# mmetcalf14/qml-cutensornet

Measured on AMD Instinct MI355X. Metric: Gram kernel entries/sec @ 60 qubits x 6 layers, higher is better.
Workload: dtype f64 (complex128)

## Files before the change

qml-cutensornet_amd/csrc/qk_fused.h:

```cpp
#pragma once
#include "qk_device.h"
#include "qk_plan.h"

#define QKF_PRIO_LO() __builtin_amdgcn_s_setprio(0)
#define QKF_PRIO_HI() __builtin_amdgcn_s_setprio(2)
typedef double v2d __attribute__((ext_vector_type(2)));
typedef __attribute__((address_space(3))) v2d lds_v2d;
static constexpr int QKF_XSTEP = 4 * TILE;
static constexpr int QKF_XBLOCK = TILE * TILE;


#ifndef QKF_LDS3M
#define QKF_LDS3M 0
#endif
#ifndef QKF_P2_PROBE
#define QKF_P2_PROBE 0
#endif
#ifndef QKF_ABL
#define QKF_ABL 0
#endif
#define QKF_STEP_BARRIER()                            \
  do {                                                \
    if (QKF_ABL & 4) asm volatile("s_waitcnt lgkmcnt(0)" ::: "memory"); \
    else qk_lds_barrier();                            \
  } while (0)
#define QKF_SUM(a, b) ((QKF_ABL & 1) ? (a) : (a) + (b))
#define QKF_DIF(a, b) ((QKF_ABL & 1) ? (b) : (a) - (b))
template <bool CONJB>
__device__ __forceinline__ void qkf_kstep(v4d& p1, v4d& p2, v4d& p3, const double ar, const double ai, const double br, const double bi) {
  const double sa = QKF_SUM(ar, ai), sb = CONJB ? QKF_DIF(br, bi) : QKF_SUM(br, bi);
  p1 = __builtin_amdgcn_mfma_f64_16x16x4f64(ar, br, p1, 0, 0, 0);
  p2 = __builtin_amdgcn_mfma_f64_16x16x4f64(ai, bi, p2, 0, 0, 0);
  p3 = __builtin_amdgcn_mfma_f64_16x16x4f64(sa, sb, p3, 0, 0, 0);
}

struct QkfTile {
  v4d re, im;
};

__device__ __forceinline__ v2d qkf_ldg(const v2d* __restrict__ base, const unsigned off) {
  return *reinterpret_cast<const v2d*>(reinterpret_cast<const char*>(base) + (size_t)(off * 16u));
}
#ifndef QKF_NT_A
#define QKF_NT_A 0
#endif
#ifndef QKF_NT_B
#define QKF_NT_B 0
#endif
__device__ __forceinline__ v2d qkf_ldg_nt(const v2d* __restrict__ base, const unsigned off) {
  return __builtin_nontemporal_load(reinterpret_cast<const v2d*>(reinterpret_cast<const char*>(base) + (size_t)(off * 16u)));
}
__device__ __forceinline__ v2d qkf_ldg_a(const v2d* __restrict__ base, const unsigned off) { return QKF_NT_A ? qkf_ldg_nt(base, off) : qkf_ldg(base, off); }
__device__ __forceinline__ v2d qkf_ldg_b(const v2d* __restrict__ base, const unsigned off) { return QKF_NT_B ? qkf_ldg_nt(base, off) : qkf_ldg(base, off); }
__device__ __forceinline__ v2d qkf_ldx(const v2d* __restrict__ base, const unsigned off) { return qkf_ldg(base, off); }
__device__ __forceinline__ v2d qkf_ldx(const lds_v2d* base, const unsigned off) { return base[off]; }

struct QkfStream {
  const v2d* base;
  unsigned off;
  int step;
  int lim = 4;
};
__device__ __forceinline__ const v2d* qkf_kbase(const v2d* const base, const int step, const int i, const int lim) { return base + max(min(i, lim - 1), 0) * step; }
__device__ __forceinline__ void qkf_load4(v2d (&fr)[4], const QkfStream& st) {
#pragma unroll
  for (int i = 0; i < 4; ++i) fr[i] = qkf_ldg(qkf_kbase(st.base, st.step, i, st.lim), st.off);
}
__device__ __forceinline__ v2d qkf_ldgb(const v2d* __restrict__ base, const unsigned boff) {
  const v2d* const at = reinterpret_cast<const v2d*>(reinterpret_cast<const char*>(base) + (size_t)boff);
  return QKF_NT_B ? __builtin_nontemporal_load(at) : *at;
}
struct QkfXLds {
  const lds_v2d* p;
  __device__ __forceinline__ void advance() { p += 4 * QKF_XSTEP; }
  __device__ __forceinline__ v2d kstep(const int i) const { return p[i * QKF_XSTEP]; }
};
struct QkfXGlobal {
  const v2d* base;
  unsigned bo;
  __device__ __forceinline__ void advance() { bo += 4 * QKF_XSTEP * 16u; }
  __device__ __forceinline__ v2d kstep(const int i) const { return *reinterpret_cast<const v2d*>(reinterpret_cast<const char*>(base + i * QKF_XSTEP) + (size_t)bo); }
};
__device__ __forceinline__ QkfXLds qkf_xcursor(const lds_v2d* xp, const unsigned xoff) { return QkfXLds{xp + xoff}; }
__device__ __forceinline__ QkfXGlobal qkf_xcursor(const v2d* xp, const unsigned xoff) { return QkfXGlobal{xp, xoff * 16u}; }

template <typename XPtr>
__device__ __forceinline__ void qkf_p1_tile(QkfTile& t, v2d (&fr)[4], const bool primed, QkfStream cur, XPtr xp, unsigned xoff, const int nks, const QkfStream nxt) {
  v4d p1 = {0, 0, 0, 0}, p2 = {0, 0, 0, 0}, p3 = {0, 0, 0, 0};
  v2d fx[4];
  const int ng = (nks + 3) >> 2, last = nks - 4 * (ng - 1);
  if (!primed) qkf_load4(fr, cur);
#pragma unroll
  for (int i = 0; i < 4; ++i) fx[i] = qkf_ldx(xp + i * QKF_XSTEP, xoff);
  const v2d* cb[4];
#pragma unroll
  for (int i = 0; i < 4; ++i) cb[i] = qkf_kbase(cur.base, cur.step, i, ng == 2 ? last : 4);
  unsigned bo = cur.off * 16u;
  const unsigned bs = (unsigned)(4 * cur.step) * 16u;
  auto xq = qkf_xcursor(xp, xoff);
  QKF_PRIO_LO();
  int gq = 0;
  if (ng >= 2) {
    gq = 1;
    bo += bs, xq.advance();
#pragma unroll
    for (int i = 0; i < 4; ++i) {
      if (i == 0) {
        const v4d z = {0, 0, 0, 0};
        p1 = __builtin_amdgcn_mfma_f64_16x16x4f64(fx[0].x, fr[0].x, z, 0, 0, 0);
        p2 = __builtin_amdgcn_mfma_f64_16x16x4f64(fx[0].y, fr[0].y, z, 0, 0, 0);
        p3 = __builtin_amdgcn_mfma_f64_16x16x4f64(QKF_SUM(fx[0].x, fx[0].y), QKF_SUM(fr[0].x, fr[0].y), z, 0, 0, 0);
      } else {
        qkf_kstep<false>(p1, p2, p3, fx[i].x, fx[i].y, fr[i].x, fr[i].y);
      }
      if (!(QKF_ABL & 2)) fr[i] = qkf_ldgb(cb[i], bo);
      if (!(QKF_ABL & 8)) fx[i] = xq.kstep(i);
      __builtin_amdgcn_sched_barrier(0);
    }
  }
#pragma unroll 1
  for (int pass = 0; pass < 2; ++pass) {
    const int end = ng - 2 + pass;
#pragma unroll 1
    for (; gq < end; ++gq) {
      bo += bs, xq.advance();
#pragma unroll
      for (int i = 0; i < 4; ++i) {
        qkf_kstep<false>(p1, p2, p3, fx[i].x, fx[i].y, fr[i].x, fr[i].y);
        if (!(QKF_ABL & 2)) fr[i] = qkf_ldgb(cb[i], bo);
        if (!(QKF_ABL & 8)) fx[i] = xq.kstep(i);
        __builtin_amdgcn_sched_barrier(0);
      }
    }
#pragma unroll
    for (int i = 0; i < 4; ++i) cb[i] = qkf_kbase(cur.base, cur.step, i, last);
  }
#pragma unroll
  for (int i = 0; i < 4; ++i) {
    if (i < last) qkf_kstep<false>(p1, p2, p3, fx[i].x, fx[i].y, fr[i].x, fr[i].y);
    if (!(QKF_ABL & 2)) fr[i] = qkf_ldg(qkf_kbase(nxt.base, nxt.step, i, nxt.lim), nxt.off);
    __builtin_amdgcn_sched_barrier(0);
  }
  QKF_PRIO_HI();
  t.re = p1 - p2;
  t.im = p3 - p1 - p2;
}

typedef __attribute__((address_space(3))) int lds_int;
struct QkfTurn {
  lds_int* at;
  int idx;
  lds_int* broken;
  unsigned long long* gerr;
};
__device__ __forceinline__ void qkf_turn_add(__attribute__((address_space(3))) double* const d, const long rs, const v4d& re, const v4d& im, const QkfTurn& t, const int tn) {
  lds_int* const turn = t.at + tn;
  if (t.idx > 0) {
    int spins = 0;
#ifdef QKF_FIRST_STORE
    while (__builtin_amdgcn_readfirstlane(__hip_atomic_load(turn, __ATOMIC_RELAXED, __HIP_MEMORY_SCOPE_WORKGROUP)) == 0) {
#else
    while (__builtin_amdgcn_readfirstlane(__hip_atomic_load(turn, __ATOMIC_RELAXED, __HIP_MEMORY_SCOPE_WORKGROUP)) != t.idx) {
#endif
      __builtin_amdgcn_s_sleep(1);
      if (++spins > (1 << 20) || __builtin_amdgcn_readfirstlane(__hip_atomic_load(t.broken, __ATOMIC_RELAXED, __HIP_MEMORY_SCOPE_WORKGROUP)) != 0) {
        __hip_atomic_store(t.broken, 1, __ATOMIC_RELAXED, __HIP_MEMORY_SCOPE_WORKGROUP);
        if (t.gerr) *t.gerr = 1ull;
        break;
      }
    }
#pragma unroll
    for (int r = 0; r < 4; ++r) {
      __hip_atomic_fetch_add(d + r * rs, re[r], __ATOMIC_RELAXED, __HIP_MEMORY_SCOPE_WORKGROUP);
      __hip_atomic_fetch_add(d + r * rs + 1, im[r], __ATOMIC_RELAXED, __HIP_MEMORY_SCOPE_WORKGROUP);
    }
  } else {
#pragma unroll
    for (int r = 0; r < 4; ++r) *(lds_v2d*)(d + r * rs) = (v2d){re[r], im[r]};
  }
#ifdef QKF_FIRST_STORE
  if (t.idx > 0) return;
#endif
  asm volatile("s_waitcnt lgkmcnt(0)" ::: "memory");
  __hip_atomic_store(turn, t.idx + 1, __ATOMIC_RELAXED, __HIP_MEMORY_SCOPE_WORKGROUP);
}

template <bool FULL, bool DET = false>
__device__ __forceinline__ void qkf_p2_item(const QkfTile& t, v2d (&fr)[4], const bool primed, QkfStream cur, const int ps, const int nn, const int kmax, lds_v2d* xo, const int q,
                                            const int j, const QkfStream nxt, const QkfTurn turn = QkfTurn{nullptr, 0, nullptr, nullptr}) {
  if (!primed) qkf_load4(fr, cur);
  __attribute__((address_space(3))) double* d = (__attribute__((address_space(3))) double*)(xo + q * TILE + j);
  if constexpr (!DET) {
    const v4d z = {0, 0, 0, 0};
    const v4d s = t.re + t.im;
#pragma unroll 1
    for (int tn = 0; tn < nn; ++tn) {
      v4d p1 = z, re, im;
      double sp[4], sm[4];
      const bool fin = tn + 1 == nn;
      const v2d* const rb = fin ? nxt.base : cur.base;
      const int rs = fin ? nxt.step : cur.step, rl = fin ? nxt.lim : FULL ? 4 : kmax;
      cur.off = fin ? nxt.off : cur.off + TILE;
      QKF_PRIO_LO();
#pragma unroll
      for (int i = 0; i < 4; ++i) {
        if (FULL || i == 0 || i < kmax) {
          p1 = __builtin_amdgcn_mfma_f64_16x16x4f64(s[i], fr[i].x, i == 0 ? z : p1, 0, 0, 0);
          sp[i] = QKF_DIF(-fr[i].x, fr[i].y), sm[i] = QKF_DIF(fr[i].y, fr[i].x);
        }
        if (!(QKF_ABL & 2)) fr[i] = qkf_ldg_a(qkf_kbase(rb, rs, i, rl), cur.off);
        __builtin_amdgcn_sched_barrier(0);
      }
#pragma unroll
      for (int i = 0; i < 4; ++i) {
        if (FULL || i == 0 || i < kmax) {
          re = __builtin_amdgcn_mfma_f64_16x16x4f64(t.im[i], sm[i], i == 0 ? p1 : re, 0, 0, 0);
          im = __builtin_amdgcn_mfma_f64_16x16x4f64(t.re[i], sp[i], i == 0 ? p1 : im, 0, 0, 0);
        }
        __builtin_amdgcn_sched_barrier(0);
      }
      QKF_PRIO_HI();
#pragma unroll
      for (int r = 0; r < 4; ++r) {
        __hip_atomic_fetch_add(d + r * 2 * QKF_XSTEP, re[r], __ATOMIC_RELAXED, __HIP_MEMORY_SCOPE_WORKGROUP);
        __hip_atomic_fetch_add(d + r * 2 * QKF_XSTEP + 1, im[r], __ATOMIC_RELAXED, __HIP_MEMORY_SCOPE_WORKGROUP);
      }
      d += 2 * ps;
    }
    return;
  }
#pragma unroll 1
  for (int tn = 0; tn < nn; ++tn) {
    v4d p1 = {0, 0, 0, 0}, p2 = {0, 0, 0, 0}, p3 = {0, 0, 0, 0};
    const bool fin = tn + 1 == nn;
    const v2d* const rb = fin ? nxt.base : cur.base;
    const int rs = fin ? nxt.step : cur.step, rl = fin ? nxt.lim : FULL ? 4 : kmax;
    cur.off = fin ? nxt.off : cur.off + TILE;
    QKF_PRIO_LO();
#pragma unroll
    for (int i = 0; i < 4; ++i) {
      if (FULL || i < kmax) qkf_kstep<true>(p1, p2, p3, t.re[i], t.im[i], fr[i].x, fr[i].y);
      if (!(QKF_ABL & 2)) fr[i] = qkf_ldg_a(qkf_kbase(rb, rs, i, rl), cur.off);
      __builtin_amdgcn_sched_barrier(0);
    }
    QKF_PRIO_HI();
    const v4d re = p1 + p2, im = p3 - p1 + p2;
    qkf_turn_add(d, (long)2 * QKF_XSTEP, re, im, turn, tn);
    d += 2 * ps;
  }
}

template <int S>
__device__ __forceinline__ void qkf_rotate(QkfTile (&T)[S], const int L) {
  if constexpr (S >= 2) {
    if (L == 2) {
      const QkfTile t = T[S - 2];
      T[S - 2] = T[S - 1], T[S - 1] = t;
    }
  }
  if constexpr (S >= 3) {
    if (L == 3) {
      const QkfTile t = T[S - 3];
      T[S - 3] = T[S - 2], T[S - 2] = T[S - 1], T[S - 1] = t;
    }
  }
  if constexpr (S >= 4) {
    if (L >= 4) {
      const QkfTile t0 = T[0];
#pragma unroll
      for (int e = 0; e + 1 < S; ++e) T[e] = T[e + 1];
      T[S - 1] = t0;
    }
  }
}

#ifdef QKF_EDGE_PAIRS_V
#define QKF_EDGE_PAIRS(WPS) (QKF_EDGE_PAIRS_V != 0)
#else
#define QKF_EDGE_PAIRS(WPS) false
#endif
#ifdef QKF_EDGE_SETS_V
#define QKF_EDGE_SETS(WPS) (QKF_EDGE_SETS_V)
#else
#define QKF_EDGE_SETS(WPS) ((WPS) <= 3 ? 2 : 1)
#endif
__device__ __forceinline__ v2d qkf_lde(const v2d* __restrict__ base, const unsigned boff, const int col = 0) {
  return reinterpret_cast<const v2d*>(reinterpret_cast<const char*>(base) + (size_t)boff)[col];
}
template <bool HAS1, bool MORE>
__device__ __forceinline__ void qkf_edge_group(v4d (&acc)[6], v2d (&fy)[4], v2d (&fz)[4], v2d (&fx)[4], const v2d* const* const by, const v2d* const* const bx, const unsigned boy,
                                               const unsigned box) {
#pragma unroll
  for (int i = 0; i < 4; ++i) {
    const double sb = QKF_DIF(fx[i].x, fx[i].y);
    acc[0] = __builtin_amdgcn_mfma_f64_16x16x4f64(fy[i].x, fx[i].x, acc[0], 0, 0, 0);
    acc[1] = __builtin_amdgcn_mfma_f64_16x16x4f64(fy[i].y, fx[i].y, acc[1], 0, 0, 0);
    acc[2] = __builtin_amdgcn_mfma_f64_16x16x4f64(QKF_SUM(fy[i].x, fy[i].y), sb, acc[2], 0, 0, 0);
    if (HAS1) {
      acc[3] = __builtin_amdgcn_mfma_f64_16x16x4f64(fz[i].x, fx[i].x, acc[3], 0, 0, 0);
      acc[4] = __builtin_amdgcn_mfma_f64_16x16x4f64(fz[i].y, fx[i].y, acc[4], 0, 0, 0);
      acc[5] = __builtin_amdgcn_mfma_f64_16x16x4f64(QKF_SUM(fz[i].x, fz[i].y), sb, acc[5], 0, 0, 0);
    }
    if (MORE) {
      fy[i] = qkf_lde(by[i], boy);
      if (HAS1) fz[i] = qkf_lde(by[i], boy, TILE);
      fx[i] = qkf_lde(bx[i], box);
    }
    __builtin_amdgcn_sched_barrier(0);
  }
}
template <bool HAS1, int SETS>
__device__ __forceinline__ void qkf_edge_unit(QkfTile& t0, QkfTile& t1, const v2d* __restrict__ Ay, const unsigned oy, const int ldy, const v2d* __restrict__ Ax, const unsigned ox, const int ldx,
                                              const int ng) {
  static_assert(SETS == 1 || SETS == 2, "one or two groups of k-steps in flight");
  v4d acc[6];
#pragma unroll
  for (int e = 0; e < 6; ++e) acc[e] = (v4d){0, 0, 0, 0};
  v2d fy[SETS][4], fz[SETS][4], fx[SETS][4];
  const v2d *by[4 * SETS], *bx[4 * SETS];
#pragma unroll
  for (int i = 0; i < 4 * SETS; ++i) by[i] = Ay + 4 * i * ldy, bx[i] = Ax + 4 * i * ldx;
  unsigned boy = oy * 16u, box = ox * 16u;
  const unsigned sy = (unsigned)(SETS * TILE * ldy) * 16u, sx = (unsigned)(SETS * TILE * ldx) * 16u;
  const bool two = SETS == 2 && ng > 1;
#pragma unroll
  for (int s = 0; s < SETS; ++s) {
    if (s == 0 || two) {
#pragma unroll
      for (int i = 0; i < 4; ++i) {
        fy[s][i] = qkf_lde(by[4 * s + i], boy);
        if (HAS1) fz[s][i] = qkf_lde(by[4 * s + i], boy, TILE);
        fx[s][i] = qkf_lde(bx[4 * s + i], box);
      }
    }
  }
  QKF_PRIO_LO();
#pragma unroll 1
  for (int g = SETS; g < ng; g += SETS) {
    boy += sy, box += sx;
#pragma unroll
    for (int s = 0; s < SETS; ++s) qkf_edge_group<HAS1, true>(acc, fy[s], fz[s], fx[s], by + 4 * s, bx + 4 * s, boy, box);
  }
  qkf_edge_group<HAS1, false>(acc, fy[0], fz[0], fx[0], by, bx, boy, box);
  if constexpr (SETS == 2) {
    if (two) qkf_edge_group<HAS1, false>(acc, fy[1], fz[1], fx[1], by + 4, bx + 4, boy, box);
  }
  QKF_PRIO_HI();
  t0.re = acc[0] + acc[1], t0.im = acc[2] - acc[0] + acc[1];
  if (HAS1) t1.re = acc[3] + acc[4], t1.im = acc[5] - acc[3] + acc[4];
}
__device__ __forceinline__ long long qkf_uniform(const long long v) {
  const unsigned lo = __builtin_amdgcn_readfirstlane((unsigned)v);
  const unsigned hi = __builtin_amdgcn_readfirstlane((unsigned)((unsigned long long)v >> 32));
  return (long long)(((unsigned long long)hi << 32) | lo);
}

template <int NW, bool PAIRS>
__device__ __forceinline__ QkEdgeUnit qkf_edge_unit_of(const int u, const int mt, const int nt, const int inv) {
  if constexpr (PAIRS) return qk_edge_unit(u, mt, nt, NW, inv);
  const int tb = (u * inv) >> 20;
  return QkEdgeUnit{u - tb * mt, tb, false, true};
}
template <int NW, bool PAIRS, int SETS>
__device__ __forceinline__ void qkf_edge_prefix(const SweepArgs& g, const int xi, const int yj, const int a, const int b, lds_v2d* const xl, v2d* const xg, const bool to_global, const int wave,
                                                const int q, const int j) {
  const v2d* const Lx = reinterpret_cast<const v2d*>(g.xedge) + qkf_uniform(g.xedge_offs[2 * (long long)xi]);
  const v2d* const Ly = reinterpret_cast<const v2d*>(g.yedge) + qkf_uniform(g.yedge_offs[2 * (long long)yj]);
  const int mt = a / TILE, nt = b / TILE, ng = (1 << g.edge_k) >> 4, inv = qk_recip20(mt), units = PAIRS ? qk_edge_units(mt, nt, NW) : mt * nt;
  for (int u = wave; u < units; u += NW) {
    const QkEdgeUnit un = qkf_edge_unit_of<NW, PAIRS>(u, mt, nt, inv);
    if (!un.mine) continue;
    QkfTile T0, T1;
    const unsigned oy = (unsigned)(q * b + un.tb0 * TILE + j), ox = (unsigned)(q * a + un.ta * TILE + j);
    if (un.has1) qkf_edge_unit<true, 1>(T0, T1, Ly, oy, b, Lx, ox, a, ng);
    else qkf_edge_unit<false, SETS>(T0, T1, Ly, oy, b, Lx, ox, a, ng);
    const int at = un.ta * (b * TILE) + (un.tb0 * TILE + q) * TILE + j;
    if (to_global) {
#pragma unroll
      for (int r = 0; r < 4; ++r) xg[at + r * QKF_XSTEP] = (v2d){T0.re[r], T0.im[r]};
      if (un.has1) {
#pragma unroll
        for (int r = 0; r < 4; ++r) xg[at + QKF_XBLOCK + r * QKF_XSTEP] = (v2d){T1.re[r], T1.im[r]};
      }
    } else {
#pragma unroll
      for (int r = 0; r < 4; ++r) xl[at + r * QKF_XSTEP] = (v2d){T0.re[r], T0.im[r]};
      if (un.has1) {
#pragma unroll
        for (int r = 0; r < 4; ++r) xl[at + QKF_XBLOCK + r * QKF_XSTEP] = (v2d){T1.re[r], T1.im[r]};
      }
    }
  }
}

template <int NW, bool PAIRS, int SETS>
__device__ __forceinline__ void qkf_edge_suffix(const SweepArgs& g, const int xi, const int yj, const int a, const int b, const lds_v2d* const xl, const v2d* const xg, const bool from_global,
                                                __attribute__((address_space(3))) double* zacc, const int wave, const int q, const int j) {
  const v2d* const Rx = reinterpret_cast<const v2d*>(g.xedge) + qkf_uniform(g.xedge_offs[2 * (long long)xi + 1]);
  const v2d* const Ry = reinterpret_cast<const v2d*>(g.yedge) + qkf_uniform(g.yedge_offs[2 * (long long)yj + 1]);
  const int mt = a / TILE, nt = b / TILE, ng = (1 << g.edge_k) >> 4, inv = qk_recip20(mt), units = PAIRS ? qk_edge_units(mt, nt, NW) : mt * nt;
  double zr = 0, zi = 0;
  for (int u = wave; u < units; u += NW) {
    const QkEdgeUnit un = qkf_edge_unit_of<NW, PAIRS>(u, mt, nt, inv);
    if (!un.mine) continue;
    QkfTile T0, T1;
    const unsigned oy = (unsigned)(q * b + un.tb0 * TILE + j), ox = (unsigned)(q * a + un.ta * TILE + j);
    if (un.has1) qkf_edge_unit<true, 1>(T0, T1, Ry, oy, b, Rx, ox, a, ng);
    else qkf_edge_unit<false, SETS>(T0, T1, Ry, oy, b, Rx, ox, a, ng);
    const int at = un.ta * (b * TILE) + (un.tb0 * TILE + q) * TILE + j;
#pragma unroll
    for (int r = 0; r < 4; ++r) {
      const v2d x = from_global ? xg[at + r * QKF_XSTEP] : (v2d)xl[at + r * QKF_XSTEP];
      zr += x.x * T0.re[r] - x.y * T0.im[r], zi += x.x * T0.im[r] + x.y * T0.re[r];
    }
    if (un.has1) {
#pragma unroll
      for (int r = 0; r < 4; ++r) {
        const v2d x = from_global ? xg[at + QKF_XBLOCK + r * QKF_XSTEP] : (v2d)xl[at + QKF_XBLOCK + r * QKF_XSTEP];
        zr += x.x * T1.re[r] - x.y * T1.im[r], zi += x.x * T1.im[r] + x.y * T1.re[r];
      }
    }
  }
#pragma unroll
  for (int o = 32; o > 0; o >>= 1) zr += __shfl_xor(zr, o), zi += __shfl_xor(zi, o);
  if ((q | j) == 0) zacc[2 * wave] = zr, zacc[2 * wave + 1] = zi;
}

struct QkfSite {
  int a, a2, b, b2, at, nks, mt, nt, nn, W, inv, inv2, pd, ps, next;
  bool small;
  const v2d *Ak, *Bk;
};
typedef int v4i __attribute__((ext_vector_type(4)));
typedef __attribute__((address_space(3))) v4i lds_v4i;

template <int XCAP, int NT, bool ITEM_RECIPS = false>
__device__ __forceinline__ void qkf_step_table(const SweepArgs& g, const int xi, const int yj, const long long pair, lds_v4i* const rec, long long* const m_off, const int tid, const QkSegRule rule) {
  const int ns = g.n_sites, n1 = ns + 1;
  const int32_t* const xd = g.xdims + (long long)xi * n1;
  const int32_t* const yd = g.ydims + (long long)yj * n1;
  const int32_t* const xt = g.xtrue + (long long)xi * n1;
  const int32_t* const yt = g.ytrue + (long long)yj * n1;
  const v2d* const xdata = reinterpret_cast<const v2d*>(g.xdata);
  const v2d* const ydata = reinterpret_cast<const v2d*>(g.ydata);
  auto put = [&](const int e, const int a, const int a2, const int b, const int b2, const int ps, const int next, const bool small, const v2d* const A, const v2d* const B)
                 __attribute__((always_inline)) {
    const int mt = a / TILE, nt = b2 / TILE;
    const int W = small ? nt : max(1, min(nt, XCAP / (TILE * a2)));
    rec[3 * e] = (v4i){a, a2, b, b2};
    rec[3 * e + 1] = (v4i){xt[e], (yt[e] + 3) >> 2, W, small ? 1 : 0};
    rec[3 * e + 2] = (v4i){qk_recip20(mt), ps, next, ITEM_RECIPS ? qk_unit_recips(nt, W, false) : 0};
    m_off[2 * e] = (long long)(((const char*)A - (const char*)xdata) / 16);
    m_off[2 * e + 1] = (long long)(((const char*)B - (const char*)ydata) / 16);
  };
  auto plain = [&](const int e, const int next) __attribute__((always_inline)) {
    const int a = xd[e], a2 = xd[e + 1], b = yd[e], b2 = yd[e + 1];
    put(e, a, a2, b, b2, 1, next, qk_seg_small(rule, a, a2, b, b2, 2), xdata + (g.xoffs[(long long)xi * ns + e] >> 1), ydata + (g.yoffs[(long long)yj * ns + e] >> 1));
  };
  if (g.seg == nullptr) {
    for (int e = tid; e < ns; e += NT) plain(e, e + 1);
    return;
  }
  const int ek = g.edge_k, k_hi = ns - ek;
  const unsigned long long w0 = g.seg[2 * pair], w1 = g.seg[2 * pair + 1];
  for (int e = ek + tid; e < k_hi; e += NT) {
    const int i = e - ek;
    if (qk_seg_bit(w0, w1, i) && e + 1 < k_hi) {
      const int a = xd[e], a2 = xd[e + 2], b = yd[e], b2 = yd[e + 2];
      put(e, a, a2, b, b2, 2, e + 2, qk_seg_small(rule, a, a2, b, b2, 4), reinterpret_cast<const v2d*>(g.xmg) + (g.xmg_offs[(long long)xi * g.merge_steps + i] >> 1),
          reinterpret_cast<const v2d*>(g.ymg) + (g.ymg_offs[(long long)yj * g.merge_steps + i] >> 1));
    } else plain(e, e + 1);
  }
}

#ifdef QKF_PROF
#define QKF_PROF_DECL() \
  unsigned long long pf[8] = {0, 0, 0, 0, 0, 0, 0, 0}, pt = __builtin_amdgcn_s_memtime(); \
  const unsigned long long pt0 = pt
#define QKF_STAMP(i)                                              \
  do {                                                            \
    const unsigned long long now_ = __builtin_amdgcn_s_memtime(); \
    pf[i] += now_ - pt;                                           \
    pt = now_;                                                    \
  } while (0)
#define QKF_PROF_FLUSH()                                             \
  do {                                                               \
    if (lane == 0) {                                                 \
      pf[7] = __builtin_amdgcn_s_memtime() - pt0;                    \
      for (int i_ = 0; i_ < 8; ++i_) atomicAdd(g.prof + i_, pf[i_]); \
    }                                                                \
  } while (0)
#else
#define QKF_PROF_DECL()
#define QKF_STAMP(i)
#define QKF_PROF_FLUSH()
#endif

#define QKF_PULLER(NT) ((NT) - 64)
__device__ __forceinline__ void qkf_pull_next(const SweepArgs& g, const int xcc, int& gang_round, long long* const word) {
  const long long pp = qk_pull(g, xcc);
  qk_gang_sync(g, xcc, pp >= 0, gang_round);
  *word = pp;
}

template <int NW, int S, int XCAP, int WPS, bool DET = false>
__global__ __launch_bounds__(64 * NW, WPS) void qk_sweep_fused_kernel(const SweepArgs g) {
  constexpr int NT = 64 * NW;
  extern __shared__ __attribute__((aligned(16))) double lds_raw[];
  lds_v2d* const XL = (lds_v2d*)lds_raw;
  long long* const slot = reinterpret_cast<long long*>(lds_raw + 2 * XCAP);
  const v2d* const xdata = reinterpret_cast<const v2d*>(g.xdata);
  const v2d* const ydata = reinterpret_cast<const v2d*>(g.ydata);
  v2d* const G0 = reinterpret_cast<v2d*>(g.scratch) + (long long)blockIdx.x * 2 * g.x_plane;
  const int tid = threadIdx.x, lane = tid & 63;
  const int wave = __builtin_amdgcn_readfirstlane(tid >> 6);
  const int j = lane & 15, q = lane >> 4;
  const int ns = g.n_sites;
  __attribute__((address_space(3))) double* const zacc = (__attribute__((address_space(3))) double*)(slot + 2);
  lds_v4i* const rec = (lds_v4i*)(slot + 2 + 32);
  long long* const m_off = reinterpret_cast<long long*>(slot + 2 + 32) + 6 * (long long)ns;
  lds_int* const tbroken = (lds_int*)(m_off + 2 * (long long)ns);
  lds_int* const turn0 = tbroken + 2;
  auto rfl = [&](const int v) __attribute__((always_inline)) { return __builtin_amdgcn_readfirstlane(v); };
  auto ldl = [&](const long long* p_) __attribute__((always_inline)) {
    const long long v = *p_;
    const unsigned lo = __builtin_amdgcn_readfirstlane((unsigned)v);
    const unsigned hi = __builtin_amdgcn_readfirstlane((unsigned)((unsigned long long)v >> 32));
    return (long long)(((unsigned long long)hi << 32) | lo);
  };
  auto site = [&](const int k) __attribute__((always_inline)) {
    const v4i r0 = rec[3 * k], r1 = rec[3 * k + 1], r2 = rec[3 * k + 2];
    QkfSite s;
    s.a = rfl(r0.x), s.a2 = rfl(r0.y), s.b = rfl(r0.z), s.b2 = rfl(r0.w);
    s.at = rfl(r1.x), s.nks = rfl(r1.y), s.W = rfl(r1.z), s.small = rfl(r1.w) != 0;
    s.inv = rfl(r2.x), s.inv2 = rfl(r2.w);
    s.ps = rfl(r2.y), s.pd = 1 << s.ps, s.next = rfl(r2.z);
    s.mt = s.a / TILE, s.nt = s.b2 / TILE, s.nn = s.a2 / TILE;
    s.Ak = xdata + ldl(m_off + 2 * k);
    s.Bk = ydata + ldl(m_off + 2 * k + 1);
    return s;
  };
  auto item_of = [&](const QkfSite& s, const int w, const int it) __attribute__((always_inline)) {
    return DET ? qk_unit_decode_ordered(it, s.ps, s.mt, s.inv) : qk_unit_decode(it, s.mt, w, s.inv, qk_unit_recip_of(s.inv2, w == s.W));
  };
  auto b_stream = [&](const QkfSite& s, const int s0, const int w, const int it) __attribute__((always_inline)) {
    const QkUnit un = item_of(s, w, it);
    return QkfStream{s.Bk + un.p * s.b2, (unsigned)((q * s.pd) * s.b2 + (s0 + un.tc) * TILE + j), 4 * s.pd * s.b2, min(4, s.nks)};
  };
  auto a_stream = [&](const QkfSite& s, const int w, const int it) __attribute__((always_inline)) {
    const QkUnit un = item_of(s, w, it);
    return QkfStream{s.Ak + un.p * s.a2, (unsigned)(((un.ta * TILE + q) * s.pd) * s.a2 + j), 4 * s.pd * s.a2, min(4, (s.at - un.ta * TILE + 3) >> 2)};
  };
  QKF_PROF_DECL();
  const int xcc = qk_xcc_id();
  int gang_round = 0;
  if (tid == 0) qk_tail_start(g);
  for (;;) {
    if (tid == 0) {
      const long long pp_ = qk_pull(g, xcc);
      qk_gang_sync(g, xcc, pp_ >= 0, gang_round);
      *slot = pp_;
    }
    __syncthreads();
    const long long p = *slot;
    __syncthreads();
    if (p < 0) break;
    const int xi = g.pairs[2 * p], yj = g.pairs[2 * p + 1];
    qkf_step_table<XCAP, NT, true>(g, xi, yj, p, rec, m_off, tid, QkSegRule{XCAP, NW * S, false});
    const int ek = g.edge_k, k_hi = ns - ek;
    const bool edges = ek > 0;
    if (!edges)
      for (int e = tid; e < TILE * TILE; e += NT) XL[e] = (v2d){e == 0 ? 1.0 : 0.0, 0.0};
    if constexpr (DET)
      for (int e = tid; e < 2 * g.turn_ints + 2; e += NT) tbroken[e] = 0;
    int tsel = 0;
    __syncthreads();
    bool xg = false;
    int cur = 0, xb = 0;
    if (edges) {
      const v4i r0 = rec[3 * ek];
      const int a_e = rfl(r0.x), b_e = rfl(r0.z);
      xg = a_e * b_e > XCAP;
      qkf_edge_prefix<NW, QKF_EDGE_PAIRS(WPS), QKF_EDGE_SETS(WPS)>(g, xi, yj, a_e, b_e, XL, G0, xg, wave, q, j);
      __syncthreads();
    }
    QKF_STAMP(0);
    QkfTile T[S];
    v2d fr[4];
    bool primed = false;
    QkfSite sn = site(ek);
    for (int k = ek; k < k_hi;) {
      const QkfSite sc = sn;
      k = sc.next;
      if (k < k_hi) sn = site(k);
      const int a = sc.a, a2 = sc.a2, b = sc.b, mt = sc.mt, nt = sc.nt, W = sc.W;
      const bool small = sc.small;
      v2d* const Gc = G0 + (long long)cur * g.x_plane;
      v2d* const Gn = G0 + (long long)(cur ^ 1) * g.x_plane;
      if (small && xg) {
        for (int e = tid; e < a * b; e += NT) XL[e] = Gc[e];
        __syncthreads();
        xg = false, xb = 0;
      } else if (!small && !xg) {
        for (int e = tid; e < a * b; e += NT) Gc[e] = XL[xb + e];
        __syncthreads();
        xg = true;
      }
      const int n_out = sc.b2 * a2;
      const bool pingpong = small && a * b + n_out <= XCAP;
      const int ob = !small ? 0 : pingpong ? (xb == 0 ? XCAP - n_out : 0) : 0;
      if (pingpong && !DET)
        for (int e = tid; e < n_out; e += NT) XL[ob + e] = (v2d){0.0, 0.0};
      QKF_STAMP(1);
      for (int s0 = 0; s0 < nt; s0 += W) {
        const int w = min(W, nt - s0), items = sc.pd * mt * w;
        lds_int* const tcur = turn0 + tsel * g.turn_ints;
        if constexpr (DET) {
          for (int e = tid; e < g.turn_ints; e += NT) turn0[(tsel ^ 1) * g.turn_ints + e] = 0;
        } else if (!small) {
          for (int e = tid; e < w * TILE * a2; e += NT) XL[e] = (v2d){0.0, 0.0};
          QKF_STEP_BARRIER();
        }
        QKF_STAMP(6);
        for (int r0 = 0; r0 < items; r0 += NW * S) {
          const int L = min(S, (items - r0 + NW - 1) / NW);
          const bool multi = L > 1;
          const int it0 = r0 + wave;
          auto phase1 = [&](auto xbase) __attribute__((always_inline)) {
#pragma unroll 1
            for (int s = 0; s < L; ++s) {
              if (multi) qkf_rotate<S>(T, L);
              const int it = it0 + NW * s;
              if (it < items) {
                const int ta = item_of(sc, w, it).ta;
                const bool more = s + 1 < L && it + NW < items;
                const QkfStream nxt = more ? b_stream(sc, s0, w, it + NW) : a_stream(sc, w, it0);
                qkf_p1_tile(T[S - 1], fr, primed, b_stream(sc, s0, w, it), xbase, (unsigned)(ta * (b * TILE) + q * TILE + j), sc.nks, nxt);
                primed = true;
              }
            }
          };
          if (xg) phase1((const v2d*)Gc);
          else phase1((const lds_v2d*)(XL + xb));
          QKF_STAMP(2);
          if (small && r0 == 0 && !(DET && pingpong)) {
            QKF_STEP_BARRIER();
            if (!pingpong && !DET) {
              for (int e = tid; e < n_out; e += NT) XL[e] = (v2d){0.0, 0.0};
              QKF_STEP_BARRIER();
            }
          }
          QKF_STAMP(3);
          const bool last_round = s0 + W >= nt && r0 + NW * S >= items;
#pragma unroll 1
          for (int s = 0; s < S; ++s) {
            const int it = it0 + NW * s;
            if (it >= items) break;
            if (multi) qkf_rotate<S>(T, L);
            const QkUnit un = item_of(sc, w, it);
            const int ta = un.ta, tbl = un.tc;
            const int kmax = min(4, (sc.at - ta * TILE + 3) >> 2);
            const bool more = s + 1 < S && it + NW < items;
            const int wn = min(sn.W, sn.nt);
            const bool chain = !more && last_round && k < k_hi && wave < sn.pd * sn.mt * wn;
            const QkfStream nxt = more ? a_stream(sc, w, it + NW) : chain ? b_stream(sn, 0, wn, wave) : a_stream(sc, w, it);
            const int tix = sc.pd * ta + un.p;
            const QkfTurn turn{tcur + tbl * sc.nn, tix, tbroken, g.err};
            if (kmax == 4) qkf_p2_item<true, DET>(T[S - 1], fr, primed, a_stream(sc, w, it), w * QKF_XBLOCK, sc.nn, 4, XL + ob + tbl * QKF_XBLOCK, q, j, nxt, turn);
            else qkf_p2_item<false, DET>(T[S - 1], fr, primed, a_stream(sc, w, it), w * QKF_XBLOCK, sc.nn, kmax, XL + ob + tbl * QKF_XBLOCK, q, j, nxt, turn);
            primed = more || chain;
          }
          QKF_STAMP(4);
        }
        QKF_STEP_BARRIER();
        tsel ^= 1;
        QKF_STAMP(5);
        if (!small && nt > W) {
          for (int tn = 0; tn < sc.nn; ++tn)
            for (int e = tid; e < w * QKF_XBLOCK; e += NT) Gn[(long long)tn * (sc.b2 * TILE) + s0 * QKF_XBLOCK + e] = XL[tn * w * QKF_XBLOCK + e];
          __syncthreads();
          QKF_STAMP(1);
        }
      }
      if (!small) {
        if (nt > W) cur ^= 1;
        else xg = false, xb = 0;
      } else {
        xb = ob;
      }
    }
    if (edges) {
      const v4i r0 = rec[3 * (k_hi - 1)];
      const int a_e = rfl(r0.y), b_e = rfl(r0.w);
      qkf_edge_suffix<NW, QKF_EDGE_PAIRS(WPS), QKF_EDGE_SETS(WPS)>(g, xi, yj, a_e, b_e, (const lds_v2d*)(XL + xb), (const v2d*)(G0 + (long long)cur * g.x_plane), xg, zacc, wave, q, j);
      __syncthreads();
    }
    if (tid == 0) {
      v2d zz = {0.0, 0.0};
      if (edges)
        for (int w_ = 0; w_ < NW; ++w_) zz.x += zacc[2 * w_], zz.y += zacc[2 * w_ + 1];
      else zz = xg ? G0[(long long)cur * g.x_plane] : (v2d)XL[xb];
      g.values[p] = zz.x * zz.x + zz.y * zz.y;
      if (g.z) {
        g.z[2 * p] = zz.x;
        g.z[2 * p + 1] = zz.y;
      }
    }
    __syncthreads();
  }
  if (tid == 0) qk_tail_exit(g);
  QKF_PROF_FLUSH();
}

template <bool HAS1, typename XPtr>
__device__ __forceinline__ void qkf_p1_dual(QkfTile& t0, QkfTile& t1, v2d (&fr)[4], v2d (&fs)[4], const bool primed, QkfStream cur, XPtr xp, unsigned xoff, const int nks,
                                            const QkfStream nxt) {
  v4d p1 = {0, 0, 0, 0}, p2 = {0, 0, 0, 0}, p3 = {0, 0, 0, 0}, r1 = {0, 0, 0, 0}, r2 = {0, 0, 0, 0}, r3 = {0, 0, 0, 0};
  v2d fx[4];
  if (!primed) qkf_load4(fr, cur);
  if (HAS1) {
#pragma unroll
    for (int i = 0; i < 4; ++i) fs[i] = qkf_ldg(cur.base + i * cur.step, cur.off + TILE);
  }
#pragma unroll
  for (int i = 0; i < 4; ++i) fx[i] = qkf_ldx(xp + i * QKF_XSTEP, xoff);
  const int ng = (nks + 3) >> 2, last = nks - 4 * (ng - 1);
  QKF_PRIO_LO();
  int gq = 0;
  if (ng >= 2) {
    gq = 1;
    cur.off += 4 * cur.step, xoff += 4 * QKF_XSTEP;
#pragma unroll
    for (int i = 0; i < 4; ++i) {
      if (i == 0) {
        const v4d z = {0, 0, 0, 0};
        const double sa = QKF_SUM(fx[0].x, fx[0].y);
        p1 = __builtin_amdgcn_mfma_f64_16x16x4f64(fx[0].x, fr[0].x, z, 0, 0, 0);
        p2 = __builtin_amdgcn_mfma_f64_16x16x4f64(fx[0].y, fr[0].y, z, 0, 0, 0);
        p3 = __builtin_amdgcn_mfma_f64_16x16x4f64(sa, QKF_SUM(fr[0].x, fr[0].y), z, 0, 0, 0);
        if (HAS1) {
          r1 = __builtin_amdgcn_mfma_f64_16x16x4f64(fx[0].x, fs[0].x, z, 0, 0, 0);
          r2 = __builtin_amdgcn_mfma_f64_16x16x4f64(fx[0].y, fs[0].y, z, 0, 0, 0);
          r3 = __builtin_amdgcn_mfma_f64_16x16x4f64(sa, QKF_SUM(fs[0].x, fs[0].y), z, 0, 0, 0);
        }
      } else {
        qkf_kstep<false>(p1, p2, p3, fx[i].x, fx[i].y, fr[i].x, fr[i].y);
        if (HAS1) qkf_kstep<false>(r1, r2, r3, fx[i].x, fx[i].y, fs[i].x, fs[i].y);
      }
      if (!(QKF_ABL & 2)) fr[i] = qkf_ldg_b(cur.base + i * cur.step, cur.off);
      if (HAS1 && !(QKF_ABL & 2)) fs[i] = qkf_ldg_b(cur.base + i * cur.step, cur.off + TILE);
      if (!(QKF_ABL & 8)) fx[i] = qkf_ldx(xp + i * QKF_XSTEP, xoff);
      __builtin_amdgcn_sched_barrier(0);
    }
  }
#pragma unroll 1
  for (; gq + 1 < ng; ++gq) {
    cur.off += 4 * cur.step, xoff += 4 * QKF_XSTEP;
#pragma unroll
    for (int i = 0; i < 4; ++i) {
      qkf_kstep<false>(p1, p2, p3, fx[i].x, fx[i].y, fr[i].x, fr[i].y);
      if (HAS1) qkf_kstep<false>(r1, r2, r3, fx[i].x, fx[i].y, fs[i].x, fs[i].y);
      if (!(QKF_ABL & 2)) fr[i] = qkf_ldg_b(cur.base + i * cur.step, cur.off);
      if (HAS1 && !(QKF_ABL & 2)) fs[i] = qkf_ldg_b(cur.base + i * cur.step, cur.off + TILE);
      if (!(QKF_ABL & 8)) fx[i] = qkf_ldx(xp + i * QKF_XSTEP, xoff);
      __builtin_amdgcn_sched_barrier(0);
    }
  }
#pragma unroll
  for (int i = 0; i < 4; ++i) {
    if (i < last) {
      qkf_kstep<false>(p1, p2, p3, fx[i].x, fx[i].y, fr[i].x, fr[i].y);
      if (HAS1) qkf_kstep<false>(r1, r2, r3, fx[i].x, fx[i].y, fs[i].x, fs[i].y);
    }
    if (!(QKF_ABL & 2)) fr[i] = qkf_ldg(nxt.base + i * nxt.step, nxt.off);
    __builtin_amdgcn_sched_barrier(0);
  }
  QKF_PRIO_HI();
  t0.re = p1 - p2, t0.im = p3 - p1 - p2;
  if (HAS1) t1.re = r1 - r2, t1.im = r3 - r1 - r2;
}

typedef __attribute__((address_space(3))) double lds_double;
template <bool FULL, bool HAS1>
__device__ __forceinline__ void qkf_p2_block(const QkfTile& t0, const QkfTile& t1, const v4d& s0, const v4d& s1, v2d (&fr)[4], const int kmax, const v2d* const b0, const v2d* const b1,
                                             const v2d* const b2, const v2d* const b3, const unsigned off, lds_double* const d, lds_double* const d1, const long rs) {
  const v4d z = {0, 0, 0, 0};
  v4d p1 = z, r1 = z, re, im, re1, im1;
  double sp[4], sm[4];
  QKF_PRIO_LO();
#pragma unroll
  for (int i = 0; i < 4; ++i) {
    if (FULL || i == 0 || i < kmax) {
      p1 = __builtin_amdgcn_mfma_f64_16x16x4f64(s0[i], fr[i].x, i == 0 ? z : p1, 0, 0, 0);
      if (HAS1) r1 = __builtin_amdgcn_mfma_f64_16x16x4f64(s1[i], fr[i].x, i == 0 ? z : r1, 0, 0, 0);
      sp[i] = QKF_DIF(-fr[i].x, fr[i].y), sm[i] = QKF_DIF(fr[i].y, fr[i].x);
    }
    if (!(QKF_ABL & 2)) fr[i] = qkf_ldg_a(i == 0 ? b0 : i == 1 ? b1 : i == 2 ? b2 : b3, off);
    __builtin_amdgcn_sched_barrier(0);
  }
#pragma unroll
  for (int i = 0; i < 4; ++i) {
    if (FULL || i == 0 || i < kmax) {
      re = __builtin_amdgcn_mfma_f64_16x16x4f64(t0.im[i], sm[i], i == 0 ? p1 : re, 0, 0, 0);
      im = __builtin_amdgcn_mfma_f64_16x16x4f64(t0.re[i], sp[i], i == 0 ? p1 : im, 0, 0, 0);
      if (HAS1) {
        re1 = __builtin_amdgcn_mfma_f64_16x16x4f64(t1.im[i], sm[i], i == 0 ? r1 : re1, 0, 0, 0);
        im1 = __builtin_amdgcn_mfma_f64_16x16x4f64(t1.re[i], sp[i], i == 0 ? r1 : im1, 0, 0, 0);
      }
    }
    __builtin_amdgcn_sched_barrier(0);
  }
  QKF_PRIO_HI();
#pragma unroll
  for (int r = 0; r < 4; ++r) {
    __hip_atomic_fetch_add(d + r * rs, re[r], __ATOMIC_RELAXED, __HIP_MEMORY_SCOPE_WORKGROUP);
    __hip_atomic_fetch_add(d + r * rs + 1, im[r], __ATOMIC_RELAXED, __HIP_MEMORY_SCOPE_WORKGROUP);
  }
  if (HAS1) {
#pragma unroll
    for (int r = 0; r < 4; ++r) {
      __hip_atomic_fetch_add(d1 + r * rs, re1[r], __ATOMIC_RELAXED, __HIP_MEMORY_SCOPE_WORKGROUP);
      __hip_atomic_fetch_add(d1 + r * rs + 1, im1[r], __ATOMIC_RELAXED, __HIP_MEMORY_SCOPE_WORKGROUP);
    }
  }
}
template <bool FULL, bool HAS1, bool DET>
__device__ __forceinline__ void qkf_p2_dual_turn(const QkfTile& t0, const QkfTile& t1, v2d (&fr)[4], v2d (&fs)[4], QkfStream cur, const int ps, const int nn, const int kmax, lds_v2d* xo, const int q,
                                            const int j, const QkfStream nxt, const bool nxt_p1, const unsigned n1, const QkfTurn turn = QkfTurn{nullptr, 0, nullptr, nullptr}) {
  __attribute__((address_space(3))) double* d = (__attribute__((address_space(3))) double*)(xo + q * TILE + j);
#pragma unroll 1
  for (int tn = 0; tn < nn; ++tn) {
    v4d p1 = {0, 0, 0, 0}, p2 = {0, 0, 0, 0}, p3 = {0, 0, 0, 0}, r1 = {0, 0, 0, 0}, r2 = {0, 0, 0, 0}, r3 = {0, 0, 0, 0};
    const bool fin = tn + 1 == nn;
    const v2d* const rb = fin ? nxt.base : cur.base;
    const int rs = fin ? nxt.step : cur.step;
    cur.off = fin ? nxt.off : cur.off + TILE;
    QKF_PRIO_LO();
#pragma unroll
    for (int i = 0; i < 4; ++i) {
      if (FULL || i < kmax) {
        qkf_kstep<true>(p1, p2, p3, t0.re[i], t0.im[i], fr[i].x, fr[i].y);
        if (HAS1) qkf_kstep<true>(r1, r2, r3, t1.re[i], t1.im[i], fr[i].x, fr[i].y);
      }
      fr[i] = qkf_ldg_a(rb + i * rs, cur.off);
      __builtin_amdgcn_sched_barrier(0);
    }
    QKF_PRIO_HI();
    {
      const v4d re = p1 + p2, im = p3 - p1 + p2;
      if constexpr (DET) qkf_turn_add(d, (long)2 * QKF_XSTEP, re, im, turn, tn);
      else {
#pragma unroll
        for (int r = 0; r < 4; ++r) {
          __hip_atomic_fetch_add(d + r * 2 * QKF_XSTEP, re[r], __ATOMIC_RELAXED, __HIP_MEMORY_SCOPE_WORKGROUP);
          __hip_atomic_fetch_add(d + r * 2 * QKF_XSTEP + 1, im[r], __ATOMIC_RELAXED, __HIP_MEMORY_SCOPE_WORKGROUP);
        }
      }
    }
    if (HAS1) {
      const v4d re = r1 + r2, im = r3 - r1 + r2;
      __attribute__((address_space(3))) double* const d1 = d + 2 * QKF_XBLOCK;
      if constexpr (DET) qkf_turn_add(d1, (long)2 * QKF_XSTEP, re, im, QkfTurn{turn.at + nn, turn.idx, turn.broken, turn.gerr}, tn);
      else {
#pragma unroll
        for (int r = 0; r < 4; ++r) {
          __hip_atomic_fetch_add(d1 + r * 2 * QKF_XSTEP, re[r], __ATOMIC_RELAXED, __HIP_MEMORY_SCOPE_WORKGROUP);
          __hip_atomic_fetch_add(d1 + r * 2 * QKF_XSTEP + 1, im[r], __ATOMIC_RELAXED, __HIP_MEMORY_SCOPE_WORKGROUP);
        }
      }
    }
    d += 2 * ps;
  }
}

template <bool FULL, bool HAS1, bool DET = false>
__device__ __forceinline__ void qkf_p2_dual(const QkfTile& t0, const QkfTile& t1, v2d (&fr)[4], v2d (&fs)[4], QkfStream cur, const int ps, const int nn, const int kmax, lds_v2d* xo, const int q,
                                            const int j, const QkfStream nxt, const bool nxt_p1, const unsigned n1, const QkfTurn turn = QkfTurn{nullptr, 0, nullptr, nullptr}) {
  if constexpr (DET) {
    qkf_p2_dual_turn<FULL, HAS1, DET>(t0, t1, fr, fs, cur, ps, nn, kmax, xo, q, j, nxt, nxt_p1, n1, turn);
    return;
  }
  lds_double* d = (lds_double*)(xo + q * TILE + j);
  lds_double* d1 = d + 2 * QKF_XBLOCK;
  constexpr long rs = 2 * QKF_XSTEP;
  const v4d s0 = t0.re + t0.im, s1 = HAS1 ? t1.re + t1.im : s0;
  const v2d *const c0 = cur.base, *const c1 = cur.base + cur.step, *const c2 = cur.base + 2 * cur.step, *const c3 = cur.base + 3 * cur.step;
  unsigned off = cur.off;
#pragma unroll 1
  for (int tn = 0; tn + 1 < nn; ++tn) {
    off += TILE;
    qkf_p2_block<FULL, HAS1>(t0, t1, s0, s1, fr, kmax, c0, c1, c2, c3, off, d, d1, rs);
    d += 2 * ps, d1 += 2 * ps;
  }
  qkf_p2_block<FULL, HAS1>(t0, t1, s0, s1, fr, kmax, nxt.base, nxt.base + nxt.step, nxt.base + 2 * nxt.step, nxt.base + 3 * nxt.step, nxt.off, d, d1, rs);
}

template <int NW, int XCAP, int WPS, bool DET = false>
__global__ __launch_bounds__(64 * NW, WPS) void qk_sweep_fused_dual_kernel(const SweepArgs g) {
  constexpr int NT = 64 * NW;
  extern __shared__ __attribute__((aligned(16))) double lds_raw[];
  lds_v2d* const XL = (lds_v2d*)lds_raw;
  long long* const slot = reinterpret_cast<long long*>(lds_raw + 2 * XCAP);
  const v2d* const xdata = reinterpret_cast<const v2d*>(g.xdata);
  const v2d* const ydata = reinterpret_cast<const v2d*>(g.ydata);
  v2d* const G0 = reinterpret_cast<v2d*>(g.scratch) + (long long)blockIdx.x * 2 * g.x_plane;
  const int tid = threadIdx.x, lane = tid & 63;
  const int wave = __builtin_amdgcn_readfirstlane(tid >> 6);
  const int j = lane & 15, q = lane >> 4;
  const int ns = g.n_sites;
  __attribute__((address_space(3))) double* const zacc = (__attribute__((address_space(3))) double*)(slot + 2);
  lds_v4i* const rec = (lds_v4i*)(slot + 2 + 32);
  long long* const m_off = reinterpret_cast<long long*>(slot + 2 + 32) + 6 * (long long)ns;
  lds_int* const tbroken = (lds_int*)(m_off + 2 * (long long)ns);
  lds_int* const turn0 = tbroken + 2;
  auto rfl = [&](const int v) __attribute__((always_inline)) { return __builtin_amdgcn_readfirstlane(v); };
  auto ldl = [&](const long long* p_) __attribute__((always_inline)) {
    const long long v = *p_;
    const unsigned lo = __builtin_amdgcn_readfirstlane((unsigned)v);
    const unsigned hi = __builtin_amdgcn_readfirstlane((unsigned)((unsigned long long)v >> 32));
    return (long long)(((unsigned long long)hi << 32) | lo);
  };
  auto site = [&](const int k) __attribute__((always_inline)) {
    const v4i r0 = rec[3 * k], r1 = rec[3 * k + 1], r2 = rec[3 * k + 2];
    QkfSite s;
    s.a = rfl(r0.x), s.a2 = rfl(r0.y), s.b = rfl(r0.z), s.b2 = rfl(r0.w);
    s.at = rfl(r1.x), s.nks = rfl(r1.y), s.W = rfl(r1.z), s.small = rfl(r1.w) != 0;
    s.inv = rfl(r2.x);
    s.ps = rfl(r2.y), s.pd = 1 << s.ps, s.next = rfl(r2.z);
    s.mt = s.a / TILE, s.nt = s.b2 / TILE, s.nn = s.a2 / TILE;
    s.Ak = xdata + ldl(m_off + 2 * k);
    s.Bk = ydata + ldl(m_off + 2 * k + 1);
    return s;
  };
  auto pair_of = [&](const QkfSite& s, const int v) __attribute__((always_inline)) { return qk_unit_decode_ordered(v, s.ps, s.mt, s.inv); };
  auto b_stream = [&](const QkfSite& s, const int s0, const int v, const int half) __attribute__((always_inline)) {
    const QkUnit un = pair_of(s, v);
    return QkfStream{s.Bk + un.p * s.b2, (unsigned)((q * s.pd) * s.b2 + (s0 + 2 * un.tc + half) * TILE + j), 4 * s.pd * s.b2};
  };
  struct Unit {
    bool mine, has1;
    int v, half;
  };
  auto unit_of = [&](const QkfSite& s, const int w, const int units, const int r0) __attribute__((always_inline)) {
    Unit un;
    const int left = units - r0;
    const bool halves = 2 * left <= NW;
    un.half = (halves && wave >= left) ? 1 : 0;
    un.v = r0 + wave - (un.half ? left : 0);
    const int tp = pair_of(s, un.v).tc;
    const bool second = 2 * tp + 1 < w;
    un.mine = un.v < units && (un.half == 0 || second);
    un.has1 = !halves && second;
    return un;
  };
  auto a_stream = [&](const QkfSite& s, const int v) __attribute__((always_inline)) {
    const QkUnit un = pair_of(s, v);
    return QkfStream{s.Ak + un.p * s.a2, (unsigned)(((un.ta * TILE + q) * s.pd) * s.a2 + j), 4 * s.pd * s.a2};
  };
  QKF_PROF_DECL();
  const int xcc = qk_xcc_id();
  int gang_round = 0;
  if (tid == 0) qk_tail_start(g);
  if (tid == QKF_PULLER(NT)) qkf_pull_next(g, xcc, gang_round, slot);
  __syncthreads();
  long long p = slot[0];
  int psel = 0;
  auto table_of = [&](const long long pp) __attribute__((always_inline)) {
    if (pp < 0) return;
    const int xi_ = g.pairs[2 * pp], yj_ = g.pairs[2 * pp + 1];
    qkf_step_table<XCAP, NT>(g, xi_, yj_, pp, rec, m_off, tid, QkSegRule{XCAP, NW, true});
  };
  table_of(p);
  while (p >= 0) {
    const int xi = g.pairs[2 * p], yj = g.pairs[2 * p + 1];
    const int ek = g.edge_k, k_hi = ns - ek;
    const bool edges = ek > 0;
    if (!edges)
      for (int e = tid; e < TILE * TILE; e += NT) XL[e] = (v2d){e == 0 ? 1.0 : 0.0, 0.0};
    if constexpr (DET)
      for (int e = tid; e < 2 * g.turn_ints + 2; e += NT) tbroken[e] = 0;
    int tsel = 0;
    __syncthreads();
    bool xg = false;
    int cur = 0, xb = 0;
    if (edges) {
      const v4i r0 = rec[3 * ek];
      const int a_e = rfl(r0.x), b_e = rfl(r0.z);
      xg = a_e * b_e > XCAP;
      qkf_edge_prefix<NW, QKF_EDGE_PAIRS(WPS), QKF_EDGE_SETS(WPS)>(g, xi, yj, a_e, b_e, XL, G0, xg, wave, q, j);
      __syncthreads();
    }
    QKF_STAMP(0);
    QkfTile T0, T1;
    v2d fr[4], fs[4];
    bool primed = false;
    QkfSite sn = site(ek);
    for (int k = ek; k < k_hi;) {
      const QkfSite sc = sn;
      k = sc.next;
      if (k < k_hi) sn = site(k);
      const int a = sc.a, a2 = sc.a2, b = sc.b, mt = sc.mt, nt = sc.nt, W = sc.W;
      const bool small = sc.small;
      v2d* const Gc = G0 + (long long)cur * g.x_plane;
      v2d* const Gn = G0 + (long long)(cur ^ 1) * g.x_plane;
      if (small && xg) {
        for (int e = tid; e < a * b; e += NT) XL[e] = Gc[e];
        __syncthreads();
        xg = false, xb = 0;
      } else if (!small && !xg) {
        for (int e = tid; e < a * b; e += NT) Gc[e] = XL[xb + e];
        __syncthreads();
        xg = true;
      }
      const int n_out = sc.b2 * a2;
      const bool pingpong = small && a * b + n_out <= XCAP;
      const int ob = !small ? 0 : pingpong ? (xb == 0 ? XCAP - n_out : 0) : 0;
      if (pingpong && !DET)
        for (int e = tid; e < n_out; e += NT) XL[ob + e] = (v2d){0.0, 0.0};
      QKF_STAMP(1);
      for (int s0 = 0; s0 < nt; s0 += W) {
        const int w = min(W, nt - s0), units = sc.pd * mt * ((w + 1) >> 1);
        lds_int* const tcur = turn0 + tsel * g.turn_ints;
        if constexpr (DET) {
          for (int e = tid; e < g.turn_ints; e += NT) turn0[(tsel ^ 1) * g.turn_ints + e] = 0;
        } else if (!small) {
          for (int e = tid; e < w * TILE * a2; e += NT) XL[e] = (v2d){0.0, 0.0};
          QKF_STEP_BARRIER();
        }
        for (int r0 = 0; r0 < units; r0 += NW) {
          const Unit un = unit_of(sc, w, units, r0);
          const int v = un.v;
          const bool mine = un.mine, has1 = un.has1;
          const QkUnit pr = pair_of(sc, v);
          const int tp = pr.tc, ta = pr.ta;
          if (mine) {
            const QkfStream bs = b_stream(sc, s0, v, un.half), as = a_stream(sc, v);
            const unsigned xoff = (unsigned)(ta * (b * TILE) + q * TILE + j);
            if (xg) {
              if (has1) qkf_p1_dual<true>(T0, T1, fr, fs, primed, bs, (const v2d*)Gc, xoff, sc.nks, as);
              else qkf_p1_dual<false>(T0, T1, fr, fs, primed, bs, (const v2d*)Gc, xoff, sc.nks, as);
            } else {
              if (has1) qkf_p1_dual<true>(T0, T1, fr, fs, primed, bs, (const lds_v2d*)(XL + xb), xoff, sc.nks, as);
              else qkf_p1_dual<false>(T0, T1, fr, fs, primed, bs, (const lds_v2d*)(XL + xb), xoff, sc.nks, as);
            }
          }
          QKF_STAMP(2);
          if (small && r0 == 0 && !(DET && pingpong)) {
            QKF_STEP_BARRIER();
            if (!pingpong && !DET) {
              for (int e = tid; e < n_out; e += NT) XL[e] = (v2d){0.0, 0.0};
              QKF_STEP_BARRIER();
            }
          }
          QKF_STAMP(3);
          if (mine) {
            const int kmax = min(4, (sc.at - ta * TILE + 3) >> 2);
            QkfStream nxt = a_stream(sc, v);
            bool np1 = false;
            if (r0 + NW < units) {
              const Unit nu = unit_of(sc, w, units, r0 + NW);
              if (nu.mine) nxt = b_stream(sc, s0, nu.v, nu.half), np1 = true;
            } else if (s0 + W < nt) {
              const int w2 = min(W, nt - s0 - W);
              const Unit nu = unit_of(sc, w2, sc.pd * mt * ((w2 + 1) >> 1), 0);
              if (nu.mine) nxt = b_stream(sc, s0 + W, nu.v, nu.half), np1 = true;
            } else if (k < k_hi) {
              const int w2 = min(sn.W, sn.nt);
              const Unit nu = unit_of(sn, w2, sn.pd * sn.mt * ((w2 + 1) >> 1), 0);
              if (nu.mine) nxt = b_stream(sn, 0, nu.v, nu.half), np1 = true;
            }
            const unsigned nd1 = 0;
            lds_v2d* const xo = XL + ob + (2 * tp + un.half) * QKF_XBLOCK;
            const QkfTurn tp_turn{tcur + (2 * tp + un.half) * sc.nn, sc.pd * ta + pr.p, tbroken, g.err};
            if (has1) {
              if (kmax == 4) qkf_p2_dual<true, true, DET>(T0, T1, fr, fs, a_stream(sc, v), w * QKF_XBLOCK, sc.nn, 4, xo, q, j, nxt, np1, nd1, tp_turn);
              else qkf_p2_dual<false, true, DET>(T0, T1, fr, fs, a_stream(sc, v), w * QKF_XBLOCK, sc.nn, kmax, xo, q, j, nxt, np1, nd1, tp_turn);
            } else {
              if (kmax == 4) qkf_p2_dual<true, false, DET>(T0, T1, fr, fs, a_stream(sc, v), w * QKF_XBLOCK, sc.nn, 4, xo, q, j, nxt, np1, nd1, tp_turn);
              else qkf_p2_dual<false, false, DET>(T0, T1, fr, fs, a_stream(sc, v), w * QKF_XBLOCK, sc.nn, kmax, xo, q, j, nxt, np1, nd1, tp_turn);
            }
            primed = np1;
          }
          QKF_STAMP(4);
        }
        QKF_STEP_BARRIER();
        tsel ^= 1;
        QKF_STAMP(5);
        if (!small && nt > W) {
          for (int tn = 0; tn < sc.nn; ++tn)
            for (int e = tid; e < w * QKF_XBLOCK; e += NT) Gn[(long long)tn * (sc.b2 * TILE) + s0 * QKF_XBLOCK + e] = XL[tn * w * QKF_XBLOCK + e];
          __syncthreads();
        }
      }
      if (!small) {
        if (nt > W) cur ^= 1;
        else xg = false, xb = 0;
      } else {
        xb = ob;
      }
    }
    if (tid == QKF_PULLER(NT)) qkf_pull_next(g, xcc, gang_round, slot + (psel ^ 1));
    if (edges) {
      const v4i r0 = rec[3 * (k_hi - 1)];
      const int a_e = rfl(r0.y), b_e = rfl(r0.w);
      qkf_edge_suffix<NW, QKF_EDGE_PAIRS(WPS), QKF_EDGE_SETS(WPS)>(g, xi, yj, a_e, b_e, (const lds_v2d*)(XL + xb), (const v2d*)(G0 + (long long)cur * g.x_plane), xg, zacc, wave, q, j);
    }
    __syncthreads();
    const long long pn = slot[psel ^ 1];
    if (tid == 0) {
      v2d zz = {0.0, 0.0};
      if (edges)
        for (int w_ = 0; w_ < NW; ++w_) zz.x += zacc[2 * w_], zz.y += zacc[2 * w_ + 1];
      else zz = xg ? G0[(long long)cur * g.x_plane] : (v2d)XL[xb];
      g.values[p] = zz.x * zz.x + zz.y * zz.y;
      if (g.z) {
        g.z[2 * p] = zz.x;
        g.z[2 * p + 1] = zz.y;
      }
    }
    table_of(pn);
    if (!edges) __syncthreads();
    p = pn, psel ^= 1;
    QKF_STAMP(6);
  }
  if (tid == 0) qk_tail_exit(g);
  QKF_PROF_FLUSH();
}

template <typename T>
__global__ void qk_interleave_kernel(const T* __restrict__ src, T* __restrict__ dst, const int32_t* __restrict__ dims, const int64_t* __restrict__ offs,
                                     const int n_sites, const long long n_tensors) {
  typedef T v2 __attribute__((ext_vector_type(2)));
  for (long long t = blockIdx.x; t < n_tensors; t += gridDim.x) {
    const long long s = t / n_sites;
    const int k = (int)(t - s * n_sites);
    const long long plane = (long long)dims[s * (n_sites + 1) + k] * 2 * dims[s * (n_sites + 1) + k + 1];
    const T* re = src + offs[t];
    const T* im = re + plane;
    v2* d = reinterpret_cast<v2*>(dst + offs[t]);
    for (long long e = threadIdx.x; e < plane; e += blockDim.x) d[e] = (v2){re[e], im[e]};
  }
}

template <int N>
__device__ __forceinline__ void qkw_wait_vmcnt() {
  static_assert(N >= 0 && N < 64, "vmcnt is a 6-bit field");
  asm volatile("s_waitcnt vmcnt(%0)" ::"n"(N) : "memory");
}

template <int NG, typename SRC>
__global__ __launch_bounds__(64, 2) void qk_sweep_wave2_kernel(const SweepArgs g) {
  constexpr bool F32 = sizeof(SRC) == 4;
  static_assert(!F32 || NG > 0, "complex64 images go through the LDS ring");
  constexpr int ES = F32 ? 8 : 16;
  constexpr int GROUP = F32 ? 128 : 256;
  __shared__ long long slot;
  __shared__ v2d ring[NG > 0 ? NG * GROUP : 1];
  typedef __attribute__((address_space(3))) void* lds_ptr_t;
  const int lane = threadIdx.x, j = lane & 15, q = lane >> 4;
  const unsigned ring_lds = (unsigned)(uintptr_t)(lds_ptr_t)ring + (F32 ? (unsigned)(q * 128 + j * 8) : (unsigned)lane * 16u);
  const int ns = g.n_sites, n1 = ns + 1;
  const char* const xdata = reinterpret_cast<const char*>(g.xdata);
  const char* const ydata = reinterpret_cast<const char*>(g.ydata);
  auto uni = [](const int v) __attribute__((always_inline)) { return __builtin_amdgcn_readfirstlane(v); };
  auto unil = [](const long long v) __attribute__((always_inline)) {
    const unsigned lo = __builtin_amdgcn_readfirstlane((unsigned)v);
    const unsigned hi = __builtin_amdgcn_readfirstlane((unsigned)((unsigned long long)v >> 32));
    return (long long)(((unsigned long long)hi << 32) | lo);
  };
  const int xcc = qk_xcc_id();
  if (lane == 0) qk_tail_start(g);
  for (;;) {
    if (lane == 0) slot = qk_pull(g, xcc);
    __syncthreads();
    const long long p = unil(slot);
    __syncthreads();
    if (p < 0) break;
    typedef const __attribute__((address_space(4))) int* sint_p;
    typedef const __attribute__((address_space(4))) int64_t* slong_p;
    const int xi = ((sint_p)g.pairs)[2 * p], yj = ((sint_p)g.pairs)[2 * p + 1];
    const sint_p xd = (sint_p)(g.xdims + (long long)xi * n1);
    const sint_p yd = (sint_p)(g.ydims + (long long)yj * n1);
    const sint_p xt = (sint_p)(g.xtrue + (long long)xi * n1);
    const sint_p yt = (sint_p)(g.ytrue + (long long)yj * n1);
    const slong_p xo = (slong_p)(g.xoffs + (long long)xi * ns);
    const slong_p yo = (slong_p)(g.yoffs + (long long)yj * ns);
    QkfTile XA[2][2], XN[2][2];
#pragma unroll
    for (int u = 0; u < 2; ++u)
#pragma unroll
      for (int v = 0; v < 2; ++v) XA[u][v].re = XA[u][v].im = XN[u][v].re = XN[u][v].im = (v4d){0, 0, 0, 0};
    XA[0][0].re[0] = (lane == 0) ? 1.0 : 0.0;
    int f_k = 0, f_i = 0, f_n = 0, f_slot = 0, c_slot = 0;
    int f_a2 = 0, f_b2 = 0;
    const char* f_A = xdata;
    const char* f_B = ydata;
    int desc = 0;
    auto enter = [&]() __attribute__((always_inline)) {
      const int fa = xd[f_k], fb = yd[f_k], fat = __builtin_amdgcn_readfirstlane(xt[f_k]), fbt = __builtin_amdgcn_readfirstlane(yt[f_k]);
      f_a2 = xd[f_k + 1], f_b2 = yd[f_k + 1];
      f_A = xdata + (xo[f_k] >> 1) * ES, f_B = ydata + (yo[f_k] >> 1) * ES;
      const int kb = fb >> 4, nn = f_a2 >> 4, mt = fa >> 4, nt = f_b2 >> 4, gpb = kb + nn;
      const int inv = (gpb == 2) ? 32768 : (gpb == 3) ? 21846 : 16384;
      const int gi = lane, blk = (gi * inv) >> 16, h = gi - blk * gpb, pp = blk & 1, r = blk >> 1;
      const int ta = (mt == 2) ? (r & 1) : 0, tb = (mt == 2) ? (r >> 1) : r;
      const bool is_b = h < kb;
      const int off = is_b ? ((h * TILE) * 2 + pp) * f_b2 + tb * TILE : ((ta * TILE) * 2 + pp) * f_a2 + (h - kb) * TILE;
      const int cnt = is_b ? min(4, (fbt - h * TILE + 3) >> 2) : min(4, (fat - ta * TILE + 3) >> 2);
      desc = off | (cnt << 16) | ((is_b ? 1 : 0) << 20);
      f_n = nt * mt * 2 * gpb, f_i = 0;
    };
    auto issue = [&]() __attribute__((always_inline)) {
      if (f_k >= ns) return;
      const int d = __builtin_amdgcn_readlane(desc, f_i);
      const int off = d & 0xffff, cnt = (d >> 16) & 7;
      const bool is_b = (d >> 20) != 0;
      const int ld = is_b ? f_b2 : f_a2;
      const char* const base = (is_b ? f_B : f_A) + (long)off * ES;
      if constexpr (F32) {
        const char* const src = base + (((lane >> 3) * 2) * ld + (lane & 7) * 2) * ES;
        const int last = (cnt - 1) >> 1;
#pragma unroll
        for (int pc = 0; pc < 2; ++pc) if (!(QKF_ABL & 16)) __builtin_amdgcn_global_load_lds(src + (min(pc, last) * 16 * ld) * ES, (lds_ptr_t)(ring + f_slot * GROUP + pc * 64), 16, 0, 0);
      } else {
        const char* const src = base + ((q * 2) * ld + j) * ES;
#pragma unroll
        for (int i = 0; i < 4; ++i) if (!(QKF_ABL & 16)) __builtin_amdgcn_global_load_lds(src + (min(i, cnt - 1) * 8 * ld) * ES, (lds_ptr_t)(ring + (f_slot * 4 + i) * 64), 16, 0, 0);
      }
      f_slot = (f_slot == NG - 1) ? 0 : f_slot + 1;
      if (++f_i == f_n) {
        if (++f_k < ns) enter();
      }
    };
    auto take = [&](v2d(&f)[4]) __attribute__((always_inline)) {
      issue();
      if (f_k >= ns) qkw_wait_vmcnt<0>();
      else qkw_wait_vmcnt<(NG > 0 ? (F32 ? 2 : 4) * (NG - 1) : 0)>();
      const unsigned at = ring_lds + (unsigned)c_slot * (unsigned)(GROUP * 16);
      if constexpr (F32) {
        double h[4];
        asm volatile("ds_read_b64 %0, %1" : "=v"(h[0]) : "v"(at));
        asm volatile("ds_read_b64 %0, %1 offset:512" : "=v"(h[1]) : "v"(at));
        asm volatile("ds_read_b64 %0, %1 offset:1024" : "=v"(h[2]) : "v"(at));
        asm volatile("ds_read_b64 %0, %1 offset:1536" : "=v"(h[3]) : "v"(at));
        asm volatile("s_waitcnt lgkmcnt(0)" : "+v"(h[0]), "+v"(h[1]), "+v"(h[2]), "+v"(h[3])::"memory");
#pragma unroll
        for (int i = 0; i < 4; ++i) {
          const long long bits = __double_as_longlong(h[i]);
          f[i] = (v2d){(double)__int_as_float((int)bits), (double)__int_as_float((int)(bits >> 32))};
        }
      } else if (QKF_ABL & 32) {
        asm volatile("" : "+v"(f[0]), "+v"(f[1]), "+v"(f[2]), "+v"(f[3]) : "v"(at));
      } else {
        asm volatile("ds_read_b128 %0, %1" : "=v"(f[0]) : "v"(at));
        asm volatile("ds_read_b128 %0, %1 offset:1024" : "=v"(f[1]) : "v"(at));
        asm volatile("ds_read_b128 %0, %1 offset:2048" : "=v"(f[2]) : "v"(at));
        asm volatile("ds_read_b128 %0, %1 offset:3072" : "=v"(f[3]) : "v"(at));
        asm volatile("s_waitcnt lgkmcnt(0)" : "+v"(f[0]), "+v"(f[1]), "+v"(f[2]), "+v"(f[3])::"memory");
      }
      c_slot = (c_slot == NG - 1) ? 0 : c_slot + 1;
    };
    if constexpr (NG > 0) {
      enter();
#pragma unroll
      for (int i = 0; i < NG - 1; ++i) issue();
    }
    int a_nx = xd[0], b_nx = yd[0], a2_nx = xd[1], b2_nx = yd[1], at_nx = xt[0], bt_nx = yt[0];
    long long xo_nx = xo[0], yo_nx = yo[0];
    for (int k = 0; k < ns; ++k) {
      const int a = a_nx, a2 = a2_nx, b = b_nx, b2 = b2_nx, at = at_nx, bt = bt_nx;
      const v2d* const Ak = reinterpret_cast<const v2d*>(xdata) + (xo_nx >> 1);
      const v2d* const Bk = reinterpret_cast<const v2d*>(ydata) + (yo_nx >> 1);
      {
        const int k1 = min(k + 1, ns - 1);
        a_nx = a2, b_nx = b2, a2_nx = xd[k1 + 1], b2_nx = yd[k1 + 1], at_nx = xt[k1], bt_nx = yt[k1];
        xo_nx = xo[k1], yo_nx = yo[k1];
      }
      const int mt = a >> 4, kb = b >> 4, nn = a2 >> 4, nt = b2 >> 4;
#pragma unroll
      for (int tb = 0; tb < 2; ++tb) {
        if (tb < nt) {
          v4d n1a[2], n2a[2], n3a[2];
#pragma unroll
          for (int tn = 0; tn < 2; ++tn) n1a[tn] = n2a[tn] = n3a[tn] = (v4d){0, 0, 0, 0};
#pragma unroll
          for (int ta = 0; ta < 2; ++ta) {
            if (ta < mt) {
              const int ka = min(4, (at - ta * TILE + 3) >> 2);
#pragma unroll
              for (int pp = 0; pp < 2; ++pp) {
                v4d p1 = {0, 0, 0, 0}, p2 = {0, 0, 0, 0}, p3 = {0, 0, 0, 0};
#pragma unroll
                for (int tk = 0; tk < 2; ++tk) {
                  if (tk < kb) {
                    const int kk = min(4, (bt - tk * TILE + 3) >> 2);
                    const v2d* const bp = Bk + ((tk * TILE + q) * 2 + pp) * b2 + tb * TILE + j;
                    v2d f[4];
                    if constexpr (NG > 0) take(f);
                    else {
#pragma unroll
                      for (int i = 0; i < 4; ++i) f[i] = bp[i * 8 * b2];
                    }
#pragma unroll
                    for (int i = 0; i < 4; ++i)
                      if (i < kk) qkf_kstep<false>(p1, p2, p3, XA[tk][ta].re[i], XA[tk][ta].im[i], f[i].x, f[i].y);
                  }
                }
                QkfTile t;
                if (QKF_ABL & 64) t.re = p1, t.im = p3;
                else t.re = p1 - p2, t.im = p3 - p1 - p2;
#pragma unroll
                for (int tn = 0; tn < 2; ++tn) {
                  if (tn < nn) {
                    const v2d* const ap = Ak + ((ta * TILE + q) * 2 + pp) * a2 + tn * TILE + j;
                    v2d f[4];
                    if constexpr (NG > 0) take(f);
                    else {
#pragma unroll
                      for (int i = 0; i < 4; ++i) f[i] = ap[i * 8 * a2];
                    }
#pragma unroll
                    for (int i = 0; i < 4; ++i)
                      if (i < ka) qkf_kstep<true>(n1a[tn], n2a[tn], n3a[tn], t.re[i], t.im[i], f[i].x, f[i].y);
                  }
                }
              }
            }
          }
#pragma unroll
          for (int tn = 0; tn < 2; ++tn) XN[tb][tn].re = n1a[tn] + n2a[tn], XN[tb][tn].im = n3a[tn] - n1a[tn] + n2a[tn];
        }
      }
#pragma unroll
      for (int u = 0; u < 2; ++u)
#pragma unroll
        for (int v = 0; v < 2; ++v) XA[u][v] = XN[u][v];
    }
    {
      const double re = __longlong_as_double(unil(__double_as_longlong(XA[0][0].re[0])));
      const double im = __longlong_as_double(unil(__double_as_longlong(XA[0][0].im[0])));
      g.values[p] = re * re + im * im;
      if (g.z) {
        g.z[2 * p] = re;
        g.z[2 * p + 1] = im;
      }
    }
  }
  if (lane == 0) qk_tail_exit(g);
}
```

qml-cutensornet_amd/csrc/qk_plan.h:

```cpp
#pragma once
#include "../../include/qkgram.h"

#include <algorithm>
#include <cstdint>
#include <cstdio>
#include <vector>

int qk_fail(int code, const char* fmt, ...) __attribute__((format(printf, 2, 3)));

#ifndef QKF_XCAP_ONE_V
#define QKF_XCAP_ONE_V 8192
#endif
#ifndef QKF_XCAP_TWO_V
#define QKF_XCAP_TWO_V 4608
#endif
#ifndef QKF_TWO_WGS
#define QKF_TWO_WGS 2
#endif
static constexpr int QKF_XCAP_ONE = QKF_XCAP_ONE_V, QKF_XCAP_TWO = QKF_XCAP_TWO_V;
static constexpr int QK_TILE = 16;
static inline int qk_pad16(int x) { return (x + QK_TILE - 1) / QK_TILE * QK_TILE; }
static constexpr int GMAX = 4;

#if defined(__HIPCC__)
#define QK_HD __host__ __device__
#else
#define QK_HD
#endif
struct QkUnit {
  int ta, tc, p;
};
QK_HD static inline int qk_unit_cols(const int w, const bool dual) { return dual ? (w + 1) >> 1 : w; }
QK_HD static inline int qk_recip20(const int d) { return ((1 << 20) + d - 1) / d; }
QK_HD static inline int qk_recip15(const int d) { return ((1 << 15) + d - 1) / d; }
QK_HD static inline int qk_unit_recips(const int nt, const int W, const bool dual) {
  const int wl = nt - (nt - 1) / W * W;
  return qk_recip15(qk_unit_cols(W, dual)) | (qk_recip15(qk_unit_cols(wl, dual)) << 16);
}
QK_HD static inline int qk_unit_recip_of(const int recips, const bool full_strip) { return full_strip ? (recips & 0xffff) : (int)((unsigned)recips >> 16); }
QK_HD static inline QkUnit qk_unit_decode(const int v, const int mt, const int wc, const int inv_mt, const int inv_wc) {
  const int c = (v * inv_mt) >> 20, p = (c * inv_wc) >> 15;
  return QkUnit{v - c * mt, c - p * wc, p};
}
QK_HD static inline QkUnit qk_unit_decode_ordered(const int v, const int ps, const int mt, const int inv_mt) {
  const int u = v >> ps, tc = (u * inv_mt) >> 20;
  return QkUnit{u - tc * mt, tc, v & ((1 << ps) - 1)};
}

struct QkEdgeUnit {
  int ta, tb0;
  bool has1, mine;
};
QK_HD static inline int qk_edge_units(const int mt, const int nt, const int NW) {
  const int pairs = mt * ((nt + 1) >> 1), r0 = (pairs - 1) / NW * NW, left = pairs - r0;
  return 2 * left <= NW ? r0 + 2 * left : pairs;
}
QK_HD static inline QkEdgeUnit qk_edge_unit(const int u, const int mt, const int nt, const int NW, const int inv_mt) {
  const int pairs = mt * ((nt + 1) >> 1), r0 = (pairs - 1) / NW * NW, left = pairs - r0;
  const bool halves = 2 * left <= NW, single = halves && u >= r0, half = halves && u >= r0 + left;
  const int v = u - (half ? left : 0), tp = (v * inv_mt) >> 20;
  const bool second = 2 * tp + 1 < nt;
  return QkEdgeUnit{v - tp * mt, 2 * tp + (half ? 1 : 0), !single && second, u < (halves ? r0 + 2 * left : pairs) && (!half || second)};
}

static constexpr int QK_STEP_PRICE = 375;
static constexpr int QK_SEG_BITS = 128;
struct QkSegRule {
  int xcap, cap;
  bool dual;
};
struct QkSegMask {
  unsigned long long w[2];
};
QK_HD static inline bool qk_seg_bit(const unsigned long long w0, const unsigned long long w1, const int i) { return i < QK_SEG_BITS && (((i < 64 ? w0 : w1) >> (i & 63)) & 1ull) != 0; }
QK_HD static inline bool qk_seg_one_round(const QkSegRule& r, const int pmt, const int nt) { return pmt * (r.dual ? (nt + 1) / 2 : nt) <= r.cap; }
QK_HD static inline bool qk_seg_small(const QkSegRule& r, const int a, const int a2, const int b, const int b2, const int pd) {
  return a * b <= r.xcap && a2 * b2 <= r.xcap && (qk_seg_one_round(r, pd * (a / QK_TILE), b2 / QK_TILE) || a * b + a2 * b2 <= r.xcap);
}
QK_HD static inline long long qk_step_instr(const int pd, const int a, const int a2, const int b, const int b2, const int at, const int bt) {
  return 3ll * pd * (b2 / QK_TILE) * ((long long)(a / QK_TILE) * ((bt + 3) >> 2) + (long long)(a2 / QK_TILE) * ((at + 3) >> 2));
}
QK_HD static inline bool qk_merge_admissible(const QkSegRule& r, const int32_t* const xd, const int32_t* const yd, const int e) {
  const int a = xd[e], am = xd[e + 1], a2 = xd[e + 2], b = yd[e], bm = yd[e + 1], b2 = yd[e + 2];
  const long long work_m = 4ll * a * b2 * (b + a2), work_p = 2ll * a * bm * (b + am) + 2ll * am * b2 * (bm + a2);
  return (qk_seg_small(r, a, a2, b, b2, 4) || (!qk_seg_small(r, a, am, b, bm, 2) && !qk_seg_small(r, am, a2, bm, b2, 2))) && work_m <= work_p;
}
QK_HD static inline QkSegMask qk_segment_chain(const int32_t* const xd, const int32_t* const xt, const int32_t* const yd, const int32_t* const yt, const int n_sites, const int ek,
                                               const QkSegRule& rule, const int parities, const bool greedy, long long* const objective = nullptr, int* const steps = nullptr) {
  const int m = n_sites - 2 * ek;
  auto may = [&](const int i) { return i + 1 < m && i < QK_SEG_BITS && ((parities >> (i & 1)) & 1) != 0 && qk_merge_admissible(rule, xd, yd, ek + i); };
  auto plain_cost = [&](const int i) { return qk_step_instr(2, xd[ek + i], xd[ek + i + 1], yd[ek + i], yd[ek + i + 1], xt[ek + i], yt[ek + i]) + QK_STEP_PRICE; };
  auto merged_cost = [&](const int i) { return qk_step_instr(4, xd[ek + i], xd[ek + i + 2], yd[ek + i], yd[ek + i + 2], xt[ek + i], yt[ek + i]) + QK_STEP_PRICE; };
  QkSegMask take{{0ull, 0ull}};
  if (greedy) {
    for (int i = 0; i < m && i < QK_SEG_BITS; ++i)
      if (may(i)) take.w[i >> 6] |= 1ull << (i & 63);
  } else {
    long long c1 = 0, c2 = 0;
    int s1 = 0, s2 = 0;
    for (int i = m - 1; i >= 0; --i) {
      long long c = plain_cost(i) + c1;
      int s = s1 + 1;
      if (may(i)) {
        const long long cm = merged_cost(i) + c2;
        const int sm = s2 + 1;
        if (cm < c || (cm == c && (sm < s || (sm == s && (i & 1) == 0)))) c = cm, s = sm, take.w[i >> 6] |= 1ull << (i & 63);
      }
      c2 = c1, s2 = s1, c1 = c, s1 = s;
    }
  }
  QkSegMask out{{0ull, 0ull}};
  long long obj = 0;
  int n_steps = 0;
  for (int i = 0; i < m; ++n_steps) {
    if (qk_seg_bit(take.w[0], take.w[1], i)) out.w[i >> 6] |= 1ull << (i & 63), obj += merged_cost(i), i += 2;
    else obj += plain_cost(i), i += 1;
  }
  if (objective) *objective = obj;
  if (steps) *steps = n_steps;
  return out;
}

struct qk_ctx;

struct qk_plan {
  int n_sites = 0, nx = 0, ny = 0;
  bool symmetric = false;
  bool quad = false;
  int world = 1, rank = 0;
  int64_t total_pairs = 0, max_per_rank = 0;
  std::vector<int32_t> pairs;
  std::vector<int32_t> groups;
  int group = 1;
  qk_stats stats{};
  qk_stats second{};
  int64_t n_first = 0;
  int nq = 1;
  int64_t qstart[17] = {0};
  int edge_k = 0;
  bool second_wave2 = false;
  double fit_two = 1.0;
  double fit_narrow = 1.0;
  double tile_reuse_bytes = 0;
  double plan_ms = 0;
  int plan_threads = 1;
  qk_ctx* up_ctx = nullptr;
  int32_t* d_pairs = nullptr;
  int32_t* d_groups = nullptr;
  unsigned long long* d_seg = nullptr;
  unsigned long long seg_key[8] = {0};
};

struct QkSweepPolicy {
  int variant = 20;
  int wgs_per_cu = 2;
  bool wave_path = true;
  bool wave2_ring = true;
  bool wave2_path = true;
  bool small_path = true;
  int fused_path = 1;
  int fused_split = 1;
  int fused_wgs = 0;
  bool deterministic = false;
  int merge_mode = 2;
  bool fused_dual = true;
  bool gang = false;
};

struct QkSetShape {
  int max_pad = 0, precision = 64, n_sites = 0;
};

struct QkSweepRun {
  int kernel = QK_KERNEL_NONE;
  long long grid = 0;
  size_t lds = 0;
  long long first = 0, count = 0;
  int nq = 1, gang_n = 0;
  bool gang2 = false;
};

struct QkSweepChoice {
  int rc = QK_OK;
  char err[192] = {};
  int n_runs = 0;
  QkSweepRun run[2];
  long long launched_grid = 0;
  long long x_plane = 0, t_plane = 0;
  int turn_ints = 0;
  size_t scratch_bytes = 0;
  bool interleaved = false;
  bool fused_images = false;
  int queues = 1;
  bool tails = false;
};

static inline QkSweepChoice qk_choose_sweep(const QkSweepPolicy& p, const qk_plan& plan, const QkSetShape& x, const QkSetShape& y, const int num_cus) {
  QkSweepChoice ch;
  const long long np = (long long)plan.pairs.size() / 2;
  const bool f32 = x.precision == 32, quad = plan.quad, det = p.deterministic;
  const int n = x.n_sites, max_pad = std::max(x.max_pad, y.max_pad);
  const bool grouped = p.variant == 14 && !f32 && !quad, duo = p.variant == 16 && !f32 && !quad;
  const long long chains = quad ? 4 : (duo ? 2 : 1);
  const long long units = quad ? np / 4 : grouped ? (long long)plan.groups.size() / 2 : (duo ? (np + 1) / 2 : np);
  ch.x_plane = (grouped ? GMAX : 1) * (long long)x.max_pad * y.max_pad, ch.t_plane = 2 * ch.x_plane;
  ch.turn_ints = det ? (y.max_pad / QK_TILE) * (x.max_pad / QK_TILE) : 0;
  const size_t lds_meta = 16 + 256 + (size_t)n * (48 + 16) + (det ? (size_t)(2 * ch.turn_ints + 2) * sizeof(int) : 0);
  const bool can_one = max_pad <= QKF_XCAP_ONE / QK_TILE && (size_t)QKF_XCAP_ONE * 16 + lds_meta <= 160 * 1024;
  const bool can_two = max_pad <= QKF_XCAP_TWO / QK_TILE && (size_t)QKF_XCAP_TWO * 16 + lds_meta <= 160 * 1024 / QKF_TWO_WGS;
  const bool fused = p.variant == 20 && !f32 && !quad && p.fused_path != 0 && max_pad > (p.fused_path >= 2 ? 16 : 32) && (can_one || can_two);
  const bool second_class = fused && plan.n_first > 0 && plan.n_first < np;
  const bool split = second_class && can_one && can_two && p.fused_wgs == 0 && p.fused_split != 0 && !plan.second_wave2 && (p.fused_split == 2 || np >= 100ll * num_cus);
  const bool mixed = second_class && plan.second_wave2 && p.wave2_path && p.wave2_ring;
  const bool fused_two = fused && can_two && !split && (!can_one || p.fused_wgs == 2 || (p.fused_wgs == 0 && plan.fit_two >= 0.75 && plan.fit_narrow >= 0.5));
  const bool dual = fused && !fused_two && p.fused_dual;
  const int wgs = fused ? (fused_two ? QKF_TWO_WGS : 1) : p.wgs_per_cu;
  const long long grid = std::min(units, (long long)wgs * num_cus);
  ch.scratch_bytes = (size_t)(split ? 2ll * num_cus : grid) * (size_t)chains * 2 * (size_t)(ch.x_plane + ch.t_plane) * sizeof(double);
  const size_t site_meta = 16 + (size_t)(4 * (n + 1) + 2) * sizeof(int) + (size_t)2 * n * sizeof(long long);
  const size_t lds_ring = 3 * 16 * 1024 + site_meta;
  const size_t esz = f32 ? sizeof(float) : sizeof(double), lds_small = (size_t)(3 * 2 * (64 / esz) * 64 + 6 * 32 * 32) * esz + site_meta;
  if (lds_ring > 80 * 1024)
    return ch.rc = QK_EINVAL, snprintf(ch.err, sizeof ch.err, "qk_gram_values: %d sites need %zu bytes of LDS per workgroup (limit 80 KiB for 2 workgroups per CU)", n, lds_ring), ch;
  QkSweepRun& r = ch.run[0];
  ch.n_runs = 1, ch.launched_grid = r.grid = grid, r.count = np;
  if (quad) {
#ifdef QK_LAB
    r.kernel = QK_KERNEL_LAB;
#else
    ch.rc = QK_EINVAL, snprintf(ch.err, sizeof ch.err, "qk_gram_values: QK_PLAN_QUADS plans are swept by an experimental kernel that only libqklab.so contains");
#endif
  } else if (p.variant == 20 && p.wave_path && !f32 && max_pad <= 16) {
    r.kernel = QK_KERNEL_WAVE, ch.launched_grid = r.grid = std::min(np, 16ll * num_cus);
  } else if (!fused && p.variant == 20 && p.wave2_path && (!f32 || p.wave2_ring) && max_pad <= 32) {
    r.kernel = (f32 || p.wave2_ring) ? QK_KERNEL_WAVE2 : QK_KERNEL_WAVE2_PLAIN, ch.launched_grid = r.grid = std::min(np, 8ll * num_cus);
    ch.interleaved = ch.tails = true, ch.queues = plan.nq > 1 ? 8 : 1, r.nq = plan.nq;
  } else if (!fused && p.variant == 20 && p.small_path && max_pad <= 32 && lds_small <= 80 * 1024) {
    r.kernel = QK_KERNEL_SMALL, r.lds = lds_small;
  } else if (fused) {
    ch.interleaved = ch.fused_images = ch.tails = true, ch.queues = plan.nq > 1 ? 8 : 1, r.nq = plan.nq;
    r.kernel = fused_two ? (det ? QK_KERNEL_FUSED2_DET : QK_KERNEL_FUSED2) : dual ? (det ? QK_KERNEL_FUSED_DUAL_DET : QK_KERNEL_FUSED_DUAL) : (det ? QK_KERNEL_FUSED1_DET : QK_KERNEL_FUSED1);
    r.lds = (size_t)(fused_two ? QKF_XCAP_TWO : QKF_XCAP_ONE) * 16 + lds_meta;
    auto gang_of = [&](const long long g) { return p.gang && plan.nq > 1 && g >= 16 && g % 8 == 0 ? (int)(g / 8) : 0; };
    if (split || mixed) {
      QkSweepRun& r2 = ch.run[1];
      ch.n_runs = 2;
      r.count = plan.n_first, r2.first = plan.n_first, r2.count = np - plan.n_first;
      r.nq = r2.nq = plan.nq > 1 ? 8 : plan.nq;
      r.grid = std::min(r.count, (long long)wgs * num_cus);
      if (split) {
        r2.kernel = det ? QK_KERNEL_FUSED2_DET : QK_KERNEL_FUSED2, r2.grid = std::min(r2.count, (long long)QKF_TWO_WGS * num_cus);
        r2.lds = (size_t)QKF_XCAP_TWO * 16 + lds_meta, r2.gang_n = gang_of(r2.grid), r2.gang2 = true;
      } else {
        r2.kernel = QK_KERNEL_WAVE2, r2.grid = std::min(r2.count, 8ll * num_cus);
      }
    }
    r.gang_n = gang_of(r.grid);
  } else if (f32 || p.variant == 20) {
    r.kernel = QK_KERNEL_RING, r.lds = lds_ring;
  } else {
#ifdef QK_LAB
    r.kernel = QK_KERNEL_LAB;
#else
    ch.rc = QK_EINVAL, snprintf(ch.err, sizeof ch.err, "qk_gram_values: no kernel for this call");
#endif
  }
  return ch;
}
```

qml-cutensornet_amd/csrc/qkgram.hip:

```cpp
#include "qk_host.h"
#include "qk_ring.h"
#include "qk_fused.h"
#ifndef QKF_QUAD
#define QKF_QUAD 0
#endif
#if QKF_QUAD
#include "qk_quad.h"
#endif

#include <algorithm>
#include <cmath>
#include <cstdarg>
#include <cstdio>
#include <cstdlib>
#include <cstring>
#include <new>
#include <numeric>
#include <string>
#include <vector>

static thread_local std::string g_err;

int qk_fail(int code, const char* fmt, ...) {
  char buf[512];
  va_list ap;
  va_start(ap, fmt);
  vsnprintf(buf, sizeof buf, fmt, ap);
  va_end(ap);
  g_err = buf;
  return code;
}
#define fail qk_fail

extern "C" const char* qk_last_error(void) { return g_err.c_str(); }

#include <atomic>
uint64_t qk_next_uid() {
  static std::atomic<uint64_t> next{1};
  return next.fetch_add(1);
}

#include <dlfcn.h>
namespace {
struct Roctx {
  int (*push)(const char*) = nullptr;
  int (*pop)() = nullptr;
};
Roctx& roctx() {
  static Roctx r = [] {
    Roctx x;
    const char* e = std::getenv("QK_ROCTX");
    const char* pre = std::getenv("LD_PRELOAD");
    const bool attached = std::getenv("ROCP_TOOL_LIBRARIES") || (pre && std::strstr(pre, "rocprofiler"));
    if (e ? std::atoi(e) == 0 : !attached) return x;
    void* h = nullptr;
    for (const char* name : {"librocprofiler-sdk-roctx.so.1", "librocprofiler-sdk-roctx.so", "libroctx64.so.4", "libroctx64.so"})
      if ((h = dlopen(name, RTLD_NOW | RTLD_GLOBAL))) break;
    if (!h) return x;
    x.push = reinterpret_cast<int (*)(const char*)>(dlsym(h, "roctxRangePushA"));
    x.pop = reinterpret_cast<int (*)()>(dlsym(h, "roctxRangePop"));
    if (!x.push || !x.pop) x.push = nullptr, x.pop = nullptr;
    return x;
  }();
  return r;
}
}
extern "C" int qk_range_push(const char* name) {
  Roctx& r = roctx();
  return (r.push && name) ? r.push(name) : 0;
}
extern "C" int qk_range_pop(void) {
  Roctx& r = roctx();
  return r.pop ? r.pop() : 0;
}

static inline int pad16(int x) { return (x + TILE - 1) / TILE * TILE; }

extern "C" int64_t qk_pack_state_size(int32_t n_sites, const int32_t* bond_dims) {
  int64_t tot = 0;
  for (int k = 0; k < n_sites; ++k) tot += 2ll * pad16(bond_dims[k]) * 2 * pad16(bond_dims[k + 1]);
  return tot;
}

extern "C" int qk_pack_state(int32_t n_sites, const int32_t* bond_dims, const double* const* site_tensors,
                             int32_t layout, double* out, int64_t* site_offsets) {
  if (n_sites <= 0 || !bond_dims || !site_tensors || !out) return fail(QK_EINVAL, "qk_pack_state: null argument");
  if (layout != QK_LAYOUT_LPR && layout != QK_LAYOUT_LRP) return fail(QK_EINVAL, "qk_pack_state: unknown layout %d", layout);
  if (bond_dims[0] != 1 || bond_dims[n_sites] != 1) return fail(QK_EINVAL, "qk_pack_state: boundary bonds must be 1");
  int64_t off = 0;
  for (int k = 0; k < n_sites; ++k) {
    const int cl = bond_dims[k], cr = bond_dims[k + 1];
    if (cl <= 0 || cr <= 0) return fail(QK_EINVAL, "qk_pack_state: non-positive bond at site %d", k);
    const int pl = pad16(cl), pr = pad16(cr);
    const int64_t plane = (int64_t)pl * 2 * pr;
    double* re = out + off;
    double* im = re + plane;
    std::memset(re, 0, sizeof(double) * 2 * plane);
    const double* src = site_tensors[k];
    if (!src) return fail(QK_EINVAL, "qk_pack_state: null tensor at site %d", k);
    for (int l = 0; l < cl; ++l)
      for (int p = 0; p < 2; ++p)
        for (int r = 0; r < cr; ++r) {
          const int64_t s = (layout == QK_LAYOUT_LPR) ? (((int64_t)l * 2 + p) * cr + r) : (((int64_t)l * cr + r) * 2 + p);
          const int64_t d = ((int64_t)l * 2 + p) * pr + r;
          re[d] = src[2 * s];
          im[d] = src[2 * s + 1];
        }
    if (site_offsets) site_offsets[k] = off;
    off += 2 * plane;
  }
  return QK_OK;
}

#ifndef QKF_ONE_NW
#define QKF_ONE_NW 12
#define QKF_ONE_S 2
#define QKF_ONE_WPS 3
#endif
#ifndef QKF_TWO_NW
#define QKF_TWO_NW 8
#define QKF_TWO_S 1
#define QKF_TWO_WPS 4
#endif
#define QKF_KERNEL_ONE qk_sweep_fused_kernel<QKF_ONE_NW, QKF_ONE_S, QKF_XCAP_ONE, QKF_ONE_WPS>
#define QKF_KERNEL_TWO qk_sweep_fused_kernel<QKF_TWO_NW, QKF_TWO_S, QKF_XCAP_TWO, QKF_TWO_WPS>
#ifndef QKF_DUAL_NW
#define QKF_DUAL_NW 12
#define QKF_DUAL_WPS 3
#endif
#define QKF_KERNEL_DUAL qk_sweep_fused_dual_kernel<QKF_DUAL_NW, QKF_XCAP_ONE, QKF_DUAL_WPS>
#define QKF_KERNEL_ONE_DET qk_sweep_fused_kernel<QKF_ONE_NW, QKF_ONE_S, QKF_XCAP_ONE, QKF_ONE_WPS, true>
#define QKF_KERNEL_TWO_DET qk_sweep_fused_kernel<QKF_TWO_NW, QKF_TWO_S, QKF_XCAP_TWO, QKF_TWO_WPS, true>
#define QKF_KERNEL_DUAL_DET qk_sweep_fused_dual_kernel<QKF_DUAL_NW, QKF_XCAP_ONE, QKF_DUAL_WPS, true>
#if QKF_QUAD
#define QKF_QUAD_NW 8
#define QKF_KERNEL_QUAD qk_sweep_fused_quad_kernel<QKF_QUAD_NW, QKF_XCAP_ONE, 2>
#endif

extern "C" int qk_plan_destroy(qk_plan* plan) {
  if (!plan) return QK_OK;
  if (plan->d_pairs) (void)hipFree(plan->d_pairs);
  if (plan->d_groups) (void)hipFree(plan->d_groups);
  if (plan->d_seg) (void)hipFree(plan->d_seg);
  delete plan;
  return QK_OK;
}
__global__ void qk_convert_f32_kernel(const double* __restrict__ src, float* __restrict__ dst, const long long n) {
  for (long long e = (long long)blockIdx.x * blockDim.x + threadIdx.x; e < n; e += (long long)gridDim.x * blockDim.x) dst[e] = (float)src[e];
}

__global__ void qk_scatter_kernel(const int32_t* __restrict__ pairs, const double* __restrict__ vals, long long n,
                                  double* __restrict__ K, long long ld, int mirror) {
  const long long t = (long long)blockIdx.x * blockDim.x + threadIdx.x;
  if (t >= n) return;
  const int i = pairs[2 * t], j = pairs[2 * t + 1];
  if (i < 0) return;
  const double v = vals[t];
  K[(long long)j * ld + i] = v;
  if (mirror) K[(long long)i * ld + j] = v;
}

typedef double qk_v2d __attribute__((ext_vector_type(2)));

__device__ __forceinline__ void qk_ctile(QkfTile& t, const qk_v2d* __restrict__ P, const long pk, const long pm, const qk_v2d* __restrict__ Q, const long qk, const long qn, const int ks4,
                                         const int q, const int j) {
  const qk_v2d* pp = P + q * pk + j * pm;
  const qk_v2d* qq = Q + q * qk + j * qn;
  v4d p1 = {0, 0, 0, 0}, p2 = {0, 0, 0, 0}, p3 = {0, 0, 0, 0};
  qk_v2d a = pp[0], b = qq[0];
  for (int ks = 0; ks < ks4; ++ks) {
    const qk_v2d a0 = a, b0 = b;
    if (ks + 1 < ks4) a = pp[(long)4 * (ks + 1) * pk], b = qq[(long)4 * (ks + 1) * qk];
    qkf_kstep<false>(p1, p2, p3, a0.x, a0.y, b0.x, b0.y);
  }
  t.re = p1 - p2, t.im = p3 - p1 - p2;
}

__global__ __launch_bounds__(256) void qk_edge_kernel(const qk_v2d* __restrict__ il, const int32_t* __restrict__ dims, const int32_t* __restrict__ dtrue, const int64_t* __restrict__ offs,
                                                      const int n_sites, const int k, const long long n_states, qk_v2d* __restrict__ edge, const long long* __restrict__ edge_offs,
                                                      qk_v2d* __restrict__ tmp, const long long tmp_elems) {
  qk_v2d* const t0 = tmp + (long long)blockIdx.x * 2 * tmp_elems;
  qk_v2d* const t1 = t0 + tmp_elems;
  const int n1 = n_sites + 1, lane = threadIdx.x & 63, wave = threadIdx.x >> 6, nw = blockDim.x >> 6, j = lane & 15, q = lane >> 4;
  for (long long t = blockIdx.x; t < 2 * n_states; t += gridDim.x) {
    const long long st = t >> 1;
    const int right = (int)(t & 1);
    const int32_t* d = dims + st * n1;
    const int32_t* dt = dtrue + st * n1;
    qk_v2d* const dst = edge + edge_offs[t];
    for (int e = threadIdx.x; e < 256; e += blockDim.x) t0[e] = (qk_v2d){e == 0 ? 1.0 : 0.0, 0.0};
    __syncthreads();
    const qk_v2d* in = t0;
    for (int jj = 0; jj < k; ++jj) {
      const int site = right ? n_sites - 1 - jj : jj;
      const int lp = d[site], rp = d[site + 1];
      const qk_v2d* const A = il + (offs[st * n_sites + site] >> 1);
      const int ld_in = right ? rp : lp, ld_out = right ? lp : rp, rows_in = 1 << jj;
      const int ks4 = ((right ? dt[site + 1] : dt[site]) + 3) >> 2;
      qk_v2d* const out = (jj + 1 == k) ? dst : (in == t0 ? t1 : t0);
      const int nts = (rows_in + 15) >> 4, ntc = ld_out >> 4;
      for (int u = wave; u < nts * 2 * ntc; u += nw) {
        const int tc = u % ntc, pp = (u / ntc) & 1, ts = u / (2 * ntc);
        QkfTile T;
        if (right) qk_ctile(T, in + (long)(ts * 16) * ld_in, 1, ld_in, A + (long)pp * rp + (long)(tc * 16) * 2 * rp, 1, 2 * rp, ks4, q, j);
        else qk_ctile(T, in + (long)(ts * 16) * ld_in, 1, ld_in, A + (long)pp * rp + tc * 16, 2 * rp, 1, ks4, q, j);
#pragma unroll
        for (int r = 0; r < 4; ++r) {
          const int s_ = ts * 16 + q + 4 * r;
          if (s_ < rows_in) out[(long)(2 * s_ + pp) * ld_out + tc * 16 + j] = (qk_v2d){T.re[r], T.im[r]};
        }
      }
      __syncthreads();
      in = out;
    }
  }
}

__global__ __launch_bounds__(256, 2) void qk_merge_kernel(const qk_v2d* __restrict__ il, const int32_t* __restrict__ dims, const int32_t* __restrict__ dtrue, const int64_t* __restrict__ offs,
                                                          const int n_sites, const int k, const int steps, const int stride, const int n_starts, const long long n_tasks, const long long* __restrict__ unit_start,
                                                          qk_v2d* __restrict__ out, const int64_t* __restrict__ out_offs) {
  const int n1 = n_sites + 1, lane = threadIdx.x & 63, wave = threadIdx.x >> 6, nw = blockDim.x >> 6, j = lane & 15, q = lane >> 4;
  const long long n_units = unit_start[n_tasks];
  for (long long u = (long long)blockIdx.x * nw + wave; u < n_units; u += (long long)gridDim.x * nw) {
    long long lo = 0, hi = n_tasks;
    while (hi - lo > 1) {
      const long long mid = (lo + hi) >> 1;
      if (unit_start[mid] <= u) lo = mid;
      else hi = mid;
    }
    const long long t = lo, st = t / steps;
    const int step = (int)(t - st * steps), s_ = k + stride * step, v = (int)(u - unit_start[t]);
    const int32_t* d = dims + st * n1;
    const int lp = d[s_], mp = d[s_ + 1], rp = d[s_ + 2], ntr = rp >> 4, tl = v / ntr, tr = v - tl * ntr;
    (void)lp;
    const int ks4 = (dtrue[st * n1 + s_ + 1] + 3) >> 2;
    const qk_v2d* const A1 = il + (offs[st * n_sites + s_] >> 1);
    const qk_v2d* const A2 = il + (offs[st * n_sites + s_ + 1] >> 1);
    const qk_v2d* pa = A1 + ((long)(tl * 16 + j) * 2) * mp + q;
    const qk_v2d* pb = A2 + ((long)q * 2) * rp + tr * 16 + j;
    v4d acc[4][3];
#pragma unroll
    for (int c = 0; c < 4; ++c)
#pragma unroll
      for (int e = 0; e < 3; ++e) acc[c][e] = (v4d){0, 0, 0, 0};
    qk_v2d a0 = pa[0], a1 = pa[mp], b0 = pb[0], b1 = pb[rp];
    for (int ks = 0; ks < ks4; ++ks) {
      const qk_v2d x0 = a0, x1 = a1, y0 = b0, y1 = b1;
      if (ks + 1 < ks4) {
        pa += 4, pb += (long)8 * rp;
        a0 = pa[0], a1 = pa[mp], b0 = pb[0], b1 = pb[rp];
      }
      qkf_kstep<false>(acc[0][0], acc[0][1], acc[0][2], x0.x, x0.y, y0.x, y0.y);
      qkf_kstep<false>(acc[1][0], acc[1][1], acc[1][2], x0.x, x0.y, y1.x, y1.y);
      qkf_kstep<false>(acc[2][0], acc[2][1], acc[2][2], x1.x, x1.y, y0.x, y0.y);
      qkf_kstep<false>(acc[3][0], acc[3][1], acc[3][2], x1.x, x1.y, y1.x, y1.y);
    }
    qk_v2d* const dst = out + (out_offs[st * n_starts + stride * step] >> 1);
#pragma unroll
    for (int c = 0; c < 4; ++c) {
      const v4d re = acc[c][0] - acc[c][1], im = acc[c][2] - acc[c][0] - acc[c][1];
#pragma unroll
      for (int r = 0; r < 4; ++r) dst[(long)(4 * (tl * 16 + q + 4 * r) + c) * rp + tr * 16 + j] = (qk_v2d){re[r], im[r]};
    }
  }
}

__global__ __launch_bounds__(256) void qk_segment_kernel(const int32_t* __restrict__ xdims, const int32_t* __restrict__ xtrue, const int32_t* __restrict__ ydims, const int32_t* __restrict__ ytrue,
                                                         const int n_sites, const int ek, const int32_t* __restrict__ pairs, const long long npairs, const QkSegRule rule, const int parities,
                                                         const bool greedy, unsigned long long* __restrict__ seg) {
  const long long p = (long long)blockIdx.x * blockDim.x + threadIdx.x;
  if (p >= npairs) return;
  const long long xo = (long long)pairs[2 * p] * (n_sites + 1), yo = (long long)pairs[2 * p + 1] * (n_sites + 1);
  const QkSegMask m = qk_segment_chain(xdims + xo, xtrue + xo, ydims + yo, ytrue + yo, n_sites, ek, rule, parities, greedy);
  seg[2 * p] = m.w[0], seg[2 * p + 1] = m.w[1];
}

#ifdef QK_LAB
__global__ void qk_lab_fold_kernel(const int64_t* __restrict__ src, int64_t* __restrict__ dst, const long long n, const long long win) {
  for (long long i = blockIdx.x * (long long)blockDim.x + threadIdx.x; i < n; i += (long long)gridDim.x * blockDim.x) dst[i] = (src[i] % win) & ~1ll;
}
#endif
__global__ void qk_selftest_f32_kernel(const float* __restrict__ P, const float* __restrict__ Q, float* __restrict__ C) {
  const int lane = threadIdx.x & 63, j = lane & 15, q = lane >> 4;
  v4f acc = {0, 0, 0, 0};
  for (int ks = 0; ks < 4; ++ks) acc = __builtin_amdgcn_mfma_f32_16x16x4f32(P[(4 * ks + q) * 16 + j], Q[(4 * ks + q) * 16 + j], acc, 0, 0, 0);
  for (int r = 0; r < 4; ++r) C[(4 * q + r) * 16 + j] = acc[r];
}

__global__ void qk_selftest_kernel(const double* __restrict__ P, const double* __restrict__ Q, double* __restrict__ C) {
  const int lane = threadIdx.x & 63, j = lane & 15, q = lane >> 4;
  v4d acc = {0, 0, 0, 0};
  for (int ks = 0; ks < 4; ++ks) acc = __builtin_amdgcn_mfma_f64_16x16x4f64(P[(4 * ks + q) * 16 + j], Q[(4 * ks + q) * 16 + j], acc, 0, 0, 0);
  for (int r = 0; r < 4; ++r) C[(q + 4 * r) * 16 + j] = acc[r];
}

extern "C" int qk_device_count(void) {
  int n = 0;
  if (hipGetDeviceCount(&n) != hipSuccess) return 0;
  return n;
}

static int ctx_init(qk_ctx* c, int device_id, int num_cus);

extern "C" int qk_ctx_create(int device_id, qk_ctx** out) {
  if (!out) return fail(QK_EINVAL, "qk_ctx_create: null out");
  int n = 0;
  hipError_t e = hipGetDeviceCount(&n);
  if (e != hipSuccess || n <= 0)
    return fail(QK_EDEVICE, "qk_ctx_create: no HIP device available (%s); this engine has no CPU fallback",
                e == hipSuccess ? "device count is 0" : hipGetErrorString(e));
  if (device_id < 0 || device_id >= n) return fail(QK_EINVAL, "qk_ctx_create: device %d out of range [0,%d)", device_id, n);
  HIP_TRY(hipSetDevice(device_id));
  hipDeviceProp_t prop;
  HIP_TRY(hipGetDeviceProperties(&prop, device_id));
  if (std::strncmp(prop.gcnArchName, "gfx950", 6) != 0)
    return fail(QK_EDEVICE, "qk_ctx_create: device %d is %s; this library is built for gfx950 only", device_id, prop.gcnArchName);
  qk_ctx* c = new (std::nothrow) qk_ctx;
  if (!c) return fail(QK_ENOMEM, "qk_ctx_create: out of memory");
  const int rc_init = ctx_init(c, device_id, prop.multiProcessorCount);
  if (rc_init != QK_OK) {
    qk_ctx_destroy(c);
    return rc_init;
  }
  *out = c;
  return QK_OK;
}

static int ctx_init(qk_ctx* c, int device_id, int num_cus) {
  c->device = device_id;
  c->num_cus = num_cus;
  HIP_TRY(hipStreamCreateWithFlags(&c->own_stream, hipStreamNonBlocking));
  c->stream = c->own_stream;
  HIP_TRY(hipEventCreate(&c->ev0));
  HIP_TRY(hipEventCreate(&c->ev1));
  HIP_TRY(hipEventCreate(&c->ev_mid));
  HIP_TRY(hipEventCreate(&c->ev_d));
  HIP_TRY(c->counter.alloc((QK_NQ_MAX * QK_QSTRIDE + 8 + 2 * 8 * QK_QSTRIDE) * sizeof(unsigned long long)));
  HIP_TRY(c->prof.alloc(8 * sizeof(unsigned long long)));
  HIP_TRY(hipMemset(c->prof.get(), 0, 8 * sizeof(unsigned long long)));
  for (const void* k : {(const void*)qk_sweep_ring_kernel<float>, (const void*)qk_sweep_ring_kernel<double>, (const void*)qk_sweep_small_kernel<double>, (const void*)qk_sweep_small_kernel<float>})
    HIP_TRY(hipFuncSetAttribute(k, hipFuncAttributeMaxDynamicSharedMemorySize, 80 * 1024));
  for (const void* k : {(const void*)QKF_KERNEL_ONE, (const void*)QKF_KERNEL_DUAL, (const void*)QKF_KERNEL_ONE_DET, (const void*)QKF_KERNEL_DUAL_DET})
    HIP_TRY(hipFuncSetAttribute(k, hipFuncAttributeMaxDynamicSharedMemorySize, 160 * 1024));
  for (const void* k : {(const void*)QKF_KERNEL_TWO, (const void*)QKF_KERNEL_TWO_DET}) HIP_TRY(hipFuncSetAttribute(k, hipFuncAttributeMaxDynamicSharedMemorySize, 160 * 1024 / QKF_TWO_WGS));
#if QKF_QUAD
  HIP_TRY(hipFuncSetAttribute(reinterpret_cast<const void*>(QKF_KERNEL_QUAD), hipFuncAttributeMaxDynamicSharedMemorySize, 160 * 1024));
#endif
  QkSweepPolicy& p = c->policy;
#ifdef QK_LAB
  {
    const int rc = qk_lab_init(c);
    if (rc != QK_OK) return rc;
  }
  if (const char* v = std::getenv("QK_VARIANT")) p.variant = std::atoi(v);
#endif
  if (const char* v = std::getenv("QK_SMALL")) p.small_path = std::atoi(v) != 0;
  if (const char* v = std::getenv("QK_WAVE")) p.wave_path = std::atoi(v) != 0;
  if (const char* v = std::getenv("QK_WAVE2")) p.wave2_path = std::atoi(v) != 0, p.wave2_ring = std::atoi(v) != 2;
  if (const char* v = std::getenv("QK_FUSED")) p.fused_path = std::atoi(v);
  if (const char* v = std::getenv("QK_MERGE")) p.merge_mode = std::max(0, std::min(2, std::atoi(v)));
  if (const char* v = std::getenv("QK_DETERMINISTIC"))
    if (std::atoi(v) != 0) p.deterministic = true;
  if (const char* v = std::getenv("QK_FUSED_SPLIT")) p.fused_split = std::max(0, std::min(2, std::atoi(v)));
  if (const char* v = std::getenv("QK_FUSED_WGS")) p.fused_wgs = std::max(0, std::min(2, std::atoi(v)));
  if (const char* v = std::getenv("QK_WGS_PER_CU")) p.wgs_per_cu = std::max(1, std::min(4, std::atoi(v)));
  return QK_OK;
}

extern "C" int qk_ctx_destroy(qk_ctx* c) {
  if (!c) return QK_OK;
  (void)hipSetDevice(c->device);
  if (c->stream) (void)hipStreamSynchronize(c->stream);
  if (c->ev0) (void)hipEventDestroy(c->ev0);
  if (c->ev1) (void)hipEventDestroy(c->ev1);
  if (c->ev_mid) (void)hipEventDestroy(c->ev_mid);
  if (c->ev_d) (void)hipEventDestroy(c->ev_d);
  if (c->own_stream) (void)hipStreamDestroy(c->own_stream);
  delete c;
  return QK_OK;
}

extern "C" int qk_ctx_trim(qk_ctx* c) {
  if (!c) return fail(QK_EINVAL, "qk_ctx_trim: null context");
  HIP_TRY(hipSetDevice(c->device));
  HIP_TRY(hipStreamSynchronize(c->stream));
  for (QkGrowBuf* b : {&c->scratch, &c->build_arena, &c->build_work, &c->derive_tmp, &c->local_scratch}) b->reset();
  return QK_OK;
}

extern "C" int qk_ctx_set_stream(qk_ctx* c, void* s) {
  if (!c) return fail(QK_EINVAL, "qk_ctx_set_stream: null context");
  c->stream = reinterpret_cast<hipStream_t>(s);
  return QK_OK;
}

extern "C" int qk_ctx_use_own_stream(qk_ctx* c) {
  if (!c) return fail(QK_EINVAL, "qk_ctx_use_own_stream: null context");
  c->stream = c->own_stream;
  return QK_OK;
}

extern "C" int qk_ctx_synchronize(qk_ctx* c) {
  if (!c) return fail(QK_EINVAL, "qk_ctx_synchronize: null context");
  HIP_TRY(hipSetDevice(c->device));
  HIP_TRY(hipStreamSynchronize(c->stream));
  return QK_OK;
}

int qk_mps_set_alloc(qk_ctx* c, int n_states, int n_sites, int64_t data_bytes, int precision, qk_mps_set** out, const char* who) {
  qk_mps_set* m = new (std::nothrow) qk_mps_set;
  if (!m) return fail(QK_ENOMEM, "%s: out of memory", who);
  m->ctx = c, m->n_states = n_states, m->n_sites = n_sites, m->precision = precision, m->bytes = data_bytes;
  const size_t nd = (size_t)n_states * (n_sites + 1), no = (size_t)n_states * n_sites;
  hipError_t e = m->d_data.alloc((size_t)data_bytes);
  if (e == hipSuccess) e = m->d_dims.alloc(nd * sizeof(int32_t));
  if (e == hipSuccess) e = m->d_true.alloc(nd * sizeof(int32_t));
  if (e == hipSuccess) e = m->d_offs.alloc(no * sizeof(int64_t));
  if (e != hipSuccess) {
    qk_mps_set_destroy(m);
    return fail(QK_EDEVICE, "%s: hipMalloc of a set of %lld bytes and its tables failed: %s", who, (long long)data_bytes, hipGetErrorString(e));
  }
  *out = m;
  return QK_OK;
}

extern "C" int qk_mps_set_create(qk_ctx* c, int32_t n_states, int32_t n_sites, const int32_t* bond_dims,
                                 const double* const* site_tensors, int32_t layout, qk_mps_set** out) {
  if (!c || !out || !bond_dims || !site_tensors) return fail(QK_EINVAL, "qk_mps_set_create: null argument");
  if (n_states <= 0 || n_sites <= 0) return fail(QK_EINVAL, "qk_mps_set_create: empty set (%d states, %d sites)", n_states, n_sites);
  QkRangeGuard range_("qk:upload");
  HIP_TRY(hipSetDevice(c->device));
  const int stride = n_sites + 1;
  std::vector<int32_t> pad((size_t)n_states * stride);
  std::vector<int64_t> offs((size_t)n_states * n_sites);
  std::vector<int64_t> state_off(n_states + 1, 0);
  int max_pad = 0;
  for (int s = 0; s < n_states; ++s) {
    const int32_t* d = bond_dims + (size_t)s * stride;
    if (d[0] != 1 || d[n_sites] != 1) return fail(QK_EINVAL, "qk_mps_set_create: state %d: boundary bonds must be 1", s);
    for (int k = 0; k <= n_sites; ++k) {
      if (d[k] <= 0) return fail(QK_EINVAL, "qk_mps_set_create: state %d: non-positive bond %d", s, k);
      pad[(size_t)s * stride + k] = pad16(d[k]);
      max_pad = std::max(max_pad, pad16(d[k]));
    }
    state_off[s + 1] = state_off[s] + qk_pack_state_size(n_sites, d);
  }
  qk_mps_set* m = nullptr;
  int rc = qk_mps_set_alloc(c, n_states, n_sites, state_off[n_states] * (int64_t)sizeof(double), 64, &m, "qk_mps_set_create");
  if (rc != QK_OK) return rc;
  m->max_pad = max_pad;
  m->dims_true.assign(bond_dims, bond_dims + (size_t)n_states * stride);
  hipError_t e = hipSuccess;
  std::vector<double> stage;
  std::vector<int64_t> so(n_sites);
  for (int s = 0; s < n_states; ++s) {
    const int64_t sz = state_off[s + 1] - state_off[s];
    stage.resize((size_t)sz);
    rc = qk_pack_state(n_sites, bond_dims + (size_t)s * stride, site_tensors + (size_t)s * n_sites, layout, stage.data(), so.data());
    if (rc != QK_OK) {
      qk_mps_set_destroy(m);
      return rc;
    }
    for (int k = 0; k < n_sites; ++k) offs[(size_t)s * n_sites + k] = state_off[s] + so[k];
    e = hipMemcpy(m->d_data.get<double>() + state_off[s], stage.data(), (size_t)sz * sizeof(double), hipMemcpyHostToDevice);
    if (e != hipSuccess) {
      qk_mps_set_destroy(m);
      return fail(QK_EDEVICE, "qk_mps_set_create: upload failed: %s", hipGetErrorString(e));
    }
  }
  e = hipMemcpy(m->d_dims.get(), pad.data(), pad.size() * sizeof(int32_t), hipMemcpyHostToDevice);
  if (e == hipSuccess) e = hipMemcpy(m->d_true.get(), bond_dims, pad.size() * sizeof(int32_t), hipMemcpyHostToDevice);
  if (e == hipSuccess) e = hipMemcpy(m->d_offs.get(), offs.data(), offs.size() * sizeof(int64_t), hipMemcpyHostToDevice);
  if (e != hipSuccess) {
    qk_mps_set_destroy(m);
    return fail(QK_EDEVICE, "qk_mps_set_create: table upload failed: %s", hipGetErrorString(e));
  }
  *out = m;
  return QK_OK;
}

extern "C" int qk_mps_set_destroy(qk_mps_set* m) {
  if (!m) return QK_OK;
  (void)hipSetDevice(m->ctx->device);
  (void)hipStreamSynchronize(m->ctx->stream);
  delete m;
  return QK_OK;
}

extern "C" int qk_mps_set_info(const qk_mps_set* m, int32_t* n_states, int32_t* n_sites, int32_t* max_padded_bond, int64_t* device_bytes) {
  if (!m) return fail(QK_EINVAL, "qk_mps_set_info: null set");
  if (n_states) *n_states = m->n_states;
  if (n_sites) *n_sites = m->n_sites;
  if (max_padded_bond) *max_padded_bond = m->max_pad;
  if (device_bytes) *device_bytes = m->bytes * (m->d_il ? 2 : 1) + m->edge_bytes + m->mg_bytes;
  return QK_OK;
}

extern "C" int qk_mps_set_precision(const qk_mps_set* m) { return m ? m->precision : 0; }

extern "C" int qk_mps_set_image(const qk_mps_set* m, int64_t* n_doubles, const double** planes_dev, int32_t* dims_true, int64_t* offsets) {
  if (!m) return fail(QK_EINVAL, "qk_mps_set_image: null set");
  if (m->precision != 64) return fail(QK_EINVAL, "qk_mps_set_image: only fp64 sets are exchanged");
  if (n_doubles) *n_doubles = m->bytes / (int64_t)sizeof(double);
  if (planes_dev) *planes_dev = m->d_data.get<double>();
  if (dims_true) std::memcpy(dims_true, m->dims_true.data(), m->dims_true.size() * sizeof(int32_t));
  if (offsets) {
    HIP_TRY(hipSetDevice(m->ctx->device));
    HIP_TRY(hipStreamSynchronize(m->ctx->stream));
    HIP_TRY(hipMemcpy(offsets, m->d_offs.get<int64_t>(), (size_t)m->n_states * m->n_sites * sizeof(int64_t), hipMemcpyDeviceToHost));
  }
  return QK_OK;
}

extern "C" int qk_mps_set_copy_image(const qk_mps_set* m, double* dst, int64_t n_doubles) {
  if (!m || !dst) return fail(QK_EINVAL, "qk_mps_set_copy_image: null argument");
  if (m->precision != 64) return fail(QK_EINVAL, "qk_mps_set_copy_image: only fp64 sets are exchanged");
  if (n_doubles * (int64_t)sizeof(double) < m->bytes) return fail(QK_EINVAL, "qk_mps_set_copy_image: destination holds %lld doubles, the image has %lld", (long long)n_doubles, (long long)(m->bytes / 8));
  HIP_TRY(hipSetDevice(m->ctx->device));
  HIP_TRY(hipMemcpyAsync(dst, m->d_data.get<double>(), (size_t)m->bytes, hipMemcpyDefault, m->ctx->stream));
  HIP_TRY(hipStreamSynchronize(m->ctx->stream));
  return QK_OK;
}

extern "C" int qk_mps_set_from_packed(qk_ctx* c, int32_t n_states, int32_t n_sites, const int32_t* dims_true, const int64_t* offsets,
                                      const double* planes_dev, int64_t n_doubles, qk_mps_set** out) {
  if (!c || !out || !dims_true || !offsets || !planes_dev) return fail(QK_EINVAL, "qk_mps_set_from_packed: null argument");
  if (n_states <= 0 || n_sites <= 0 || n_doubles <= 0) return fail(QK_EINVAL, "qk_mps_set_from_packed: empty set");
  const int stride = n_sites + 1;
  std::vector<int32_t> pad((size_t)n_states * stride);
  int max_pad = 0;
  for (int s = 0; s < n_states; ++s) {
    const int32_t* d = dims_true + (size_t)s * stride;
    if (d[0] != 1 || d[n_sites] != 1) return fail(QK_EINVAL, "qk_mps_set_from_packed: state %d: boundary bonds must be 1", s);
    for (int k = 0; k <= n_sites; ++k) {
      if (d[k] <= 0) return fail(QK_EINVAL, "qk_mps_set_from_packed: state %d: non-positive bond %d", s, k);
      pad[(size_t)s * stride + k] = pad16(d[k]);
      max_pad = std::max(max_pad, pad16(d[k]));
    }
    for (int k = 0; k < n_sites; ++k) {
      const int64_t off = offsets[(size_t)s * n_sites + k], sz = 2ll * pad[(size_t)s * stride + k] * 2 * pad[(size_t)s * stride + k + 1];
      if (off < 0 || (off & 1) || off + sz > n_doubles) return fail(QK_EINVAL, "qk_mps_set_from_packed: state %d site %d: tensor [%lld, %lld) outside the %lld-double image", s, k, (long long)off, (long long)(off + sz), (long long)n_doubles);
    }
  }
  HIP_TRY(hipSetDevice(c->device));
  qk_mps_set* m = nullptr;
  const int rc = qk_mps_set_alloc(c, n_states, n_sites, n_doubles * (int64_t)sizeof(double), 64, &m, "qk_mps_set_from_packed");
  if (rc != QK_OK) return rc;
  m->max_pad = max_pad;
  m->dims_true.assign(dims_true, dims_true + (size_t)n_states * stride);
  hipError_t e = hipMemcpyAsync(m->d_data.get(), planes_dev, (size_t)m->bytes, hipMemcpyDefault, c->stream);
  if (e == hipSuccess) e = hipMemcpyAsync(m->d_dims.get(), pad.data(), pad.size() * sizeof(int32_t), hipMemcpyHostToDevice, c->stream);
  if (e == hipSuccess) e = hipMemcpyAsync(m->d_true.get(), dims_true, pad.size() * sizeof(int32_t), hipMemcpyHostToDevice, c->stream);
  if (e == hipSuccess) e = hipMemcpyAsync(m->d_offs.get(), offsets, (size_t)n_states * n_sites * sizeof(int64_t), hipMemcpyHostToDevice, c->stream);
  if (e == hipSuccess) e = hipStreamSynchronize(c->stream);
  if (e != hipSuccess) {
    qk_mps_set_destroy(m);
    return fail(QK_EDEVICE, "qk_mps_set_from_packed: %s", hipGetErrorString(e));
  }
  *out = m;
  return QK_OK;
}

extern "C" int qk_mps_set_to_f32(qk_ctx* c, const qk_mps_set* src, qk_mps_set** out) {
  if (!c || !src || !out) return fail(QK_EINVAL, "qk_mps_set_to_f32: null argument");
  if (src->ctx != c) return fail(QK_EINVAL, "qk_mps_set_to_f32: the set belongs to another context");
  if (src->precision != 64) return fail(QK_EINVAL, "qk_mps_set_to_f32: the source set is not fp64");
  HIP_TRY(hipSetDevice(c->device));
  const long long n = src->bytes / (long long)sizeof(double);
  qk_mps_set* m = nullptr;
  const int rc = qk_mps_set_alloc(c, src->n_states, src->n_sites, n * (long long)sizeof(float), 32, &m, "qk_mps_set_to_f32");
  if (rc != QK_OK) return rc;
  m->max_pad = src->max_pad;
  m->dims_true = src->dims_true;
  const size_t nd = (size_t)src->n_states * (src->n_sites + 1), no = (size_t)src->n_states * src->n_sites;
  hipError_t e = hipMemcpyAsync(m->d_dims.get(), src->d_dims.get(), nd * sizeof(int32_t), hipMemcpyDeviceToDevice, c->stream);
  if (e == hipSuccess) e = hipMemcpyAsync(m->d_true.get(), src->d_true.get(), nd * sizeof(int32_t), hipMemcpyDeviceToDevice, c->stream);
  if (e == hipSuccess) e = hipMemcpyAsync(m->d_offs.get(), src->d_offs.get(), no * sizeof(int64_t), hipMemcpyDeviceToDevice, c->stream);
  if (e == hipSuccess) {
    qk_convert_f32_kernel<<<dim3(4 * c->num_cus), dim3(256), 0, c->stream>>>(src->d_data.get<double>(), m->d_data.get<float>(), n);
    e = hipGetLastError();
  }
  if (e == hipSuccess) e = hipStreamSynchronize(c->stream);
  if (e != hipSuccess) {
    qk_mps_set_destroy(m);
    return fail(QK_EDEVICE, "qk_mps_set_to_f32: %s", hipGetErrorString(e));
  }
  *out = m;
  return QK_OK;
}

static int ensure_interleaved(qk_ctx* c, qk_mps_set* m) {
  if (m->d_il) return QK_OK;
  QkDevBuf il;
  HIP_TRY(il.alloc((size_t)m->bytes));
  const long long nt = (long long)m->n_states * m->n_sites;
  const dim3 grid((unsigned)std::min<long long>(nt, 64ll * c->num_cus));
  if (m->precision == 64) qk_interleave_kernel<double><<<grid, dim3(256), 0, c->stream>>>(m->d_data.get<double>(), il.get<double>(), m->d_dims.get<int32_t>(), m->d_offs.get<int64_t>(), m->n_sites, nt);
  else
    qk_interleave_kernel<float><<<grid, dim3(256), 0, c->stream>>>(m->d_data.get<float>(), il.get<float>(), m->d_dims.get<int32_t>(), m->d_offs.get<int64_t>(), m->n_sites, nt);
  HIP_TRY(hipGetLastError());
  m->d_il = std::move(il);
  return QK_OK;
}

static int ensure_edges(qk_ctx* c, qk_mps_set* m, const int k) {
  if (k <= 0 || (m->d_edge && m->edge_k == k)) return QK_OK;
  if (m->d_edge || m->d_edge_offs) HIP_TRY(hipStreamSynchronize(c->stream));
  m->d_edge.reset(), m->d_edge_offs.reset(), m->edge_k = 0, m->edge_bytes = 0;
  const int n = m->n_sites, stride = n + 1;
  std::vector<long long>& offs = m->h_edge_offs;
  offs.assign((size_t)m->n_states * 2, 0);
  long long total = 0;
  int maxld = 16;
  for (int s_ = 0; s_ < m->n_states; ++s_) {
    const int32_t* d = m->dims_true.data() + (size_t)s_ * stride;
    offs[(size_t)2 * s_] = total;
    total += (long long)(1 << k) * pad16(d[k]);
    offs[(size_t)2 * s_ + 1] = total;
    total += (long long)(1 << k) * pad16(d[n - k]);
    for (int jj = 0; jj <= k; ++jj) maxld = std::max(maxld, std::max(pad16(d[jj]), pad16(d[n - jj])));
  }
  const long long tmp_elems = (long long)std::max(1 << (k - 1), 16) * maxld;
  const int grid = (int)std::min<long long>(2ll * m->n_states, 4ll * c->num_cus);
  const size_t tmp_bytes = (size_t)grid * 2 * tmp_elems * 2 * sizeof(double);
  if (tmp_bytes > c->derive_tmp.bytes) HIP_TRY(hipStreamSynchronize(c->stream));
  HIP_TRY(c->derive_tmp.ensure(tmp_bytes));
  QkDevBuf eb, ob;
  HIP_TRY(eb.alloc((size_t)total * 2 * sizeof(double)));
  HIP_TRY(ob.alloc(offs.size() * sizeof(long long)));
  HIP_TRY(hipMemcpyAsync(ob.get(), offs.data(), offs.size() * sizeof(long long), hipMemcpyHostToDevice, c->stream));
  qk_edge_kernel<<<dim3(grid), dim3(256), 0, c->stream>>>(m->d_il.get<qk_v2d>(), m->d_dims.get<int32_t>(), m->d_true.get<int32_t>(), m->d_offs.get<int64_t>(), n, k, m->n_states, eb.get<qk_v2d>(),
                                                          ob.get<long long>(), c->derive_tmp.get<qk_v2d>(), tmp_elems);
  HIP_TRY(hipGetLastError());
  m->d_edge = std::move(eb), m->d_edge_offs = std::move(ob);
  m->edge_k = k, m->edge_bytes = total * 2 * (long long)sizeof(double);
  return QK_OK;
}

static void free_merged(qk_mps_set* m) {
  m->d_mg.reset(), m->d_mg_offs.reset(), m->d_mg_units.reset(), m->mg_k = -1, m->mg_steps = 0, m->mg_stride = 0, m->mg_bytes = 0;
}

static int ensure_merged(qk_ctx* c, qk_mps_set* m, const int k, int stride) {
  if (m->mg_full_failed) stride = 2;
  if (m->d_mg && m->mg_k == k && m->mg_stride <= stride) return QK_OK;
  if (m->d_mg) HIP_TRY(hipStreamSynchronize(c->stream));
  free_merged(m);
  const int n = m->n_sites, n1 = n + 1, starts = n - 2 * k - 1;
  if (starts < 1) return fail(QK_EINVAL, "ensure_merged: a chain of %d sites", n - 2 * k);
  std::vector<int64_t>& mo = m->h_mg_offs;
  std::vector<long long>& us = m->h_mg_units;
  QkDevBuf ib, ob, ub;
  int steps = 0;
  long long total = 0, units = 0;
  for (;; stride = 2) {
    steps = (starts + stride - 1) / stride;
    mo.assign((size_t)m->n_states * starts, 0);
    us.assign((size_t)m->n_states * steps + 1, 0);
    total = units = 0;
    for (int s_ = 0; s_ < m->n_states; ++s_) {
      const int32_t* d = m->dims_true.data() + (size_t)s_ * n1;
      for (int t = 0; t < steps; ++t) {
        const long long lp = pad16(d[k + stride * t]), rp = pad16(d[k + stride * t + 2]);
        mo[(size_t)s_ * starts + stride * t] = 2 * total;
        us[(size_t)s_ * steps + t] = units;
        total += 4ll * lp * rp;
        units += (lp / 16) * (rp / 16);
      }
    }
    us.back() = units;
    if (ib.alloc((size_t)total * 2 * sizeof(double)) == hipSuccess) break;
    (void)hipGetLastError();
    if (stride == 2) return fail(QK_EDEVICE, "ensure_merged: no device memory for %lld bytes of merged steps", total * 2 * (long long)sizeof(double));
    m->mg_full_failed = true;
  }
  HIP_TRY(ob.alloc(mo.size() * sizeof(int64_t)));
  HIP_TRY(ub.alloc(us.size() * sizeof(long long)));
  HIP_TRY(hipMemcpyAsync(ob.get(), mo.data(), mo.size() * sizeof(int64_t), hipMemcpyHostToDevice, c->stream));
  HIP_TRY(hipMemcpyAsync(ub.get(), us.data(), us.size() * sizeof(long long), hipMemcpyHostToDevice, c->stream));
  const long long tasks = (long long)m->n_states * steps;
  const unsigned grid = (unsigned)std::min<long long>((units + 3) / 4, 4ll * c->num_cus);
  qk_merge_kernel<<<dim3(grid), dim3(256), 0, c->stream>>>(m->d_il.get<qk_v2d>(), m->d_dims.get<int32_t>(), m->d_true.get<int32_t>(), m->d_offs.get<int64_t>(), n, k, steps, stride, starts, tasks,
                                                          ub.get<long long>(), ib.get<qk_v2d>(), ob.get<int64_t>());
  HIP_TRY(hipGetLastError());
  m->d_mg = std::move(ib), m->d_mg_offs = std::move(ob), m->d_mg_units = std::move(ub);
  m->mg_k = k, m->mg_steps = starts, m->mg_stride = stride, m->mg_bytes = total * 2 * (long long)sizeof(double);
  return QK_OK;
}

static int ensure_plan_uploaded(qk_ctx* c, qk_plan* p) {
  if (p->d_pairs && p->up_ctx == c) return QK_OK;
  if (p->d_pairs) (void)hipFree(p->d_pairs);
  if (p->d_groups) (void)hipFree(p->d_groups);
  if (p->d_seg) (void)hipFree(p->d_seg);
  p->d_pairs = nullptr, p->d_groups = nullptr, p->d_seg = nullptr, p->up_ctx = nullptr;
  if (p->pairs.empty()) return QK_OK;
  QkDevBuf pairs, groups;
  HIP_TRY(pairs.alloc(p->pairs.size() * sizeof(int32_t)));
  HIP_TRY(hipMemcpy(pairs.get(), p->pairs.data(), p->pairs.size() * sizeof(int32_t), hipMemcpyHostToDevice));
  HIP_TRY(groups.alloc(p->groups.size() * sizeof(int32_t)));
  HIP_TRY(hipMemcpy(groups.get(), p->groups.data(), p->groups.size() * sizeof(int32_t), hipMemcpyHostToDevice));
  p->d_pairs = static_cast<int32_t*>(pairs.release()), p->d_groups = static_cast<int32_t*>(groups.release()), p->up_ctx = c;
  return QK_OK;
}

static int derive_fused_images(qk_ctx* c, const qk_mps_set* xs, const qk_mps_set* ys, const qk_plan* plan, const int merge_mode, SweepArgs& a) {
  int ek = plan->edge_k, rc = QK_OK;
  if (ek > 0) {
    if (xs->edge_k > 0 && (ys == xs || ys->edge_k == 0 || ys->edge_k == xs->edge_k)) ek = xs->edge_k;
    else if (xs->edge_k == 0 && ys->edge_k > 0) ek = ys->edge_k;
    for (const qk_mps_set* m : {xs, ys})
      if ((rc = ensure_edges(c, const_cast<qk_mps_set*>(m), ek)) != QK_OK) return rc;
    a.xedge = xs->d_edge.get<double>(), a.xedge_offs = xs->d_edge_offs.get<long long>(), a.yedge = ys->d_edge.get<double>(), a.yedge_offs = ys->d_edge_offs.get<long long>(), a.edge_k = ek;
  }
  if (merge_mode > 0 && xs->n_sites - 2 * ek >= 2) {
    for (const qk_mps_set* m : {xs, ys})
      if ((rc = ensure_merged(c, const_cast<qk_mps_set*>(m), ek, merge_mode >= 2 ? 1 : 2)) != QK_OK) return rc;
    a.xmg = xs->d_mg.get<double>(), a.xmg_offs = xs->d_mg_offs.get<int64_t>(), a.ymg = ys->d_mg.get<double>(), a.ymg_offs = ys->d_mg_offs.get<int64_t>(), a.merge_steps = xs->mg_steps;
  }
#ifdef QK_LAB
  if (const char* v = std::getenv("QK_DEBUG_ALIAS")) {
    const long long win = std::atoll(v);
    if (win > 0) {
      auto fold = [&](const int64_t* src, const long long n) -> const int64_t* {
        QkDevBuf buf;
        if (buf.alloc((size_t)n * sizeof(int64_t)) != hipSuccess) return src;
        int64_t* dst = static_cast<int64_t*>(buf.release());
        qk_lab_fold_kernel<<<dim3(256), dim3(256), 0, c->stream>>>(src, dst, n, win);
        return dst;
      };
      a.xoffs = fold(a.xoffs, (long long)xs->n_states * xs->n_sites), a.yoffs = fold(a.yoffs, (long long)ys->n_states * ys->n_sites);
      if (a.merge_steps > 0)
        a.xmg_offs = fold(a.xmg_offs, (long long)xs->n_states * xs->mg_steps), a.ymg_offs = fold(a.ymg_offs, (long long)ys->n_states * ys->mg_steps);
    }
  }
#endif
  return QK_OK;
}

static QkSegRule seg_rule_of(const int kernel) {
  switch (kernel) {
    case QK_KERNEL_FUSED1: case QK_KERNEL_FUSED1_DET: return {QKF_XCAP_ONE, QKF_ONE_NW * QKF_ONE_S, false};
    case QK_KERNEL_FUSED2: case QK_KERNEL_FUSED2_DET: return {QKF_XCAP_TWO, QKF_TWO_NW * QKF_TWO_S, false};
#if QKF_QUAD
    case QK_KERNEL_FUSED_DUAL: return {QKF_XCAP_ONE, QKF_QUAD_NW, true};
#else
    case QK_KERNEL_FUSED_DUAL: return {QKF_XCAP_ONE, QKF_DUAL_NW, true};
#endif
    case QK_KERNEL_FUSED_DUAL_DET: return {QKF_XCAP_ONE, QKF_DUAL_NW, true};
    default: return {0, 0, false};
  }
}

static int ensure_segments(qk_ctx* c, const qk_mps_set* xs, const qk_mps_set* ys, qk_plan* plan, const QkSweepChoice& ch, const int merge_mode, SweepArgs& a) {
  const long long np = (long long)plan->pairs.size() / 2;
  const bool both = merge_mode >= 2 && xs->mg_stride == 1 && ys->mg_stride == 1;
  const unsigned long long key[8] = {1ull,
                                     xs->uid,
                                     ys->uid,
                                     (unsigned long long)a.edge_k,
                                     both ? 3ull : 1ull,
                                     merge_mode == 1 ? 1ull : 0ull,
                                     (unsigned long long)ch.run[0].kernel | ((unsigned long long)(ch.n_runs > 1 ? ch.run[1].kernel : 0) << 32),
                                     (unsigned long long)ch.run[0].count};
  if (plan->d_seg && std::equal(key, key + 8, plan->seg_key)) return a.seg = plan->d_seg, QK_OK;
  if (plan->d_seg) {
    HIP_TRY(hipStreamSynchronize(c->stream));
    (void)hipFree(plan->d_seg), plan->d_seg = nullptr;
  }
  QkDevBuf seg;
  HIP_TRY(seg.alloc((size_t)np * 2 * sizeof(unsigned long long)));
  unsigned long long* const d = seg.get<unsigned long long>();
  for (int i = 0; i < ch.n_runs; ++i) {
    const QkSweepRun& r = ch.run[i];
    const QkSegRule rule = seg_rule_of(r.kernel);
    if (r.count <= 0) continue;
    if (rule.cap == 0) {
      HIP_TRY(hipMemsetAsync(d + 2 * r.first, 0, (size_t)r.count * 2 * sizeof(unsigned long long), c->stream));
      continue;
    }
    qk_segment_kernel<<<dim3((unsigned)((r.count + 255) / 256)), dim3(256), 0, c->stream>>>(a.xdims, a.xtrue, a.ydims, a.ytrue, a.n_sites, a.edge_k, a.pairs + 2 * r.first, r.count, rule, both ? 3 : 1,
                                                                                            merge_mode == 1, d + 2 * r.first);
  }
  HIP_TRY(hipGetLastError());
  plan->d_seg = static_cast<unsigned long long*>(seg.release());
  std::copy(key, key + 8, plan->seg_key);
  a.seg = plan->d_seg;
  return QK_OK;
}

static int launch_sweep(const int kernel, const bool f32, const long long grid_, const size_t lds, const hipStream_t s, const SweepArgs& a) {
  const dim3 grid((unsigned)grid_);
  switch (kernel) {
    case QK_KERNEL_WAVE: qk_sweep_wave_kernel<0><<<grid, dim3(64), lds, s>>>(a); break;
    case QK_KERNEL_WAVE2: if (f32) qk_sweep_wave2_kernel<3, float><<<grid, dim3(64), lds, s>>>(a); else qk_sweep_wave2_kernel<3, double><<<grid, dim3(64), lds, s>>>(a); break;
    case QK_KERNEL_WAVE2_PLAIN: qk_sweep_wave2_kernel<0, double><<<grid, dim3(64), lds, s>>>(a); break;
    case QK_KERNEL_SMALL: if (f32) qk_sweep_small_kernel<float><<<grid, dim3(512), lds, s>>>(a); else qk_sweep_small_kernel<double><<<grid, dim3(512), lds, s>>>(a); break;
    case QK_KERNEL_RING: if (f32) qk_sweep_ring_kernel<float><<<grid, dim3(512), lds, s>>>(a); else qk_sweep_ring_kernel<double><<<grid, dim3(512), lds, s>>>(a); break;
    case QK_KERNEL_FUSED1: QKF_KERNEL_ONE<<<grid, dim3(64 * QKF_ONE_NW), lds, s>>>(a); break;
    case QK_KERNEL_FUSED1_DET: QKF_KERNEL_ONE_DET<<<grid, dim3(64 * QKF_ONE_NW), lds, s>>>(a); break;
    case QK_KERNEL_FUSED2: QKF_KERNEL_TWO<<<grid, dim3(64 * QKF_TWO_NW), lds, s>>>(a); break;
    case QK_KERNEL_FUSED2_DET: QKF_KERNEL_TWO_DET<<<grid, dim3(64 * QKF_TWO_NW), lds, s>>>(a); break;
#if QKF_QUAD
    case QK_KERNEL_FUSED_DUAL: QKF_KERNEL_QUAD<<<grid, dim3(64 * QKF_QUAD_NW), lds, s>>>(a); break;
#else
    case QK_KERNEL_FUSED_DUAL: QKF_KERNEL_DUAL<<<grid, dim3(64 * QKF_DUAL_NW), lds, s>>>(a); break;
#endif
    case QK_KERNEL_FUSED_DUAL_DET: QKF_KERNEL_DUAL_DET<<<grid, dim3(64 * QKF_DUAL_NW), lds, s>>>(a); break;
    default: return fail(QK_EINVAL, "qk_gram_values: no kernel for this call");
  }
  return QK_OK;
}

extern "C" int qk_gram_values(qk_ctx* c, const qk_mps_set* xs, const qk_mps_set* ys, const qk_plan* plan_c, double* values_dev, double* z_dev) {
  if (!c || !xs || !plan_c || !values_dev) return fail(QK_EINVAL, "qk_gram_values: null argument");
  qk_plan* plan = const_cast<qk_plan*>(plan_c);
  if (!ys) ys = xs;
  if (xs->ctx != c || ys->ctx != c) return fail(QK_EINVAL, "qk_gram_values: sets belong to another context");
  if (xs->n_sites != ys->n_sites || xs->n_sites != plan->n_sites) return fail(QK_EINVAL, "qk_gram_values: site counts differ (%d, %d, plan %d)", xs->n_sites, ys->n_sites, plan->n_sites);
  if (plan->nx != xs->n_states || plan->ny != ys->n_states) return fail(QK_EINVAL, "qk_gram_values: plan is for %dx%d states, sets hold %dx%d", plan->nx, plan->ny, xs->n_states, ys->n_states);
  QkRangeGuard range_("qk:sweep");
  HIP_TRY(hipSetDevice(c->device));
  const long long np = (long long)plan->pairs.size() / 2;
  c->last = plan->stats;
  c->split_pending = c->tail_pending = false;
  c->last.max_bond = std::max(xs->max_pad, ys->max_pad);
  c->last.kernel_ms = 0, c->last.grid = 0, c->last.kernel = QK_KERNEL_NONE, c->last.precision = xs->precision;
  if (np == 0) return QK_OK;
  int rc = ensure_plan_uploaded(c, plan);
  if (rc != QK_OK) return rc;
  if (xs->precision != ys->precision) return fail(QK_EINVAL, "qk_gram_values: the two sets differ in precision (fp%d, fp%d)", xs->precision, ys->precision);
  const bool f32 = (xs->precision == 32);
  if (f32) c->last.bytes *= 0.5;

  QkSweepPolicy pol = c->policy;
  if (const char* v = std::getenv("QK_FUSED_DUAL")) pol.fused_dual = std::atoi(v) != 0;
  if (const char* v = std::getenv("QK_GANG")) pol.gang = std::atoi(v) != 0;
  const QkSweepChoice ch = qk_choose_sweep(pol, *plan, {xs->max_pad, xs->precision, xs->n_sites}, {ys->max_pad, ys->precision, ys->n_sites}, c->num_cus);
  if (ch.rc != QK_OK) return fail(ch.rc, "%s", ch.err);
  c->last.queues = ch.queues, c->last.tail_frac = c->last.second_tail_frac = 0;
  if (ch.scratch_bytes > c->scratch.bytes) HIP_TRY(hipStreamSynchronize(c->stream));
  HIP_TRY(c->scratch.ensure(ch.scratch_bytes));
  SweepArgs a{};
  a.xdata = xs->d_data.get<double>(), a.xdims = xs->d_dims.get<int32_t>(), a.xtrue = xs->d_true.get<int32_t>(), a.xoffs = xs->d_offs.get<int64_t>();
  a.ydata = ys->d_data.get<double>(), a.ydims = ys->d_dims.get<int32_t>(), a.ytrue = ys->d_true.get<int32_t>(), a.yoffs = ys->d_offs.get<int64_t>();
  a.n_sites = xs->n_sites;
  a.pairs = plan->d_pairs, a.npairs = np;
  a.groups = plan->d_groups, a.ngroups = (long long)plan->groups.size() / 2;
  a.values = values_dev, a.z = z_dev;
  a.scratch = c->scratch.get<double>(), a.x_plane = ch.x_plane, a.t_plane = ch.t_plane, a.turn_ints = ch.turn_ints;
  unsigned long long* const counter = c->counter.get<unsigned long long>();
  a.counter = counter, a.prof = c->prof.get<unsigned long long>();
  for (int s_ = 0; s_ <= QK_NQ_MAX; ++s_) a.qstart[s_] = plan->nq > 1 ? plan->qstart[s_] : (s_ == 0 ? 0 : np);
  a.tail = counter + QK_NQ_MAX * QK_QSTRIDE, a.err = a.tail + 7, a.gang = a.tail + 8;
#ifdef QK_LAB
  if (const char* v = std::getenv("QK_DEBUG_FLAGS")) a.debug_flags = std::atoi(v);
  if (const char* v = std::getenv("QK_PRIO")) a.prio_mode = std::atoi(v);
#endif
  HIP_TRY(hipEventRecord(c->ev_d, c->stream));
  HIP_TRY(hipMemsetAsync(counter, 0, (QK_NQ_MAX * QK_QSTRIDE + 8 + 2 * 8 * QK_QSTRIDE) * sizeof(unsigned long long), c->stream));
  HIP_TRY(hipMemsetAsync(a.tail, 0xFF, 4 * sizeof(unsigned long long), c->stream));
  if (ch.interleaved) {
    for (const qk_mps_set* m : {xs, ys})
      if ((rc = ensure_interleaved(c, const_cast<qk_mps_set*>(m))) != QK_OK) return rc;
    a.xdata = xs->d_il.get<double>(), a.ydata = ys->d_il.get<double>();
  }
  if (ch.fused_images && (rc = derive_fused_images(c, xs, ys, plan, pol.merge_mode, a)) != QK_OK) return rc;
  if (a.merge_steps > 0 && (rc = ensure_segments(c, xs, ys, plan, ch, pol.merge_mode, a)) != QK_OK) return rc;
  HIP_TRY(hipEventRecord(c->ev0, c->stream));
  for (int i = 0; i < ch.n_runs; ++i) {
    const QkSweepRun& r = ch.run[i];
    SweepArgs ar = a;
    ar.npairs = r.count, ar.nq = r.nq, ar.gang_n = r.gang_n;
    if (i == 1) {
      HIP_TRY(hipEventRecord(c->ev_mid, c->stream));
      ar.pairs = a.pairs + 2 * r.first, ar.values = a.values + r.first, ar.z = a.z ? a.z + 2 * r.first : nullptr, ar.seg = a.seg ? a.seg + 2 * r.first : nullptr;
      ar.counter = counter + 8 * QK_QSTRIDE, ar.tail = a.tail + 2;
      if (plan->nq > 1)
        for (int s_ = 0; s_ <= 8; ++s_) ar.qstart[s_] = plan->qstart[8 + s_] - r.first;
      if (r.gang2) ar.gang = a.gang + 8 * QK_QSTRIDE;
      c->last.second_pairs = plan->second.pairs, c->last.second_flops = plan->second.flops, c->last.second_padded_flops = plan->second.padded_flops;
      c->last.second_bytes = plan->second.bytes, c->last.second_kernel = r.kernel;
      c->split_pending = true;
    }
#ifdef QK_LAB
    if (r.kernel == QK_KERNEL_LAB) rc = plan->quad ? qk_lab_launch_quad(c, ar, (int)r.grid, xs->n_sites, f32) : qk_lab_launch(c, pol.variant, ar, (int)r.grid, xs->n_sites);
    else
#endif
      rc = launch_sweep(r.kernel, f32, r.grid, r.lds, c->stream, ar);
    if (rc != QK_OK) return rc;
  }
  HIP_TRY(hipGetLastError());
  HIP_TRY(hipEventRecord(c->ev1, c->stream));
  c->ev_pending = true;
  c->last.kernel = ch.run[0].kernel, c->last.grid = (int)ch.launched_grid;
  c->tail_pending = ch.tails;
  return QK_OK;
}

extern "C" int qk_gram_values_host(qk_ctx* c, const qk_mps_set* xs, const qk_mps_set* ys, const qk_plan* plan, double* values_host, double* z_host) {
  if (!c || !plan || !values_host) return fail(QK_EINVAL, "qk_gram_values_host: null argument");
  const int64_t np = qk_plan_num_pairs(plan);
  if (np == 0) return QK_OK;
  HIP_TRY(hipSetDevice(c->device));
  QkDevBuf vals, z;
  HIP_TRY(vals.alloc((size_t)np * sizeof(double)));
  if (z_host) HIP_TRY(z.alloc((size_t)np * 2 * sizeof(double)));
  const int rc = qk_gram_values(c, xs, ys, plan, vals.get<double>(), z.get<double>());
  if (rc != QK_OK) return rc;
  HIP_TRY(hipMemcpyAsync(values_host, vals.get(), (size_t)np * sizeof(double), hipMemcpyDeviceToHost, c->stream));
  if (z_host) HIP_TRY(hipMemcpyAsync(z_host, z.get(), (size_t)np * 2 * sizeof(double), hipMemcpyDeviceToHost, c->stream));
  HIP_TRY(hipStreamSynchronize(c->stream));
  return QK_OK;
}

extern "C" int qk_scatter(qk_ctx* c, const int32_t* pairs_dev, const double* values_dev, int64_t n, double* k_dev, int64_t ld, int32_t mirror) {
  if (!c || !pairs_dev || !values_dev || !k_dev) return fail(QK_EINVAL, "qk_scatter: null argument");
  if (n <= 0) return QK_OK;
  QkRangeGuard range_("qk:scatter");
  HIP_TRY(hipSetDevice(c->device));
  const int bs = 256;
  hipLaunchKernelGGL(qk_scatter_kernel, dim3((unsigned)((n + bs - 1) / bs)), dim3(bs), 0, c->stream, pairs_dev, values_dev, (long long)n, k_dev, (long long)ld, (int)mirror);
  HIP_TRY(hipGetLastError());
  return QK_OK;
}

extern "C" const char* qk_kernel_name(int32_t kernel, int32_t precision) {
  const bool f32 = precision == 32;
  switch (kernel) {
    case QK_KERNEL_WAVE: return "qk_sweep_wave_kernel<0>";
    case QK_KERNEL_SMALL: return f32 ? "qk_sweep_small_kernel<float>" : "qk_sweep_small_kernel<double>";
    case QK_KERNEL_FUSED1: return "qk_sweep_fused_kernel<12, 2, 8192, 3, false>";
    case QK_KERNEL_FUSED2: return "qk_sweep_fused_kernel<8, 1, 4608, 4, false>";
    case QK_KERNEL_FUSED1_DET: return "qk_sweep_fused_kernel<12, 2, 8192, 3, true>";
    case QK_KERNEL_FUSED2_DET: return "qk_sweep_fused_kernel<8, 1, 4608, 4, true>";
    case QK_KERNEL_FUSED_DUAL_DET: return "qk_sweep_fused_dual_kernel<12, 8192, 3, true>";
    case QK_KERNEL_RING: return f32 ? "qk_sweep_ring_kernel<float>" : "qk_sweep_ring_kernel<double>";
    case QK_KERNEL_WAVE2: return precision == 32 ? "qk_sweep_wave2_kernel<3, float>" : "qk_sweep_wave2_kernel<3, double>";
    case QK_KERNEL_WAVE2_PLAIN: return "qk_sweep_wave2_kernel<0, double>";
    case QK_KERNEL_FUSED_DUAL: return "qk_sweep_fused_dual_kernel<12, 8192, 3, false>";
    case QK_KERNEL_LAB: return "(lab kernel)";
    default: return "(none)";
  }
}
#ifndef QKF_EXPERIMENT
static_assert(QKF_ONE_NW == 12 && QKF_ONE_S == 2 && QKF_ONE_WPS == 3 && QKF_TWO_NW == 8 && QKF_TWO_S == 1 && QKF_TWO_WPS == 4 && QKF_XCAP_ONE == 8192 && QKF_XCAP_TWO == 4608,
              "qk_kernel_name spells the fused sweep's template arguments");
#endif

extern "C" int qk_get_stats(qk_ctx* c, qk_stats* out) {
  if (!c || !out) return fail(QK_EINVAL, "qk_get_stats: null argument");
  if (c->ev_pending) {
    HIP_TRY(hipSetDevice(c->device));
    HIP_TRY(hipEventSynchronize(c->ev1));
    float ms = 0;
    HIP_TRY(hipEventElapsedTime(&ms, c->ev0, c->ev1));
    c->last.kernel_ms = ms;
    HIP_TRY(hipEventElapsedTime(&ms, c->ev_d, c->ev0));
    c->last.derive_ms = ms;
    if (c->tail_pending) {
      unsigned long long t[8];
      HIP_TRY(hipMemcpy(t, c->counter.get<unsigned long long>() + QK_NQ_MAX * QK_QSTRIDE, sizeof t, hipMemcpyDeviceToHost));
      auto frac = [](const unsigned long long start, const unsigned long long first_exit, const unsigned long long last_exit) {
        return (last_exit > start && first_exit <= last_exit && first_exit >= start) ? (double)(last_exit - first_exit) / (double)(last_exit - start) : 0.0;
      };
      if (t[7] != 0) return fail(QK_EDEVICE, "qk_get_stats: the ordered accumulation of the last sweep ran out of patience (a bug: please report); its results are not valid");
      c->last.tail_frac = frac(t[0], t[1], t[4]);
      if (c->split_pending) c->last.second_tail_frac = frac(t[2], t[3], t[6]);
      c->tail_pending = false;
    }
    if (c->split_pending) {
      HIP_TRY(hipEventElapsedTime(&ms, c->ev_mid, c->ev1));
      c->last.second_ms = ms;
      c->split_pending = false;
    }
    c->ev_pending = false;
#ifdef QKF_PROF
    {
      unsigned long long pf[8];
      HIP_TRY(hipMemcpy(pf, c->prof.get(), sizeof pf, hipMemcpyDeviceToHost));
      HIP_TRY(hipMemset(c->prof.get(), 0, sizeof pf));
      const double tot = pf[7] > 0 ? (double)pf[7] : 1.0;
      fprintf(stderr, "[qkf_prof] pair set-up %.3f  step set-up %.3f  phase1 %.3f  wait1 %.3f  phase2 %.3f  wait2 %.3f  tail %.3f  (of %.3e wave cycles)\n", pf[0] / tot, pf[1] / tot, pf[2] / tot,
              pf[3] / tot, pf[4] / tot, pf[5] / tot, pf[6] / tot, tot);
    }
#endif
  }
  *out = c->last;
  return QK_OK;
}

static int plan_for_sets(const qk_mps_set* xs, const qk_mps_set* ys, qk_plan** plan) {
  const bool sym = (ys == nullptr || ys == xs);
  return qk_plan_create(xs->n_sites, xs->n_states, xs->dims_true.data(), sym ? xs->n_states : ys->n_states,
                        sym ? nullptr : ys->dims_true.data(), sym ? (QK_PLAN_SYMMETRIC | QK_PLAN_ORIENT) : 0u, 1, 0, 0, plan);
}

struct PlanGuard {
  qk_plan* p = nullptr;
  ~PlanGuard() { qk_plan_destroy(p); }
};

extern "C" int qk_gram_host(qk_ctx* c, const qk_mps_set* xs, const qk_mps_set* ys, double* out, int64_t ld) {
  if (!c || !xs || !out) return fail(QK_EINVAL, "qk_gram_host: null argument");
  const bool sym = (ys == nullptr || ys == xs);
  const int nx = xs->n_states, ny = sym ? nx : ys->n_states;
  if (ld < nx) return fail(QK_EINVAL, "qk_gram_host: ld %lld < %d columns", (long long)ld, nx);
  PlanGuard plan;
  int rc = plan_for_sets(xs, ys, &plan.p);
  if (rc != QK_OK) return rc;
  const int64_t np = qk_plan_num_pairs(plan.p);
  QkDevBuf vals, k;
  HIP_TRY(hipSetDevice(c->device));
  HIP_TRY(vals.alloc((size_t)np * sizeof(double)));
  HIP_TRY(k.alloc((size_t)ny * nx * sizeof(double)));
  HIP_TRY(hipMemsetAsync(k.get(), 0, (size_t)ny * nx * sizeof(double), c->stream));
  rc = qk_gram_values(c, xs, ys, plan.p, vals.get<double>(), nullptr);
  if (rc == QK_OK) rc = qk_scatter(c, plan.p->d_pairs, vals.get<double>(), np, k.get<double>(), nx, sym ? 1 : 0);
  if (rc != QK_OK) return rc;
  HIP_TRY(hipMemcpy2DAsync(out, (size_t)ld * sizeof(double), k.get(), (size_t)nx * sizeof(double), (size_t)nx * sizeof(double), (size_t)ny, hipMemcpyDeviceToHost, c->stream));
  HIP_TRY(hipStreamSynchronize(c->stream));
  return QK_OK;
}

extern "C" int qk_overlaps_host(qk_ctx* c, const qk_mps_set* xs, const qk_mps_set* ys, double* out) {
  if (!c || !xs || !out) return fail(QK_EINVAL, "qk_overlaps_host: null argument");
  if (!ys) ys = xs;
  const int nx = xs->n_states, ny = ys->n_states;
  PlanGuard plan;
  int rc = qk_plan_create(xs->n_sites, nx, xs->dims_true.data(), ny, ys->dims_true.data(), 0u, 1, 0, 16, &plan.p);
  if (rc != QK_OK) return rc;
  const int64_t np = qk_plan_num_pairs(plan.p);
  QkDevBuf vals, zd;
  HIP_TRY(hipSetDevice(c->device));
  HIP_TRY(vals.alloc((size_t)np * sizeof(double)));
  HIP_TRY(zd.alloc((size_t)np * 2 * sizeof(double)));
  rc = qk_gram_values(c, xs, ys, plan.p, vals.get<double>(), zd.get<double>());
  if (rc != QK_OK) return rc;
  std::vector<double> z((size_t)np * 2);
  HIP_TRY(hipMemcpyAsync(z.data(), zd.get(), z.size() * sizeof(double), hipMemcpyDeviceToHost, c->stream));
  HIP_TRY(hipStreamSynchronize(c->stream));
  const int32_t* pr = qk_plan_pairs(plan.p);
  for (int64_t t = 0; t < np; ++t) {
    const int64_t o = ((int64_t)pr[2 * t + 1] * nx + pr[2 * t]) * 2;
    out[o] = z[2 * t], out[o + 1] = z[2 * t + 1];
  }
  return QK_OK;
}

extern "C" int qk_selftest_mfma(qk_ctx* c) {
  if (!c) return fail(QK_EINVAL, "qk_selftest_mfma: null context");
  HIP_TRY(hipSetDevice(c->device));
  double hp[256], hq[256], hc[256], ref[256];
  for (int k = 0; k < 16; ++k)
    for (int m = 0; m < 16; ++m) {
      hp[k * 16 + m] = 1.0 + 0.25 * k - 0.5 * m + 0.125 * ((k * 7 + m * 3) % 5);
      hq[k * 16 + m] = -2.0 + 0.5 * k + 0.75 * m - 0.25 * ((k * 5 + m * 11) % 7);
    }
  for (int m = 0; m < 16; ++m)
    for (int n = 0; n < 16; ++n) {
      double s = 0;
      for (int k = 0; k < 16; ++k) s += hp[k * 16 + m] * hq[k * 16 + n];
      ref[m * 16 + n] = s;
    }
  QkDevBuf bp, bq, bc;
  HIP_TRY(bp.alloc(sizeof hp));
  HIP_TRY(bq.alloc(sizeof hq));
  HIP_TRY(bc.alloc(sizeof hc));
  double *dp = bp.get<double>(), *dq = bq.get<double>(), *dc = bc.get<double>();
  HIP_TRY(hipMemcpy(dp, hp, sizeof hp, hipMemcpyHostToDevice));
  HIP_TRY(hipMemcpy(dq, hq, sizeof hq, hipMemcpyHostToDevice));
  hipLaunchKernelGGL(qk_selftest_kernel, dim3(1), dim3(64), 0, c->stream, dp, dq, dc);
  HIP_TRY(hipGetLastError());
  HIP_TRY(hipStreamSynchronize(c->stream));
  HIP_TRY(hipMemcpy(hc, dc, sizeof hc, hipMemcpyDeviceToHost));
  double worst = 0;
  for (int e = 0; e < 256; ++e) worst = std::max(worst, std::fabs(hc[e] - ref[e]));
  if (worst > 1e-9) return fail(QK_EDEVICE, "qk_selftest_mfma: f64 MFMA fragment map mismatch (max abs error %.3g)", worst);
  float fp[256], fq[256], fc[256];
  for (int e = 0; e < 256; ++e) fp[e] = (float)hp[e], fq[e] = (float)hq[e];
  QkDevBuf be, bf, bg;
  HIP_TRY(be.alloc(sizeof fp));
  HIP_TRY(bf.alloc(sizeof fq));
  HIP_TRY(bg.alloc(sizeof fc));
  float *ep = be.get<float>(), *eq = bf.get<float>(), *ec = bg.get<float>();
  HIP_TRY(hipMemcpy(ep, fp, sizeof fp, hipMemcpyHostToDevice));
  HIP_TRY(hipMemcpy(eq, fq, sizeof fq, hipMemcpyHostToDevice));
  hipLaunchKernelGGL(qk_selftest_f32_kernel, dim3(1), dim3(64), 0, c->stream, ep, eq, ec);
  HIP_TRY(hipGetLastError());
  HIP_TRY(hipStreamSynchronize(c->stream));
  HIP_TRY(hipMemcpy(fc, ec, sizeof fc, hipMemcpyDeviceToHost));
  worst = 0;
  for (int e = 0; e < 256; ++e) worst = std::max(worst, std::fabs((double)fc[e] - ref[e]));
  if (worst > 1e-3) return fail(QK_EDEVICE, "qk_selftest_mfma: f32 MFMA fragment map mismatch (max abs error %.3g)", worst);
  return QK_OK;
}
```

Before: 753,800.

## Add per-step contraction orientation choice with switch steps to segment planner

```diff
diff --git a/qml-cutensornet_amd/csrc/qk_fused.h b/qml-cutensornet_amd/csrc/qk_fused.h
--- a/qml-cutensornet_amd/csrc/qk_fused.h
+++ b/qml-cutensornet_amd/csrc/qk_fused.h
@@ -250,6 +250,56 @@
   }
 }
 
+template <bool HAS1>
+__device__ __forceinline__ void qkf_p2_switch(const QkfTile& t0, const QkfTile& t1, v2d (&fr)[4], const bool primed, QkfStream cur, const int lim, const int nn, const int kmax,
+                                              __attribute__((address_space(3))) double* d, const int d1off, const QkfStream nxt) {
+  if (!primed) qkf_load4(fr, cur);
+  const v4d dm0 = t0.im - t0.re, ng0 = -t0.re - t0.im, dm1 = HAS1 ? t1.im - t1.re : dm0, ng1 = HAS1 ? -t1.re - t1.im : ng0;
+#pragma unroll 1
+  for (int tn = 0; tn < nn; ++tn) {
+    v4d p1 = {0, 0, 0, 0}, p2 = {0, 0, 0, 0}, p3 = {0, 0, 0, 0}, r1 = {0, 0, 0, 0}, r2 = {0, 0, 0, 0}, r3 = {0, 0, 0, 0};
+    const bool fin = tn + 1 == nn;
+    const v2d* const rb = fin ? nxt.base : cur.base;
+    const int rs = fin ? nxt.step : cur.step, rl = fin ? nxt.lim : lim;
+    cur.off = fin ? nxt.off : cur.off + TILE;
+    QKF_PRIO_LO();
+#pragma unroll
+    for (int i = 0; i < 4; ++i) {
+      if (i < kmax) {
+        const double sa = QKF_SUM(fr[i].x, fr[i].y);
+        p1 = __builtin_amdgcn_mfma_f64_16x16x4f64(sa, t0.re[i], p1, 0, 0, 0);
+        p2 = __builtin_amdgcn_mfma_f64_16x16x4f64(fr[i].y, dm0[i], p2, 0, 0, 0);
+        p3 = __builtin_amdgcn_mfma_f64_16x16x4f64(fr[i].x, ng0[i], p3, 0, 0, 0);
+        if (HAS1) {
+          r1 = __builtin_amdgcn_mfma_f64_16x16x4f64(sa, t1.re[i], r1, 0, 0, 0);
+          r2 = __builtin_amdgcn_mfma_f64_16x16x4f64(fr[i].y, dm1[i], r2, 0, 0, 0);
+          r3 = __builtin_amdgcn_mfma_f64_16x16x4f64(fr[i].x, ng1[i], r3, 0, 0, 0);
+        }
+      }
+      fr[i] = qkf_ldg_a(qkf_kbase(rb, rs, i, rl), cur.off);
+      __builtin_amdgcn_sched_barrier(0);
+    }
+    QKF_PRIO_HI();
+    {
+      const v4d re = p1 + p2, im = p1 + p3;
+#pragma unroll
+      for (int r = 0; r < 4; ++r) {
+        __hip_atomic_fetch_add(d + r * 2 * QKF_XSTEP, re[r], __ATOMIC_RELAXED, __HIP_MEMORY_SCOPE_WORKGROUP);
+        __hip_atomic_fetch_add(d + r * 2 * QKF_XSTEP + 1, im[r], __ATOMIC_RELAXED, __HIP_MEMORY_SCOPE_WORKGROUP);
+      }
+    }
+    if (HAS1) {
+      const v4d re = r1 + r2, im = r1 + r3;
+#pragma unroll
+      for (int r = 0; r < 4; ++r) {
+        __hip_atomic_fetch_add(d + d1off + r * 2 * QKF_XSTEP, re[r], __ATOMIC_RELAXED, __HIP_MEMORY_SCOPE_WORKGROUP);
+        __hip_atomic_fetch_add(d + d1off + r * 2 * QKF_XSTEP + 1, im[r], __ATOMIC_RELAXED, __HIP_MEMORY_SCOPE_WORKGROUP);
+      }
+    }
+    d += 2 * QKF_XBLOCK;
+  }
+}
+
 template <int S>
 __device__ __forceinline__ void qkf_rotate(QkfTile (&T)[S], const int L) {
   if constexpr (S >= 2) {
@@ -363,9 +413,9 @@
 }
 template <int NW, bool PAIRS, int SETS>
 __device__ __forceinline__ void qkf_edge_prefix(const SweepArgs& g, const int xi, const int yj, const int a, const int b, lds_v2d* const xl, v2d* const xg, const bool to_global, const int wave,
-                                                const int q, const int j) {
-  const v2d* const Lx = reinterpret_cast<const v2d*>(g.xedge) + qkf_uniform(g.xedge_offs[2 * (long long)xi]);
-  const v2d* const Ly = reinterpret_cast<const v2d*>(g.yedge) + qkf_uniform(g.yedge_offs[2 * (long long)yj]);
+                                                const int q, const int j, const bool swap = false) {
+  const v2d* const Lx = reinterpret_cast<const v2d*>(swap ? g.yedge : g.xedge) + qkf_uniform((swap ? g.yedge_offs : g.xedge_offs)[2 * (long long)xi]);
+  const v2d* const Ly = reinterpret_cast<const v2d*>(swap ? g.xedge : g.yedge) + qkf_uniform((swap ? g.xedge_offs : g.yedge_offs)[2 * (long long)yj]);
   const int mt = a / TILE, nt = b / TILE, ng = (1 << g.edge_k) >> 4, inv = qk_recip20(mt), units = PAIRS ? qk_edge_units(mt, nt, NW) : mt * nt;
   for (int u = wave; u < units; u += NW) {
     const QkEdgeUnit un = qkf_edge_unit_of<NW, PAIRS>(u, mt, nt, inv);
@@ -395,9 +445,9 @@
 
 template <int NW, bool PAIRS, int SETS>
 __device__ __forceinline__ void qkf_edge_suffix(const SweepArgs& g, const int xi, const int yj, const int a, const int b, const lds_v2d* const xl, const v2d* const xg, const bool from_global,
-                                                __attribute__((address_space(3))) double* zacc, const int wave, const int q, const int j) {
-  const v2d* const Rx = reinterpret_cast<const v2d*>(g.xedge) + qkf_uniform(g.xedge_offs[2 * (long long)xi + 1]);
-  const v2d* const Ry = reinterpret_cast<const v2d*>(g.yedge) + qkf_uniform(g.yedge_offs[2 * (long long)yj + 1]);
+                                                __attribute__((address_space(3))) double* zacc, const int wave, const int q, const int j, const bool swap = false) {
+  const v2d* const Rx = reinterpret_cast<const v2d*>(swap ? g.yedge : g.xedge) + qkf_uniform((swap ? g.yedge_offs : g.xedge_offs)[2 * (long long)xi + 1]);
+  const v2d* const Ry = reinterpret_cast<const v2d*>(swap ? g.xedge : g.yedge) + qkf_uniform((swap ? g.xedge_offs : g.yedge_offs)[2 * (long long)yj + 1]);
   const int mt = a / TILE, nt = b / TILE, ng = (1 << g.edge_k) >> 4, inv = qk_recip20(mt), units = PAIRS ? qk_edge_units(mt, nt, NW) : mt * nt;
   double zr = 0, zi = 0;
   for (int u = wave; u < units; u += NW) {
@@ -428,7 +478,7 @@
 
 struct QkfSite {
   int a, a2, b, b2, at, nks, mt, nt, nn, W, inv, inv2, pd, ps, next;
-  bool small;
+  bool small, sw;
   const v2d *Ak, *Bk;
 };
 typedef int v4i __attribute__((ext_vector_type(4)));
@@ -443,33 +493,32 @@
   const int32_t* const yt = g.ytrue + (long long)yj * n1;
   const v2d* const xdata = reinterpret_cast<const v2d*>(g.xdata);
   const v2d* const ydata = reinterpret_cast<const v2d*>(g.ydata);
-  auto put = [&](const int e, const int a, const int a2, const int b, const int b2, const int ps, const int next, const bool small, const v2d* const A, const v2d* const B)
-                 __attribute__((always_inline)) {
-    const int mt = a / TILE, nt = b2 / TILE;
-    const int W = small ? nt : max(1, min(nt, XCAP / (TILE * a2)));
-    rec[3 * e] = (v4i){a, a2, b, b2};
-    rec[3 * e + 1] = (v4i){xt[e], (yt[e] + 3) >> 2, W, small ? 1 : 0};
-    rec[3 * e + 2] = (v4i){qk_recip20(mt), ps, next, ITEM_RECIPS ? qk_unit_recips(nt, W, false) : 0};
-    m_off[2 * e] = (long long)(((const char*)A - (const char*)xdata) / 16);
-    m_off[2 * e + 1] = (long long)(((const char*)B - (const char*)ydata) / 16);
+  auto put = [&](const int e, const int len, const int o, const bool sw, const v2d* const X, const v2d* const Y) __attribute__((always_inline)) {
+    const QkStepRec r = qk_step_record(xd, xt, yd, yt, e, len, o, sw, rule, ITEM_RECIPS);
+    rec[3 * e] = (v4i){r.w[0], r.w[1], r.w[2], r.w[3]};
+    rec[3 * e + 1] = (v4i){r.w[4], r.w[5], r.w[6], r.w[7]};
+    rec[3 * e + 2] = (v4i){r.w[8], r.w[9], r.w[10], r.w[11]};
+    m_off[2 * e] = (long long)(((const char*)(o ? Y : X) - (const char*)xdata) / 16);
+    m_off[2 * e + 1] = (long long)(((const char*)(o ? X : Y) - (const char*)ydata) / 16);
   };
-  auto plain = [&](const int e, const int next) __attribute__((always_inline)) {
-    const int a = xd[e], a2 = xd[e + 1], b = yd[e], b2 = yd[e + 1];
-    put(e, a, a2, b, b2, 1, next, qk_seg_small(rule, a, a2, b, b2, 2), xdata + (g.xoffs[(long long)xi * ns + e] >> 1), ydata + (g.yoffs[(long long)yj * ns + e] >> 1));
+  auto plain = [&](const int e, const int o, const bool sw) __attribute__((always_inline)) {
+    put(e, 1, o, sw, xdata + (g.xoffs[(long long)xi * ns + e] >> 1), ydata + (g.yoffs[(long long)yj * ns + e] >> 1));
   };
   if (g.seg == nullptr) {
-    for (int e = tid; e < ns; e += NT) plain(e, e + 1);
+    for (int e = tid; e < ns; e += NT) plain(e, 0, false);
     return;
   }
   const int ek = g.edge_k, k_hi = ns - ek;
-  const unsigned long long w0 = g.seg[2 * pair], w1 = g.seg[2 * pair + 1];
+  const unsigned long long w0 = g.seg[4 * pair], w1 = g.seg[4 * pair + 1], o0 = g.seg[4 * pair + 2], o1 = g.seg[4 * pair + 3];
   for (int e = ek + tid; e < k_hi; e += NT) {
     const int i = e - ek;
-    if (qk_seg_bit(w0, w1, i) && e + 1 < k_hi) {
-      const int a = xd[e], a2 = xd[e + 2], b = yd[e], b2 = yd[e + 2];
-      put(e, a, a2, b, b2, 2, e + 2, qk_seg_small(rule, a, a2, b, b2, 4), reinterpret_cast<const v2d*>(g.xmg) + (g.xmg_offs[(long long)xi * g.merge_steps + i] >> 1),
+    const bool merged = qk_seg_bit(w0, w1, i) && e + 1 < k_hi;
+    const int len = merged ? 2 : 1, o = qk_seg_bit(o0, o1, i) ? 1 : 0;
+    const bool sw = qk_seg_bit(o0, o1, i + len) != (o != 0);
+    if (merged)
+      put(e, 2, o, sw, reinterpret_cast<const v2d*>(g.xmg) + (g.xmg_offs[(long long)xi * g.merge_steps + i] >> 1),
           reinterpret_cast<const v2d*>(g.ymg) + (g.ymg_offs[(long long)yj * g.merge_steps + i] >> 1));
-    } else plain(e, e + 1);
+    else plain(e, o, sw);
   }
 }
 
@@ -532,7 +581,7 @@
     const v4i r0 = rec[3 * k], r1 = rec[3 * k + 1], r2 = rec[3 * k + 2];
     QkfSite s;
     s.a = rfl(r0.x), s.a2 = rfl(r0.y), s.b = rfl(r0.z), s.b2 = rfl(r0.w);
-    s.at = rfl(r1.x), s.nks = rfl(r1.y), s.W = rfl(r1.z), s.small = rfl(r1.w) != 0;
+    s.at = rfl(r1.x), s.nks = rfl(r1.y), s.W = rfl(r1.z), s.small = (rfl(r1.w) & QK_REC_SMALL) != 0, s.sw = (rfl(r1.w) & QK_REC_SWITCH) != 0;
     s.inv = rfl(r2.x), s.inv2 = rfl(r2.w);
     s.ps = rfl(r2.y), s.pd = 1 << s.ps, s.next = rfl(r2.z);
     s.mt = s.a / TILE, s.nt = s.b2 / TILE, s.nn = s.a2 / TILE;
@@ -580,8 +629,9 @@
     if (edges) {
       const v4i r0 = rec[3 * ek];
       const int a_e = rfl(r0.x), b_e = rfl(r0.z);
+      const bool o1 = !DET && (rfl(rec[3 * ek + 1].w) & QK_REC_ORIENT) != 0;
       xg = a_e * b_e > XCAP;
-      qkf_edge_prefix<NW, QKF_EDGE_PAIRS(WPS), QKF_EDGE_SETS(WPS)>(g, xi, yj, a_e, b_e, XL, G0, xg, wave, q, j);
+      qkf_edge_prefix<NW, QKF_EDGE_PAIRS(WPS), QKF_EDGE_SETS(WPS)>(g, o1 ? yj : xi, o1 ? xi : yj, a_e, b_e, XL, G0, xg, wave, q, j, o1);
       __syncthreads();
     }
     QKF_STAMP(0);
@@ -666,7 +716,9 @@
             const QkfStream nxt = more ? a_stream(sc, w, it + NW) : chain ? b_stream(sn, 0, wn, wave) : a_stream(sc, w, it);
             const int tix = sc.pd * ta + un.p;
             const QkfTurn turn{tcur + tbl * sc.nn, tix, tbroken, g.err};
-            if (kmax == 4) qkf_p2_item<true, DET>(T[S - 1], fr, primed, a_stream(sc, w, it), w * QKF_XBLOCK, sc.nn, 4, XL + ob + tbl * QKF_XBLOCK, q, j, nxt, turn);
+            if (!DET && sc.sw)
+              qkf_p2_switch<false>(T[S - 1], T[S - 1], fr, primed, a_stream(sc, w, it), kmax, sc.nn, kmax, (__attribute__((address_space(3))) double*)(XL + ob + tbl * (a2 * TILE) + q * TILE + j), 0, nxt);
+            else if (kmax == 4) qkf_p2_item<true, DET>(T[S - 1], fr, primed, a_stream(sc, w, it), w * QKF_XBLOCK, sc.nn, 4, XL + ob + tbl * QKF_XBLOCK, q, j, nxt, turn);
             else qkf_p2_item<false, DET>(T[S - 1], fr, primed, a_stream(sc, w, it), w * QKF_XBLOCK, sc.nn, kmax, XL + ob + tbl * QKF_XBLOCK, q, j, nxt, turn);
             primed = more || chain;
           }
@@ -689,10 +741,13 @@
         xb = ob;
       }
     }
+    const int fl_end = DET ? 0 : rfl(rec[3 * (k_hi - 1) + 1].w);
+    const bool sw_end = (fl_end & QK_REC_SWITCH) != 0, o_end = ((fl_end & QK_REC_ORIENT) != 0) != sw_end;
     if (edges) {
       const v4i r0 = rec[3 * (k_hi - 1)];
-      const int a_e = rfl(r0.y), b_e = rfl(r0.w);
-      qkf_edge_suffix<NW, QKF_EDGE_PAIRS(WPS), QKF_EDGE_SETS(WPS)>(g, xi, yj, a_e, b_e, (const lds_v2d*)(XL + xb), (const v2d*)(G0 + (long long)cur * g.x_plane), xg, zacc, wave, q, j);
+      const int a_l = rfl(r0.y), b_l = rfl(r0.w), a_e = sw_end ? b_l : a_l, b_e = sw_end ? a_l : b_l;
+      qkf_edge_suffix<NW, QKF_EDGE_PAIRS(WPS), QKF_EDGE_SETS(WPS)>(g, o_end ? yj : xi, o_end ? xi : yj, a_e, b_e, (const lds_v2d*)(XL + xb), (const v2d*)(G0 + (long long)cur * g.x_plane), xg, zacc, wave,
+                                                                   q, j, o_end);
       __syncthreads();
     }
     if (tid == 0) {
@@ -700,6 +755,7 @@
       if (edges)
         for (int w_ = 0; w_ < NW; ++w_) zz.x += zacc[2 * w_], zz.y += zacc[2 * w_ + 1];
       else zz = xg ? G0[(long long)cur * g.x_plane] : (v2d)XL[xb];
+      if (o_end) zz.y = -zz.y;
       g.values[p] = zz.x * zz.x + zz.y * zz.y;
       if (g.z) {
         g.z[2 * p] = zz.x;
@@ -924,7 +980,7 @@
     const v4i r0 = rec[3 * k], r1 = rec[3 * k + 1], r2 = rec[3 * k + 2];
     QkfSite s;
     s.a = rfl(r0.x), s.a2 = rfl(r0.y), s.b = rfl(r0.z), s.b2 = rfl(r0.w);
-    s.at = rfl(r1.x), s.nks = rfl(r1.y), s.W = rfl(r1.z), s.small = rfl(r1.w) != 0;
+    s.at = rfl(r1.x), s.nks = rfl(r1.y), s.W = rfl(r1.z), s.small = (rfl(r1.w) & QK_REC_SMALL) != 0, s.sw = (rfl(r1.w) & QK_REC_SWITCH) != 0;
     s.inv = rfl(r2.x);
     s.ps = rfl(r2.y), s.pd = 1 << s.ps, s.next = rfl(r2.z);
     s.mt = s.a / TILE, s.nt = s.b2 / TILE, s.nn = s.a2 / TILE;
@@ -986,8 +1042,9 @@
     if (edges) {
       const v4i r0 = rec[3 * ek];
       const int a_e = rfl(r0.x), b_e = rfl(r0.z);
+      const bool o1 = !DET && (rfl(rec[3 * ek + 1].w) & QK_REC_ORIENT) != 0;
       xg = a_e * b_e > XCAP;
-      qkf_edge_prefix<NW, QKF_EDGE_PAIRS(WPS), QKF_EDGE_SETS(WPS)>(g, xi, yj, a_e, b_e, XL, G0, xg, wave, q, j);
+      qkf_edge_prefix<NW, QKF_EDGE_PAIRS(WPS), QKF_EDGE_SETS(WPS)>(g, o1 ? yj : xi, o1 ? xi : yj, a_e, b_e, XL, G0, xg, wave, q, j, o1);
       __syncthreads();
     }
     QKF_STAMP(0);
@@ -1072,7 +1129,11 @@
             const unsigned nd1 = 0;
             lds_v2d* const xo = XL + ob + (2 * tp + un.half) * QKF_XBLOCK;
             const QkfTurn tp_turn{tcur + (2 * tp + un.half) * sc.nn, sc.pd * ta + pr.p, tbroken, g.err};
-            if (has1) {
+            if (!DET && sc.sw) {
+              lds_double* const dsw = (lds_double*)(XL + ob + (2 * tp + un.half) * (a2 * TILE) + q * TILE + j);
+              if (has1) qkf_p2_switch<true>(T0, T1, fr, true, a_stream(sc, v), 4, sc.nn, kmax, dsw, 2 * a2 * TILE, nxt);
+              else qkf_p2_switch<false>(T0, T1, fr, true, a_stream(sc, v), 4, sc.nn, kmax, dsw, 0, nxt);
+            } else if (has1) {
               if (kmax == 4) qkf_p2_dual<true, true, DET>(T0, T1, fr, fs, a_stream(sc, v), w * QKF_XBLOCK, sc.nn, 4, xo, q, j, nxt, np1, nd1, tp_turn);
               else qkf_p2_dual<false, true, DET>(T0, T1, fr, fs, a_stream(sc, v), w * QKF_XBLOCK, sc.nn, kmax, xo, q, j, nxt, np1, nd1, tp_turn);
             } else {
@@ -1100,10 +1161,13 @@
       }
     }
     if (tid == QKF_PULLER(NT)) qkf_pull_next(g, xcc, gang_round, slot + (psel ^ 1));
+    const int fl_end = DET ? 0 : rfl(rec[3 * (k_hi - 1) + 1].w);
+    const bool sw_end = (fl_end & QK_REC_SWITCH) != 0, o_end = ((fl_end & QK_REC_ORIENT) != 0) != sw_end;
     if (edges) {
       const v4i r0 = rec[3 * (k_hi - 1)];
-      const int a_e = rfl(r0.y), b_e = rfl(r0.w);
-      qkf_edge_suffix<NW, QKF_EDGE_PAIRS(WPS), QKF_EDGE_SETS(WPS)>(g, xi, yj, a_e, b_e, (const lds_v2d*)(XL + xb), (const v2d*)(G0 + (long long)cur * g.x_plane), xg, zacc, wave, q, j);
+      const int a_l = rfl(r0.y), b_l = rfl(r0.w), a_e = sw_end ? b_l : a_l, b_e = sw_end ? a_l : b_l;
+      qkf_edge_suffix<NW, QKF_EDGE_PAIRS(WPS), QKF_EDGE_SETS(WPS)>(g, o_end ? yj : xi, o_end ? xi : yj, a_e, b_e, (const lds_v2d*)(XL + xb), (const v2d*)(G0 + (long long)cur * g.x_plane), xg, zacc, wave,
+                                                                   q, j, o_end);
     }
     __syncthreads();
     const long long pn = slot[psel ^ 1];
@@ -1112,6 +1176,7 @@
       if (edges)
         for (int w_ = 0; w_ < NW; ++w_) zz.x += zacc[2 * w_], zz.y += zacc[2 * w_ + 1];
       else zz = xg ? G0[(long long)cur * g.x_plane] : (v2d)XL[xb];
+      if (o_end) zz.y = -zz.y;
       g.values[p] = zz.x * zz.x + zz.y * zz.y;
       if (g.z) {
         g.z[2 * p] = zz.x;
diff --git a/qml-cutensornet_amd/csrc/qk_plan.h b/qml-cutensornet_amd/csrc/qk_plan.h
--- a/qml-cutensornet_amd/csrc/qk_plan.h
+++ b/qml-cutensornet_amd/csrc/qk_plan.h
@@ -85,40 +85,110 @@
   const long long work_m = 4ll * a * b2 * (b + a2), work_p = 2ll * a * bm * (b + am) + 2ll * am * b2 * (bm + a2);
   return (qk_seg_small(r, a, a2, b, b2, 4) || (!qk_seg_small(r, a, am, b, bm, 2) && !qk_seg_small(r, am, a2, bm, b2, 2))) && work_m <= work_p;
 }
+static constexpr int QK_SWITCH_PRICE = 40;
+QK_HD static inline bool qk_seg_small_o(const QkSegRule& r, const int o, const int a, const int a2, const int b, const int b2, const int pd) {
+  return o ? qk_seg_small(r, b, b2, a, a2, pd) : qk_seg_small(r, a, a2, b, b2, pd);
+}
 QK_HD static inline QkSegMask qk_segment_chain(const int32_t* const xd, const int32_t* const xt, const int32_t* const yd, const int32_t* const yt, const int n_sites, const int ek,
-                                               const QkSegRule& rule, const int parities, const bool greedy, long long* const objective = nullptr, int* const steps = nullptr) {
+                                               const QkSegRule& rule, const int parities, const bool greedy, long long* const objective = nullptr, int* const steps = nullptr,
+                                               const int assoc = 0, const int switch_price = QK_SWITCH_PRICE, QkSegMask* const orient = nullptr, int* const switches = nullptr) {
   const int m = n_sites - 2 * ek;
-  auto may = [&](const int i) { return i + 1 < m && i < QK_SEG_BITS && ((parities >> (i & 1)) & 1) != 0 && qk_merge_admissible(rule, xd, yd, ek + i); };
-  auto plain_cost = [&](const int i) { return qk_step_instr(2, xd[ek + i], xd[ek + i + 1], yd[ek + i], yd[ek + i + 1], xt[ek + i], yt[ek + i]) + QK_STEP_PRICE; };
-  auto merged_cost = [&](const int i) { return qk_step_instr(4, xd[ek + i], xd[ek + i + 2], yd[ek + i], yd[ek + i + 2], xt[ek + i], yt[ek + i]) + QK_STEP_PRICE; };
-  QkSegMask take{{0ull, 0ull}};
+  const int mode = (greedy || m + 1 > QK_SEG_BITS) ? 0 : assoc;
+  auto may = [&](const int i, const int o) {
+    return i + 1 < m && i < QK_SEG_BITS && ((parities >> (i & 1)) & 1) != 0 && qk_merge_admissible(rule, o ? yd : xd, o ? xd : yd, ek + i);
+  };
+  auto step_cost = [&](const int i, const int o, const int len) {
+    const int e = ek + i;
+    return (o ? qk_step_instr(2 * len, yd[e], yd[e + len], xd[e], xd[e + len], yt[e], xt[e]) : qk_step_instr(2 * len, xd[e], xd[e + len], yd[e], yd[e + len], xt[e], yt[e])) + QK_STEP_PRICE;
+  };
+  auto may_switch = [&](const int i, const int o, const int len) {
+    const int e = ek + i;
+    return qk_seg_small_o(rule, o, xd[e], xd[e + len], yd[e], yd[e + len], 2 * len);
+  };
+  auto bit = [](const QkSegMask& k, const int i) { return qk_seg_bit(k.w[0], k.w[1], i); };
+  auto set = [](QkSegMask& k, const int i) { k.w[i >> 6] |= 1ull << (i & 63); };
+  QkSegMask take[2] = {{{0ull, 0ull}}, {{0ull, 0ull}}};
+  QkSegMask swit[2] = {{{0ull, 0ull}}, {{0ull, 0ull}}};
+  int o_start = 0;
   if (greedy) {
     for (int i = 0; i < m && i < QK_SEG_BITS; ++i)
-      if (may(i)) take.w[i >> 6] |= 1ull << (i & 63);
+      if (may(i, 0)) set(take[0], i);
+  } else if (mode <= 1) {
+    struct Best {
+      long long c;
+      int sw, n1, st;
+    };
+    auto less = [](const Best& a, const Best& b) { return a.c != b.c ? a.c < b.c : a.sw != b.sw ? a.sw < b.sw : a.n1 != b.n1 ? a.n1 < b.n1 : a.st < b.st; };
+    auto same = [](const Best& a, const Best& b) { return a.c == b.c && a.sw == b.sw && a.n1 == b.n1 && a.st == b.st; };
+    Best f1[2] = {{0, 0, 0, 0}, {0, 0, 0, 0}}, f2[2] = {{0, 0, 0, 0}, {0, 0, 0, 0}};
+    const int no = mode == 1 ? 2 : 1;
+    for (int i = m - 1; i >= 0; --i) {
+      Best f0[2] = {{0, 0, 0, 0}, {0, 0, 0, 0}};
+      for (int o = 0; o < no; ++o) {
+        auto cand = [&](const int len, bool& sw) {
+          const Best* const rest = len == 2 ? f2 : f1;
+          const long long c = step_cost(i, o, len);
+          Best b{c + rest[o].c, rest[o].sw, rest[o].n1 + o, rest[o].st + 1};
+          sw = false;
+          if (mode == 1 && may_switch(i, o, len)) {
+            const Best s{c + switch_price + rest[1 - o].c, rest[1 - o].sw + 1, rest[1 - o].n1 + o, rest[1 - o].st + 1};
+            if (less(s, b)) b = s, sw = true;
+          }
+          return b;
+        };
+        bool sw = false, swm = false;
+        Best b = cand(1, sw);
+        if (may(i, o)) {
+          const Best bm = cand(2, swm);
+          if (less(bm, b) || (same(bm, b) && (i & 1) == 0)) b = bm, sw = swm, set(take[o], i);
+        }
+        if (sw) set(swit[o], i);
+        f0[o] = b;
+      }
+      for (int o = 0; o < 2; ++o) f2[o] = f1[o], f1[o] = f0[o];
+    }
+    if (mode == 1 && less(f1[1], f1[0])) o_start = 1;
   } else {
-    long long c1 = 0, c2 = 0;
-    int s1 = 0, s2 = 0;
-    for (int i = m - 1; i >= 0; --i) {
-      long long c = plain_cost(i) + c1;
-      int s = s1 + 1;
-      if (may(i)) {
-        const long long cm = merged_cost(i) + c2;
-        const int sm = s2 + 1;
-        if (cm < c || (cm == c && (sm < s || (sm == s && (i & 1) == 0)))) c = cm, s = sm, take.w[i >> 6] |= 1ull << (i & 63);
-      }
-      c2 = c1, s2 = s1, c1 = c, s1 = s;
-    }
+    o_start = mode == 3 ? 1 : 0;
   }
-  QkSegMask out{{0ull, 0ull}};
+  QkSegMask out{{0ull, 0ull}}, ori{{0ull, 0ull}};
   long long obj = 0;
-  int n_steps = 0;
+  int n_steps = 0, n_sw = 0, o = o_start;
   for (int i = 0; i < m; ++n_steps) {
-    if (qk_seg_bit(take.w[0], take.w[1], i)) out.w[i >> 6] |= 1ull << (i & 63), obj += merged_cost(i), i += 2;
-    else obj += plain_cost(i), i += 1;
+    const bool mg = mode >= 2 ? may(i, o) : bit(take[o], i);
+    const int len = mg ? 2 : 1;
+    const bool sw = mode >= 2 ? may_switch(i, o, len) : bit(swit[o], i);
+    if (mg) set(out, i);
+    if (o)
+      for (int s = i; s < i + len; ++s) set(ori, s);
+    obj += step_cost(i, o, len) + (sw ? switch_price : 0);
+    if (sw) o ^= 1, ++n_sw;
+    i += len;
   }
+  if (o) set(ori, m);
   if (objective) *objective = obj;
   if (steps) *steps = n_steps;
+  if (orient) *orient = ori;
+  if (switches) *switches = n_sw;
   return out;
+}
+
+struct QkStepRec {
+  int w[12];
+};
+static constexpr int QK_REC_SMALL = 1, QK_REC_ORIENT = 2, QK_REC_SWITCH = 4;
+QK_HD static inline QkStepRec qk_step_record(const int32_t* xd, const int32_t* xt, const int32_t* yd, const int32_t* yt, const int e, const int len, const int o, const bool sw,
+                                             const QkSegRule& rule, const bool item_recips) {
+  if (o) {
+    const int32_t* t = xd;
+    xd = yd, yd = t, t = xt, xt = yt, yt = t;
+  }
+  const int a = xd[e], a2 = xd[e + len], b = yd[e], b2 = yd[e + len];
+  const bool small = qk_seg_small(rule, a, a2, b, b2, 2 * len);
+  const int mt = a / QK_TILE, nt = b2 / QK_TILE;
+  const int lim = rule.xcap / (QK_TILE * a2), W = small ? nt : (lim < 1 ? 1 : lim < nt ? lim : nt);
+  return QkStepRec{{a, a2, b, b2, xt[e], (yt[e] + 3) >> 2, W, (small ? QK_REC_SMALL : 0) | (o ? QK_REC_ORIENT : 0) | (sw ? QK_REC_SWITCH : 0), qk_recip20(mt), len == 2 ? 2 : 1, e + len,
+                    item_recips ? qk_unit_recips(nt, W, false) : 0}};
 }
 
 struct qk_ctx;
@@ -163,6 +233,8 @@
   int fused_wgs = 0;
   bool deterministic = false;
   int merge_mode = 2;
+  int assoc_mode = 1;
+  int switch_price = QK_SWITCH_PRICE;
   bool fused_dual = true;
   bool gang = false;
 };
diff --git a/qml-cutensornet_amd/csrc/qkgram.hip b/qml-cutensornet_amd/csrc/qkgram.hip
--- a/qml-cutensornet_amd/csrc/qkgram.hip
+++ b/qml-cutensornet_amd/csrc/qkgram.hip
@@ -267,12 +267,13 @@
 
 __global__ __launch_bounds__(256) void qk_segment_kernel(const int32_t* __restrict__ xdims, const int32_t* __restrict__ xtrue, const int32_t* __restrict__ ydims, const int32_t* __restrict__ ytrue,
                                                          const int n_sites, const int ek, const int32_t* __restrict__ pairs, const long long npairs, const QkSegRule rule, const int parities,
-                                                         const bool greedy, unsigned long long* __restrict__ seg) {
+                                                         const bool greedy, const int assoc, const int switch_price, unsigned long long* __restrict__ seg) {
   const long long p = (long long)blockIdx.x * blockDim.x + threadIdx.x;
   if (p >= npairs) return;
   const long long xo = (long long)pairs[2 * p] * (n_sites + 1), yo = (long long)pairs[2 * p + 1] * (n_sites + 1);
-  const QkSegMask m = qk_segment_chain(xdims + xo, xtrue + xo, ydims + yo, ytrue + yo, n_sites, ek, rule, parities, greedy);
-  seg[2 * p] = m.w[0], seg[2 * p + 1] = m.w[1];
+  QkSegMask o{{0ull, 0ull}};
+  const QkSegMask m = qk_segment_chain(xdims + xo, xtrue + xo, ydims + yo, ytrue + yo, n_sites, ek, rule, parities, greedy, nullptr, nullptr, assoc, switch_price, &o);
+  seg[4 * p] = m.w[0], seg[4 * p + 1] = m.w[1], seg[4 * p + 2] = o.w[0], seg[4 * p + 3] = o.w[1];
 }
 
 #ifdef QK_LAB
@@ -359,8 +360,10 @@
   if (const char* v = std::getenv("QK_WAVE2")) p.wave2_path = std::atoi(v) != 0, p.wave2_ring = std::atoi(v) != 2;
   if (const char* v = std::getenv("QK_FUSED")) p.fused_path = std::atoi(v);
   if (const char* v = std::getenv("QK_MERGE")) p.merge_mode = std::max(0, std::min(2, std::atoi(v)));
+  if (const char* v = std::getenv("QK_ASSOC")) p.assoc_mode = std::max(0, std::min(3, std::atoi(v)));
+  if (const char* v = std::getenv("QK_SWITCH_PRICE")) p.switch_price = std::max(0, std::min(100000, std::atoi(v)));
   if (const char* v = std::getenv("QK_DETERMINISTIC"))
-    if (std::atoi(v) != 0) p.deterministic = true;
+    if (std::atoi(v) != 0) p.deterministic = true, p.assoc_mode = 0;
   if (const char* v = std::getenv("QK_FUSED_SPLIT")) p.fused_split = std::max(0, std::min(2, std::atoi(v)));
   if (const char* v = std::getenv("QK_FUSED_WGS")) p.fused_wgs = std::max(0, std::min(2, std::atoi(v)));
   if (const char* v = std::getenv("QK_WGS_PER_CU")) p.wgs_per_cu = std::max(1, std::min(4, std::atoi(v)));
@@ -752,10 +755,18 @@
   }
 }
 
+static bool seg_assoc_of(const int kernel) {
+#if QKF_QUAD
+  if (kernel == QK_KERNEL_FUSED_DUAL) return false;
+#endif
+  return kernel == QK_KERNEL_FUSED_DUAL || kernel == QK_KERNEL_FUSED1 || kernel == QK_KERNEL_FUSED2;
+}
+
 static int ensure_segments(qk_ctx* c, const qk_mps_set* xs, const qk_mps_set* ys, qk_plan* plan, const QkSweepChoice& ch, const int merge_mode, SweepArgs& a) {
   const long long np = (long long)plan->pairs.size() / 2;
   const bool both = merge_mode >= 2 && xs->mg_stride == 1 && ys->mg_stride == 1;
-  const unsigned long long key[8] = {1ull,
+  const int assoc = merge_mode >= 2 ? c->policy.assoc_mode : 0, switch_price = c->policy.switch_price;
+  const unsigned long long key[8] = {2ull | ((unsigned long long)assoc << 8) | ((unsigned long long)switch_price << 16),
                                      xs->uid,
                                      ys->uid,
                                      (unsigned long long)a.edge_k,
@@ -769,18 +780,18 @@
     (void)hipFree(plan->d_seg), plan->d_seg = nullptr;
   }
   QkDevBuf seg;
-  HIP_TRY(seg.alloc((size_t)np * 2 * sizeof(unsigned long long)));
+  HIP_TRY(seg.alloc((size_t)np * 4 * sizeof(unsigned long long)));
   unsigned long long* const d = seg.get<unsigned long long>();
   for (int i = 0; i < ch.n_runs; ++i) {
     const QkSweepRun& r = ch.run[i];
     const QkSegRule rule = seg_rule_of(r.kernel);
     if (r.count <= 0) continue;
     if (rule.cap == 0) {
-      HIP_TRY(hipMemsetAsync(d + 2 * r.first, 0, (size_t)r.count * 2 * sizeof(unsigned long long), c->stream));
+      HIP_TRY(hipMemsetAsync(d + 4 * r.first, 0, (size_t)r.count * 4 * sizeof(unsigned long long), c->stream));
       continue;
     }
     qk_segment_kernel<<<dim3((unsigned)((r.count + 255) / 256)), dim3(256), 0, c->stream>>>(a.xdims, a.xtrue, a.ydims, a.ytrue, a.n_sites, a.edge_k, a.pairs + 2 * r.first, r.count, rule, both ? 3 : 1,
-                                                                                            merge_mode == 1, d + 2 * r.first);
+                                                                                            merge_mode == 1, seg_assoc_of(r.kernel) ? assoc : 0, switch_price, d + 4 * r.first);
   }
   HIP_TRY(hipGetLastError());
   plan->d_seg = static_cast<unsigned long long*>(seg.release());
@@ -874,7 +885,7 @@
     ar.npairs = r.count, ar.nq = r.nq, ar.gang_n = r.gang_n;
     if (i == 1) {
       HIP_TRY(hipEventRecord(c->ev_mid, c->stream));
-      ar.pairs = a.pairs + 2 * r.first, ar.values = a.values + r.first, ar.z = a.z ? a.z + 2 * r.first : nullptr, ar.seg = a.seg ? a.seg + 2 * r.first : nullptr;
+      ar.pairs = a.pairs + 2 * r.first, ar.values = a.values + r.first, ar.z = a.z ? a.z + 2 * r.first : nullptr, ar.seg = a.seg ? a.seg + 4 * r.first : nullptr;
       ar.counter = counter + 8 * QK_QSTRIDE, ar.tail = a.tail + 2;
       if (plan->nq > 1)
         for (int s_ = 0; s_ <= 8; ++s_) ar.qstart[s_] = plan->qstart[8 + s_] - r.first;
```

After: 766,000, median of 6. +1.6%, better.
